# ErickRosete/tacorl

Measured on AMD Instinct MI355X. Metric: offline grad-steps/sec (batch=256, 84x84 RGB), higher is better.
Workload: dtype bf16; 1 GPU; tacorl actor-critic training_step, frozen LMP (BASELINE configs[1]); per_gpu_batch=256, global_batch=256, window=16, image=84x84x3, frames=fp32 CHW (reference batch schema), latent_plan=16, n_action_samples=4, phase=Q (epoch>=bc_epochs), action_decoder_loss=every step (reference behaviour), parallelism=dp1, hip_graph=True, losses_finite=True

## Files before the change

### include/tacorl_hip.h

```cpp
#ifndef TACORL_HIP_H
#define TACORL_HIP_H
#include <stddef.h>
#ifdef __cplusplus
extern "C" {
#endif

typedef void* tacorl_stream_t;

#define TACORL_MAXP 16
enum { TACORL_F32 = 0, TACORL_BF16 = 1 };
enum { TACORL_ACT_NONE = 0, TACORL_ACT_RELU = 1, TACORL_ACT_SILU = 2, TACORL_ACT_TANH = 3 };

int tacorl_hip_version(void);
int tacorl_hip_init(int device);
const char* tacorl_hip_last_error(void);
int tacorl_time_mark(unsigned long long* marks, int slot, tacorl_stream_t stream);
int tacorl_time_spin(unsigned long long* marks, int slot, long ticks, tacorl_stream_t stream);

int tacorl_linear_fwd(int nprob, const float* const* x, int ldx, const float* const* w,
                      const float* const* b, float* const* y, float* const* z, const int* M,
                      int K, int N, int act, int compute_dtype, tacorl_stream_t stream);
size_t tacorl_linear_add_fwd_ws_bytes(int nprob, const int* M, int K, int N);
int tacorl_linear_add_fwd(int nprob, const float* const* x, int ldx, const float* const* w,
                          const float* const* b, const float* const* addend, int ld_add, float* const* y,
                          int ldy, const int* M, int K, int N, int act, int compute_dtype, void* ws,
                          size_t ws_bytes, tacorl_stream_t stream);
int tacorl_rnn_linear_supported(int M, int K, int N);
int tacorl_rnn_linear_fwd(const void* x_bf16, const void* w_bf16, const float* bias, const float* addend,
                          int ld_add, float* y, void* y_bf16, int M, int K, int N, int act,
                          tacorl_stream_t stream);
int tacorl_rnn_linear_fwd_batch(int nprob, const void* const* x_bf16, const void* const* w_bf16,
                                const float* const* bias, const float* const* addend, int ld_add,
                                float* const* y, void* const* y_bf16, int M, int K, int N, const int* acts,
                                tacorl_stream_t stream);
int tacorl_rnn_linear_fwd_batch_twin(int nprob, const void* const* x_bf16, const void* const* x2_bf16,
                                     const void* const* w_bf16, const float* const* bias, const float* const* addend,
                                     const float* const* addend2, int ld_add, float* const* y, float* const* y2,
                                     void* const* y_bf16, void* const* y2_bf16, int M, int M2, int K, int N,
                                     const int* acts, tacorl_stream_t stream);
int tacorl_rnn_linear_fwd_batch_ext(int nprob, const void* const* x_bf16, const void* const* x2_bf16,
                                    const void* const* w_bf16, const float* const* bias, const float* const* addend,
                                    const float* const* addend2, int ld_add, float* const* y, float* const* y2,
                                    void* const* y_bf16, void* const* y2_bf16, int M, int M2, int K, int N,
                                    const int* acts, const void* const* x_ext, const void* const* x2_ext,
                                    const void* const* w_ext, const float* const* bias2, tacorl_stream_t stream);
int tacorl_rnn_linear_ld_supported(int M, int K, int N, int ldx, int ldy);
int tacorl_rnn_linear_ld(int nprob, const void* const* x_bf16, int ldx, const void* const* w_bf16, const float* const* bias,
                         const float* const* bias2, const float* const* addend, int ld_add, const void* const* x_ext,
                         const void* const* w_ext, const float* const* mask_src, float* const* y, void* const* y_bf16, int ldy,
                         int M, int K, int N, int act, tacorl_stream_t stream);
int tacorl_build_ad_input_bf16(const float* plan, const float* emb, int ld_emb, void* out_bf16, int B, int T, int Tm,
                               int P, int E, tacorl_stream_t stream);
int tacorl_rnn_linear_bwd_step(const void* x_bf16, const void* wt_bf16, const float* addend, int ld_add,
                               const float* mask_src, float* y, void* y_bf16, int M, int K, int N,
                               tacorl_stream_t stream);
int tacorl_rnn_wgrad_supported(int R, int M, int N);
int tacorl_rnn_wgrad(const void* dz_bf16, int ld_dz, const void* x_bf16, int ld_x, int R, int M, int N, float* dw,
                     float* db, int accumulate, tacorl_stream_t stream);
int tacorl_rnn_wgrad_batch(int n, const void* const* dz_bf16, int ld_dz, const void* const* x_bf16, int ld_x, const int* R,
                           int M, int N, float* const* dw, float* const* db, int accumulate, tacorl_stream_t stream);
size_t tacorl_rnn_wgrad_slabs_ws_bytes(int slabs, int Mp, int N);
int tacorl_rnn_wgrad_slabs(const void* dz_bf16, int ld_dz, const void* x_bf16, int ld_x, int R, int Mp, int N, int rows,
                           int slabs, float* dw, float* db, int accumulate, void* ws, size_t ws_bytes, tacorl_stream_t stream);
int tacorl_rnn_linear_bwd_batch(int nprob, const void* const* x_bf16, const void* const* wt_bf16,
                                const float* const* addend, int ld_add, const float* const* mask_src,
                                float* const* y, void* const* y_bf16, int M, int K, int N, tacorl_stream_t stream);
int tacorl_birnn_swap_rows(const float* src, int ld_src, float* dst, int ld_dst, int n_outer, int n_inner, int cols,
                           tacorl_stream_t stream);
int tacorl_transpose_to_bf16(const float* src, void* dst, int R, int C, tacorl_stream_t stream);
int tacorl_transpose_to_bf16_batch(int n, const float* const* src, void* const* dst, const int* R, const int* C,
                                   tacorl_stream_t stream);
int tacorl_transpose_pad_to_bf16(const float* src, void* dst, int R, int C, int ld_dst, tacorl_stream_t stream);
int tacorl_pad_to_bf16(const float* src, int ld_src, void* dst, int ld_dst, long rows, int cols, tacorl_stream_t stream);

int tacorl_linear_dgrad(int nprob, const float* const* dz, int ld_dz, const float* const* w,
                        float* const* out, int ld_out, const float* const* src, int ld_src, int act_src,
                        const float* const* addend, int ld_add, const int* M, int O, int I,
                        int compute_dtype, tacorl_stream_t stream);
size_t tacorl_linear_dgrad_ws_bytes(int nprob, const int* M, int O, int I);
int tacorl_linear_dgrad_splitk(int nprob, const float* const* dz, int ld_dz, const float* const* w,
                               float* const* out, int ld_out, const float* const* src, int ld_src, int act_src,
                               const float* const* addend, int ld_add, const int* M, int O, int I,
                               int compute_dtype, void* ws, size_t ws_bytes, tacorl_stream_t stream);
size_t tacorl_linear_wgrad_ws_bytes(int nprob, const int* M, int K, int O);
int tacorl_linear_wgrad(int nprob, const float* const* x, int ldx, const float* const* dz, int ld_dz,
                        const int* M, int K, int O, float* const* dw, float* const* db, int accumulate,
                        int compute_dtype, void* ws, size_t ws_bytes, tacorl_stream_t stream);
int tacorl_conv2d_relu_fwd(int nprob, const void* const* x, const float* const* w,
                           const float* const* b, float* const* y, const int* n_img, int H, int W,
                           int C, int KH, int KW, int S, int CO, int x_dtype, int compute_dtype,
                           tacorl_stream_t stream);

long tacorl_encoder_param_layout(long* offsets11);
long tacorl_encoder_act_layout(int n_img, int H, int W, long* offsets5);
int tacorl_encoder_fwd(int nprob, const void* const* img, const float* const* params,
                       float* const* out , float* const* act, const int* n_img, int H,
                       int W, int img_dtype, int compute_dtype, tacorl_stream_t stream);
size_t tacorl_encoder_bwd_ws_bytes(int nprob, const int* n_img, int H, int W);
int tacorl_encoder_bwd(int nprob, const void* const* img, const float* const* params,
                       const float* const* act, const float* const* d_out, float* const* grads,
                       const int* n_img, int H, int W, int img_dtype, int compute_dtype,
                       int accumulate, void* ws, size_t ws_bytes, tacorl_stream_t stream);

long tacorl_encoder_fused_wpk_bytes(void);
int tacorl_encoder_fused_supported(int H, int W);
int tacorl_encoder_fused_act_format(int H, int W);
int tacorl_encoder_pack_weights(int nprob, const float* const* params, void* const* packed,
                                tacorl_stream_t stream);
int tacorl_encoder_fwd_fused(int nprob, const void* const* img, const void* const* packed,
                             const float* const* params, float* const* out, float* const* act,
                             const int* n_img, int H, int W, tacorl_stream_t stream);
int tacorl_encoder_fwd_fused_wg(int nprob, const void* const* img, const void* const* packed,
                                const float* const* params, float* const* out, float* const* act,
                                const int* n_img, int H, int W, int max_workgroups, tacorl_stream_t stream);

size_t tacorl_encoder_bwd_fused_ws_bytes(int nprob, const int* n_img, int H, int W);
int tacorl_encoder_bwd_fused(int nprob, const void* const* img, const float* const* params,
                             const float* const* act, const float* const* d_out,
                             float* const* grads, const int* n_img, int H, int W, int accumulate,
                             void* ws, size_t ws_bytes, tacorl_stream_t stream);
int tacorl_encoder_bwd_fused_pack(int nprob, const float* const* params, const int* n_img, int H, int W,
                                  void* ws, size_t ws_bytes, tacorl_stream_t stream);
int tacorl_encoder_bwd_fused_head(int nprob, const float* const* params, const float* const* act,
                                  const float* const* d_out, const int* n_img, int H, int W,
                                  int prepacked, void* ws, size_t ws_bytes, tacorl_stream_t stream);
int tacorl_encoder_bwd_fused_fc_wgrad(int nprob, const float* const* act, const float* const* d_out,
                                      float* const* grads, const int* n_img, int H, int W,
                                      int accumulate, void* ws, size_t ws_bytes, tacorl_stream_t stream);
int tacorl_encoder_bwd_fused_conv(int nprob, const void* const* img, const float* const* params,
                                  const float* const* act, float* const* grads, const int* n_img, int H,
                                  int W, int accumulate, int prepacked, void* ws, size_t ws_bytes,
                                  tacorl_stream_t stream);
int tacorl_encoder_bwd_fused_conv_parts(int nprob, const void* const* img, const float* const* params,
                                        const float* const* act, float* const* grads, const int* n_img, int H,
                                        int W, int accumulate, int prepacked, int parts, void* ws,
                                        size_t ws_bytes, tacorl_stream_t stream);

long tacorl_mlp_param_layout(int n_layers, const int* dims, long* w_off, long* b_off);
long tacorl_mlp_act_layout(int M, int n_layers, const int* dims, const int* acts, long* z_off,
                           long* y_off);
int tacorl_mlp_fwd(int nprob, const float* const* x, int ldx, const float* const* params,
                   float* const* act, const int* M, int n_layers, const int* dims,
                   const int* acts, int compute_dtype, tacorl_stream_t stream);
int tacorl_mlp_fwd_fused_supported(int nprob, int n_layers, const int* dims, int ldx);
int tacorl_mlp_lean_supported(int nprob, int n_layers, const int* dims, int ldx, int ldo, int ldd);
int tacorl_mlp_fwd_fused(int nprob, const float* const* x, int ldx, const float* const* params,
                         const void* const* params_bf16, float* const* act, const int* M,
                         int n_layers, const int* dims, const int* acts, int lean, tacorl_stream_t stream);
int tacorl_mlp_fwd_fused_gather_supported(int nprob, const int* M, int n_layers, const int* dims, const int* acts,
                                          int ldx, int lean);
int tacorl_mlp_fwd_fused_gather(int nprob, const int* nseg, const float* const* seg_ptr, const int* seg_ld,
                                const int* seg_c0, const int* seg_mod, float* const* x_out, int ldx,
                                const float* const* params, const void* const* params_bf16, float* const* act,
                                const int* M, int n_layers, const int* dims, const int* acts, int lean,
                                tacorl_stream_t stream);
int tacorl_to_bf16_batch(int n, const float* const* src, void* const* dst, const long* count,
                         tacorl_stream_t stream);
size_t tacorl_mlp_bwd_ws_bytes(int nprob, const int* M, int n_layers, const int* dims);
int tacorl_mlp_bwd(int nprob, const float* const* x, int ldx, const float* const* params,
                   const float* const* act, const float* const* d_out, int ldo, float* const* grads,
                   float* const* d_x, int ldd, const int* M, int n_layers, const int* dims,
                   const int* acts, int compute_dtype, int accumulate, void* ws, size_t ws_bytes,
                   tacorl_stream_t stream);
int tacorl_mlp_bwd_fused_supported(int nprob, int n_layers, const int* dims, int ldo, int ldd);
size_t tacorl_mlp_bwd_fused_ws_bytes(int nprob, const int* M, int n_layers, const int* dims);
int tacorl_mlp_bwd_fused_dgrad(int nprob, const float* const* params, const float* const* act,
                               const float* const* d_out, int ldo, float* const* d_x, int ldd,
                               const int* M, int n_layers, const int* dims, const int* acts,
                               int prepacked, void* ws, size_t ws_bytes, tacorl_stream_t stream);
int tacorl_mlp_bwd_fused_pack(int nprob, const float* const* params, const int* M, int n_layers,
                              const int* dims, void* ws, size_t ws_bytes, tacorl_stream_t stream);
int tacorl_prep_batch_begin(void);
int tacorl_reduce_batch_begin(void);
int tacorl_reduce_batch_end(tacorl_stream_t stream);
int tacorl_prep_batch_end(tacorl_stream_t stream);
int tacorl_mlp_bwd_fused_wgrad(int nprob, const float* const* x, int ldx, const float* const* act,
                               const float* const* d_out, int ldo, float* const* grads, const int* M,
                               int n_layers, const int* dims, const int* acts, int accumulate, int lean,
                               void* ws, size_t ws_bytes, tacorl_stream_t stream);

int tacorl_pack_images(const float* src, long img_pitch, int src_nchw, void* dst, int dst_dtype,
                       int n, int C, int H, int W, tacorl_stream_t stream);
int tacorl_pack_images_batch(int njobs, const float* const* src, const long* img_pitch, void* const* dst,
                             const int* n_img, int dst_dtype, int H, int W, tacorl_stream_t stream);
int tacorl_pack_images_window_batch(int njobs, const float* const* src, const long* img_pitch, void* const* dst,
                                    const int* n_img, void* const* dst_first, void* const* dst_last,
                                    const int* window, int dst_dtype, int H, int W, tacorl_stream_t stream);
int tacorl_pack_images_u8_batch(int njobs, const void* const* src, const long* img_pitch_bytes, void* const* dst,
                                const int* n_img, int dst_dtype, int H, int W, tacorl_stream_t stream);
int tacorl_pack_images_u8_gather_batch(int njobs, const void* const* src, const long* img_pitch_bytes,
                                       const long* const* index, const int* index_stride, void* const* dst,
                                       const int* n_img, int dst_dtype, int H, int W, tacorl_stream_t stream);
int tacorl_gather_frames_u8(const void* frames, long frame_bytes, const long* index, void* dst, long n,
                            tacorl_stream_t stream);
int tacorl_pack_images_u8_aug_batch(int njobs, const void* const* src, const long* img_pitch_bytes,
                                    void* const* dst, const int* const* shift, const float* const* jitter,
                                    const int* n_img, int dst_dtype, int H, int W, int pad,
                                    tacorl_stream_t stream);
int tacorl_pack_images_u8_resize_aug_gather_batch(int njobs, const void* const* src, const long* img_pitch_bytes,
                                                  const long* const* index, const int* index_stride, void* const* dst,
                                                  const int* const* shift, const float* const* jitter, const int* n_img,
                                                  int dst_dtype, int src_H, int src_W, int H, int W, int pad,
                                                  tacorl_stream_t stream);
int tacorl_pack_images_u8_aug_gather_batch(int njobs, const void* const* src, const long* img_pitch_bytes,
                                           const long* const* index, const int* index_stride, void* const* dst,
                                           const int* const* shift, const float* const* jitter, const int* n_img,
                                           int dst_dtype, int H, int W, int pad, tacorl_stream_t stream);
int tacorl_stage_transition(const void* disp, int disp_dtype, float* reward, float* done, int B,
                            const float* acts_src, float* acts_dst, long n_acts, tacorl_stream_t stream);
int tacorl_sample_transitions(const long* possible_steps, long n_possible, const long* ep_start, const long* ep_end,
                              int n_episodes, const long* nn_ptr, long n_nn, const long* nn_val, const float* actions,
                              const long* idx, const long* strategy, const long* disp, const double* u_choice,
                              long current_horizon, long n_frames, int B, int A, long* ids, float* action,
                              float* reward, float* done, int* status, tacorl_stream_t stream);
int tacorl_copy_cols(const float* src, int ld_src, float* dst, int ld_dst, int rows, int cols,
                     int src_row_mod, int accumulate, tacorl_stream_t stream);
int tacorl_copy_cols_batch(int n, const float* const* src, const int* ld_src, float* const* dst,
                           const int* ld_dst, const int* rows, const int* cols,
                           const int* src_row_mod, const int* accumulate, tacorl_stream_t stream);
int tacorl_reduce_rows_mod(const float* in, int ld_in, float* out, int ld_out, int B, int cols,
                           int reps, tacorl_stream_t stream);
int tacorl_reduce_rows_mod_batch(int n, const float* const* in, int ld_in, float* const* out, int ld_out, int B,
                                 int cols, int reps, tacorl_stream_t stream);
int tacorl_uniform_actions(const float* u01, float* dst, int ld_dst, int rows, int A,
                           int discrete_gripper, tacorl_stream_t stream);

int tacorl_tanh_normal_sample(const float* head, int ld_head, const float* eps, const float* gumbel_u,
                              int hard_rsample, float* act_out, int ld_act, float* logp, int* grip_idx,
                              int n, int M, int Ac, tacorl_stream_t stream);
int tacorl_tanh_normal_sample_batch(int njobs, const float* const* head, int ld_head,
                                    const float* const* eps, const float* const* gumbel_u,
                                    const int* hard_rsample, float* const* act_out, int ld_act,
                                    float* const* logp, int* const* grip_idx, const int* n, int M, int Ac,
                                    const float* u01, float* u_dst, int u_rows, int A, int u_discrete,
                                    tacorl_stream_t stream);

int tacorl_add_rows_bcast(const float* x, int ldx, const float* add, float* out, int R, int T, int D,
                          int Dp, tacorl_stream_t stream);
int tacorl_attention_fwd(const float* qkv, float* out, int B, int T, int D, int H, tacorl_stream_t stream);
int tacorl_attention_dropout_fwd(const float* qkv, float* out, const unsigned char* keep, float keep_scale, int B,
                                 int T, int D, int H, tacorl_stream_t stream);
int tacorl_attention_dropout_bwd(const float* qkv, const float* d_out, float* d_qkv, const unsigned char* keep,
                                 float keep_scale, int B, int T, int D, int H, tacorl_stream_t stream);
int tacorl_dropout_mul(float* x, const unsigned char* keep, float keep_scale, long n, tacorl_stream_t stream);
int tacorl_add_layernorm_fwd(const float* x, const float* res, const float* w, const float* b, float* y,
                             float* stats, int R, int D, float eps, tacorl_stream_t stream);
int tacorl_pr_encoder_fused_supported(int D, int T, int H, int FF, int L);
int tacorl_pr_encoder_fused_train_supported(int D, int T, int H, int FF, int L);
int tacorl_pr_encoder_fused(const float* emb, int ld_emb, const float* params, const void* params_bf16,
                            const long* offsets, float* pooled, int B, int D, int T, int H, int FF, int L,
                            tacorl_stream_t stream);
int tacorl_pr_encoder_fused_sample(const float* emb, int ld_emb, const float* params, const void* params_bf16,
                                   const long* offsets, float* pooled, int B, int D, int T, int H, int FF, int L,
                                   const float* Wc, const float* bc, const float* eps, float* head, float* plan,
                                   int A, float min_std, tacorl_stream_t stream);
int tacorl_pr_encoder_fused_train(const float* emb, int ld_emb, const float* params, const void* params_bf16,
                                  const long* offsets, float* pooled, int B, int D, int T, int H, int FF, int L,
                                  float* const* save, tacorl_stream_t stream);
int tacorl_pr_encoder_bwd_fused(const float* params, const long* offsets, const float* d_pool, const float* d_head,
                                const float* Wc, int A2, float* dx, const float* const* saved, float* const* dz,
                                const void* const* wt, float* ln_part, float* const* ln_grads, int B, int D, int T, int H,
                                int FF, int L, tacorl_stream_t stream);
int tacorl_pr_encoder_fused_train_sample(const float* emb, int ld_emb, const float* params, const void* params_bf16,
                                         const long* offsets, float* pooled, int B, int D, int T, int H, int FF, int L,
                                         float* const* save, const float* Wc, const float* bc, const float* eps,
                                         float* head, float* plan, int A, float min_std, tacorl_stream_t stream);
int tacorl_pr_head_compose(const float* w_fc, const float* b_fc, const float* w_head, const float* b_head,
                           float* Wc, float* bc, int D, int FC, int A2, tacorl_stream_t stream);
int tacorl_mean_over_t(const float* x, float* out, int B, int T, int D, tacorl_stream_t stream);
int tacorl_pr_sample(const float* head, const float* eps, float* plan, float* mu_out, float* std_out,
                     int B, int A, float min_std, tacorl_stream_t stream);

int tacorl_build_ad_input(const float* plan, const float* emb, int ld_emb, float* out, int B, int T,
// ... 89 lines not shown
```

### tacorl_amd/_lib.py

```python
import ctypes as C
import os

HERE = os.path.dirname(os.path.abspath(__file__))
LIB_PATH = os.environ.get("TACORL_HIP_LIB") or os.path.join(HERE, "lib", "libtacorl_hip.so")

F32, BF16 = 0, 1
ACT_NONE, ACT_RELU, ACT_SILU, ACT_TANH = 0, 1, 2, 3
MAXP = 16

LOG_SLOTS = [
    "alpha_loss", "alpha", "actor_loss", "bellman_q1_loss", "bellman_q2_loss", "conservative_q1_loss",
    "conservative_q2_loss", "q1_loss", "q2_loss", "alpha_prime", "alpha_prime_loss", "q1_data", "q1_random",
    "q1_policy", "q2_data", "q2_random", "q2_policy", "action_loss",
]

_p, _i, _l, _f, _sz = C.c_void_p, C.c_int, C.c_long, C.c_float, C.c_size_t
_SIGS = {
    "tacorl_hip_version": (_i, []),
    "tacorl_hip_init": (_i, [_i]),
    "tacorl_hip_last_error": (C.c_char_p, []),
    "tacorl_time_mark": (_i, [_p, _i, _p]),
    "tacorl_time_spin": (_i, [_p, _i, _l, _p]),
    "tacorl_linear_fwd": (_i, [_i, _p, _i, _p, _p, _p, _p, _p, _i, _i, _i, _i, _p]),
    "tacorl_linear_add_fwd_ws_bytes": (_sz, [_i, _p, _i, _i]),
    "tacorl_linear_add_fwd": (_i, [_i, _p, _i, _p, _p, _p, _i, _p, _i, _p, _i, _i, _i, _i, _p, _sz, _p]),
    "tacorl_rnn_linear_supported": (_i, [_i, _i, _i]),
    "tacorl_rnn_linear_fwd": (_i, [_p, _p, _p, _p, _i, _p, _p, _i, _i, _i, _i, _p]),
    "tacorl_rnn_linear_fwd_batch": (_i, [_i, _p, _p, _p, _p, _i, _p, _p, _i, _i, _i, _p, _p]),
    "tacorl_rnn_linear_fwd_batch_twin": (_i, [_i, _p, _p, _p, _p, _p, _p, _i, _p, _p, _p, _p, _i, _i, _i, _i, _p, _p]),
    "tacorl_rnn_linear_fwd_batch_ext": (_i, [_i, _p, _p, _p, _p, _p, _p, _i, _p, _p, _p, _p, _i, _i, _i, _i, _p, _p, _p, _p, _p, _p]),
    "tacorl_rnn_linear_ld_supported": (_i, [_i, _i, _i, _i, _i]),
    "tacorl_rnn_linear_ld": (_i, [_i, _p, _i, _p, _p, _p, _p, _i, _p, _p, _p, _p, _p, _i, _i, _i, _i, _i, _p]),
    "tacorl_rnn_linear_bwd_step": (_i, [_p, _p, _p, _i, _p, _p, _p, _i, _i, _i, _p]),
    "tacorl_rnn_linear_bwd_batch": (_i, [_i, _p, _p, _p, _i, _p, _p, _p, _i, _i, _i, _p]),
    "tacorl_rnn_wgrad_supported": (_i, [_i, _i, _i]),
    "tacorl_rnn_wgrad": (_i, [_p, _i, _p, _i, _i, _i, _i, _p, _p, _i, _p]),
    "tacorl_rnn_wgrad_batch": (_i, [_i, _p, _i, _p, _i, _p, _i, _i, _p, _p, _i, _p]),
    "tacorl_rnn_wgrad_slabs_ws_bytes": (_sz, [_i, _i, _i]),
    "tacorl_rnn_wgrad_slabs": (_i, [_p, _i, _p, _i, _i, _i, _i, _i, _i, _p, _p, _i, _p, _sz, _p]),
    "tacorl_birnn_swap_rows": (_i, [_p, _i, _p, _i, _i, _i, _i, _p]),
    "tacorl_transpose_to_bf16": (_i, [_p, _p, _i, _i, _p]),
    "tacorl_transpose_to_bf16_batch": (_i, [_i, _p, _p, _p, _p, _p]),
    "tacorl_transpose_pad_to_bf16": (_i, [_p, _p, _i, _i, _i, _p]),
    "tacorl_pad_to_bf16": (_i, [_p, _i, _p, _i, _l, _i, _p]),
    "tacorl_pr_encoder_fused_supported": (_i, [_i, _i, _i, _i, _i]),
    "tacorl_pr_encoder_fused_train_supported": (_i, [_i, _i, _i, _i, _i]),
    "tacorl_pr_encoder_fused": (_i, [_p, _i, _p, _p, _p, _p, _i, _i, _i, _i, _i, _i, _p]),
    "tacorl_pr_encoder_fused_train": (_i, [_p, _i, _p, _p, _p, _p, _i, _i, _i, _i, _i, _i, _p, _p]),
    "tacorl_pr_encoder_bwd_fused": (_i, [_p, _p, _p, _p, _p, _i, _p, _p, _p, _p, _p, _p, _i, _i, _i, _i, _i, _i, _p]),
    "tacorl_pr_encoder_fused_train_sample": (_i, [_p, _i, _p, _p, _p, _p, _i, _i, _i, _i, _i, _i, _p, _p, _p, _p, _p, _p, _i, _f, _p]),
    "tacorl_pr_encoder_fused_sample": (_i, [_p, _i, _p, _p, _p, _p, _i, _i, _i, _i, _i, _i, _p, _p, _p, _p, _p, _i, _f, _p]),
    "tacorl_pr_head_compose": (_i, [_p, _p, _p, _p, _p, _p, _i, _i, _i, _p]),
    "tacorl_to_bf16_batch": (_i, [_i, _p, _p, _p, _p]),
    "tacorl_mlp_bwd_fused_supported": (_i, [_i, _i, _p, _i, _i]),
    "tacorl_mlp_bwd_fused_ws_bytes": (_sz, [_i, _p, _i, _p]),
    "tacorl_mlp_bwd_fused_dgrad": (_i, [_i, _p, _p, _p, _i, _p, _i, _p, _i, _p, _p, _i, _p, _sz, _p]),
    "tacorl_mlp_bwd_fused_pack": (_i, [_i, _p, _p, _i, _p, _p, _sz, _p]),
    "tacorl_prep_batch_begin": (_i, []),
    "tacorl_reduce_batch_begin": (_i, []),
    "tacorl_reduce_batch_end": (_i, [_p]),
    "tacorl_prep_batch_end": (_i, [_p]),
    "tacorl_mlp_bwd_fused_wgrad": (_i, [_i, _p, _i, _p, _p, _i, _p, _p, _i, _p, _p, _i, _i, _p, _sz, _p]),
    "tacorl_mlp_fwd_fused_supported": (_i, [_i, _i, _p, _i]),
    "tacorl_mlp_lean_supported": (_i, [_i, _i, _p, _i, _i, _i]),
    "tacorl_mlp_fwd_fused": (_i, [_i, _p, _i, _p, _p, _p, _p, _i, _p, _p, _i, _p]),
    "tacorl_mlp_fwd_fused_gather_supported": (_i, [_i, _p, _i, _p, _p, _i, _i]),
    "tacorl_mlp_fwd_fused_gather": (_i, [_i, _p, _p, _p, _p, _p, _p, _i, _p, _p, _p, _p, _i, _p, _p, _i, _p]),
    "tacorl_add_rows_bcast": (_i, [_p, _i, _p, _p, _i, _i, _i, _i, _p]),
    "tacorl_attention_fwd": (_i, [_p, _p, _i, _i, _i, _i, _p]),
    "tacorl_attention_dropout_fwd": (_i, [_p, _p, _p, _f, _i, _i, _i, _i, _p]),
    "tacorl_attention_dropout_bwd": (_i, [_p, _p, _p, _p, _f, _i, _i, _i, _i, _p]),
    "tacorl_dropout_mul": (_i, [_p, _p, _f, _l, _p]),
    "tacorl_add_layernorm_fwd": (_i, [_p, _p, _p, _p, _p, _p, _i, _i, _f, _p]),
    "tacorl_mean_over_t": (_i, [_p, _p, _i, _i, _i, _p]),
    "tacorl_pr_sample": (_i, [_p, _p, _p, _p, _p, _i, _i, _f, _p]),
    "tacorl_build_ad_input": (_i, [_p, _p, _i, _p, _i, _i, _i, _i, _i, _p]),
    "tacorl_build_ad_input_bf16": (_i, [_p, _p, _i, _p, _i, _i, _i, _i, _i, _p]),
    "tacorl_ad_input_proj": (_i, [_p, _p, _i, _p, _p, _p, _i, _i, _i, _i, _i, _i, _p]),
    "tacorl_logistic_mixture_ws_bytes": (_sz, [_i, _i, _i]),
    "tacorl_logistic_mixture_loss": (_i, [_p, _i, _p, _p, _p, _i, _i, _i, _i, _i, _i, _f, _f, _p, _sz, _p]),
    "tacorl_logistic_mixture_finish": (_i, [_p, _sz, _i, _i, _i, _p, _p]),
    "tacorl_logistic_mixture_sample": (_i, [_p, _i, _p, _p, _p, _i, _i, _i, _p]),
    "tacorl_linear_dgrad": (_i, [_i, _p, _i, _p, _p, _i, _p, _i, _i, _p, _i, _p, _i, _i, _i, _p]),
    "tacorl_linear_dgrad_ws_bytes": (_sz, [_i, _p, _i, _i]),
    "tacorl_linear_dgrad_splitk": (_i, [_i, _p, _i, _p, _p, _i, _p, _i, _i, _p, _i, _p, _i, _i, _i, _p, _sz, _p]),
    "tacorl_linear_wgrad_ws_bytes": (_sz, [_i, _p, _i, _i]),
    "tacorl_linear_wgrad": (_i, [_i, _p, _i, _p, _i, _p, _i, _i, _p, _p, _i, _i, _p, _sz, _p]),
    "tacorl_relu_mask_mul": (_i, [_p, _p, _p, _p, _l, _p]),
    "tacorl_ad_input_bwd": (_i, [_p, _p, _p, _i, _i, _i, _i, _i, _i, _i, _p]),
    "tacorl_plmp_demb_finish": (_i, [_p, _p, _i, _i, _p, _i, _p, _p, _i, _i, _i, _i, _p]),
    "tacorl_bcast_over_t": (_i, [_p, _p, _i, _i, _i, _f, _i, _p]),
    "tacorl_attention_bwd": (_i, [_p, _p, _p, _i, _i, _i, _i, _p]),
    "tacorl_add_layernorm_bwd_ws_bytes": (_sz, [_i, _i]),
    "tacorl_add_layernorm_bwd": (_i, [_p, _p, _p, _p, _p, _p, _p, _p, _i, _i, _i, _p, _sz, _p]),
    "tacorl_gauss_kl_balanced": (_i, [_p, _p, _p, _p, _i, _i, _f, _f, _f, _i, _f, _p, _p]),
    "tacorl_pr_sample_bwd": (_i, [_p, _p, _p, _p, _i, _i, _f, _p]),
    "tacorl_conv2d_relu_fwd": (_i, [_i, _p, _p, _p, _p, _p, _i, _i, _i, _i, _i, _i, _i, _i, _i, _p]),
    "tacorl_encoder_param_layout": (_l, [_p]),
    "tacorl_encoder_act_layout": (_l, [_i, _i, _i, _p]),
    "tacorl_encoder_fwd": (_i, [_i, _p, _p, _p, _p, _p, _i, _i, _i, _i, _p]),
    "tacorl_encoder_bwd_ws_bytes": (_sz, [_i, _p, _i, _i]),
    "tacorl_encoder_bwd": (_i, [_i, _p, _p, _p, _p, _p, _p, _i, _i, _i, _i, _i, _p, _sz, _p]),
    "tacorl_encoder_fused_wpk_bytes": (_l, []),
    "tacorl_encoder_fused_supported": (_i, [_i, _i]),
    "tacorl_encoder_fused_act_format": (_i, [_i, _i]),
    "tacorl_encoder_pack_weights": (_i, [_i, _p, _p, _p]),
    "tacorl_encoder_fwd_fused": (_i, [_i, _p, _p, _p, _p, _p, _p, _i, _i, _p]),
    "tacorl_encoder_fwd_fused_wg": (_i, [_i, _p, _p, _p, _p, _p, _p, _i, _i, _i, _p]),
    "tacorl_encoder_bwd_fused_ws_bytes": (_sz, [_i, _p, _i, _i]),
    "tacorl_encoder_bwd_fused": (_i, [_i, _p, _p, _p, _p, _p, _p, _i, _i, _i, _p, _sz, _p]),
    "tacorl_encoder_bwd_fused_pack": (_i, [_i, _p, _p, _i, _i, _p, _sz, _p]),
    "tacorl_encoder_bwd_fused_head": (_i, [_i, _p, _p, _p, _p, _i, _i, _i, _p, _sz, _p]),
    "tacorl_encoder_bwd_fused_fc_wgrad": (_i, [_i, _p, _p, _p, _p, _i, _i, _i, _p, _sz, _p]),
    "tacorl_encoder_bwd_fused_conv": (_i, [_i, _p, _p, _p, _p, _p, _i, _i, _i, _i, _p, _sz, _p]),
    "tacorl_encoder_bwd_fused_conv_parts": (_i, [_i, _p, _p, _p, _p, _p, _i, _i, _i, _i, _i, _p, _sz, _p]),
    "tacorl_mlp_param_layout": (_l, [_i, _p, _p, _p]),
    "tacorl_mlp_act_layout": (_l, [_i, _i, _p, _p, _p, _p]),
    "tacorl_mlp_fwd": (_i, [_i, _p, _i, _p, _p, _p, _i, _p, _p, _i, _p]),
    "tacorl_mlp_bwd_ws_bytes": (_sz, [_i, _p, _i, _p]),
    "tacorl_mlp_bwd": (_i, [_i, _p, _i, _p, _p, _p, _i, _p, _p, _i, _p, _i, _p, _p, _i, _i, _p, _sz, _p]),
    "tacorl_pack_images": (_i, [_p, _l, _i, _p, _i, _i, _i, _i, _i, _p]),
    "tacorl_pack_images_batch": (_i, [_i, _p, _p, _p, _p, _i, _i, _i, _p]),
    "tacorl_pack_images_window_batch": (_i, [_i, _p, _p, _p, _p, _p, _p, _p, _i, _i, _i, _p]),
    "tacorl_pack_images_u8_batch": (_i, [_i, _p, _p, _p, _p, _i, _i, _i, _p]),
    "tacorl_pack_images_u8_gather_batch": (_i, [_i, _p, _p, _p, _p, _p, _p, _i, _i, _i, _p]),
    "tacorl_pack_images_u8_aug_gather_batch": (_i, [_i, _p, _p, _p, _p, _p, _p, _p, _p, _i, _i, _i, _i, _p]),
    "tacorl_pack_images_u8_resize_aug_gather_batch": (_i, [_i, _p, _p, _p, _p, _p, _p, _p, _p, _i, _i, _i, _i, _i, _i, _p]),
    "tacorl_gather_frames_u8": (_i, [_p, _l, _p, _p, _l, _p]),
    "tacorl_pack_images_u8_aug_batch": (_i, [_i, _p, _p, _p, _p, _p, _p, _i, _i, _i, _i, _p]),
    "tacorl_stage_transition": (_i, [_p, _i, _p, _p, _i, _p, _p, _l, _p]),
    "tacorl_sample_transitions": (_i, [_p, _l, _p, _p, _i, _p, _l, _p, _p, _p, _p, _p, _p, _l, _l, _i, _i, _p, _p, _p, _p, _p, _p]),
    "tacorl_copy_cols": (_i, [_p, _i, _p, _i, _i, _i, _i, _i, _p]),
    "tacorl_copy_cols_batch": (_i, [_i, _p, _p, _p, _p, _p, _p, _p, _p, _p]),
    "tacorl_reduce_rows_mod": (_i, [_p, _i, _p, _i, _i, _i, _i, _p]),
    "tacorl_reduce_rows_mod_batch": (_i, [_i, _p, _i, _p, _i, _i, _i, _i, _p]),
    "tacorl_uniform_actions": (_i, [_p, _p, _i, _i, _i, _i, _p]),
    "tacorl_tanh_normal_sample": (_i, [_p, _i, _p, _p, _i, _p, _i, _p, _p, _i, _i, _i, _p]),
    "tacorl_tanh_normal_sample_batch": (_i, [_i, _p, _i, _p, _p, _p, _p, _i, _p, _p, _p, _i, _i, _p, _p, _i, _i, _i, _p]),
    "tacorl_alpha_loss": (_i, [_p, _i, _p, _f, _f, _p, _p, _p]),
    "tacorl_alpha_loss_step": (_i, [_p, _i, _p, _f, _p, _p, _p, _p, _f, _p, _p]),
    "tacorl_actor_qmin": (_i, [_p, _p, _p, _i, _p, _p, _p, _f, _p, _p]),
    "tacorl_actor_head_bwd": (_i, [_p, _i, _p, _p, _p, _p, _i, _p, _i, _p, _p, _f, _p, _i, _i, _i, _p, _p]),
    "tacorl_tanh_normal_nll": (_i, [_p, _i, _p, _i, _i, _i, _i, _f, _p, _p, _p]),
    "tacorl_cql_ws_bytes": (_sz, [_i]),
    "tacorl_cql_loss": (_i, [_p] * 13 + [_i, _i, _i, _f, _f, _f, _f, _f, _i, _f, _p, _p, _p, _sz, _p]),
    "tacorl_adam_ws_bytes": (_sz, [_l]),
    "tacorl_adam_step": (_i, [_p, _p, _p, _p, _l, _f, _f, _p, _p, _f, _p, _sz, _p]),
    "tacorl_adam_batch_ws_bytes": (_sz, [_i]),
    "tacorl_adam_step_batch": (_i, [_i, _p, _p, _p, _p, _p, _p, _p, _p, _p, _p, _p, _sz, _p]),
    "tacorl_adam_step_batch_mirror": (_i, [_i, _p, _p, _p, _p, _p, _p, _p, _p, _p, _p, _p, _p, _p, _sz, _p]),
    "tacorl_cem_supported": (_i, [_i, _i, _i, _i, _i, _i]),
    "tacorl_cem_ws_bytes": (_sz, [_i, _i, _i, _i, _i, _i, _i]),
    "tacorl_cem_refine": (_i, [_i, _i, _p, _p, _p, _p, _p, _p, _i, _i, _i, _i, _i, _i, _i, _f, _f, _f, _i, _i, _p, _p, _p, _p, _p,
                               _p, _sz, _p]),
}

_lib = None


class TacorlHipError(RuntimeError):
    pass


def lib():
    global _lib
    if _lib is None:
        import torch

        if not os.path.exists(LIB_PATH):
            raise TacorlHipError(
                f"{LIB_PATH} not found: the HIP extension is required (no CPU fallback). "
                "Build it with `python -m tacorl_amd.build`.")
        L = C.CDLL(LIB_PATH)
        override = bool(os.environ.get("TACORL_HIP_LIB"))
        missing = []
        for name, (res, args) in _SIGS.items():
            fn = getattr(L, name, None)
            if fn is None:
                missing.append(name)
                continue
            fn.restype, fn.argtypes = res, args
        if override:
            import sys

            if missing:
                raise TacorlHipError(f"TACORL_HIP_LIB={LIB_PATH} lacks {len(missing)} entry point(s) of this binding "
                                     f"({', '.join(missing[:5])}...): rebuild it from this tree")
            print(f"[tacorl_amd] TACORL_HIP_LIB override active: {LIB_PATH}", file=sys.stderr, flush=True)
        _lib = L
    return _lib


def declared_symbols():
    return list(_SIGS)


def call(name, *args):
    fn = getattr(lib(), name)
    rc = fn(*args)
    if fn.restype is _i and rc != 0:
        raise TacorlHipError(f"{name} failed ({rc}): {lib().tacorl_hip_last_error().decode()}")
    return rc


def ptr(t):
    return None if t is None else C.c_void_p(t.data_ptr())


def ptr_array(tensors):
    arr = (C.c_void_p * len(tensors))()
    for i, t in enumerate(tensors):
        if t is None:
            arr[i] = None
        elif isinstance(t, int):
            arr[i] = t
        elif isinstance(t, C.c_void_p):
            arr[i] = t.value
        else:
            arr[i] = t.data_ptr()
    return arr


def int_array(vals):
    return (C.c_int * len(vals))(*[int(v) for v in vals])


def stream():
    import torch

    return C.c_void_p(torch.cuda.current_stream().cuda_stream)
```

### tacorl_amd/csrc/dense_ops.hip

```cpp
#include <stdio.h>
#include <stdlib.h>
#include <string.h>

#include <type_traits>

#include "../../include/tacorl_hip.h"
#include "enc_bwd_fused.h"
#include "mlp_fused.h"
#include "functors.h"

static thread_local char g_err[256] = "";
#define FAIL(code, ...)                        \
  do {                                         \
    snprintf(g_err, sizeof(g_err), __VA_ARGS__); \
    return (code);                             \
  } while (0)
#define CHECK(x)            \
  do {                      \
    int _r = (x);           \
    if (_r != TACORL_OK) return _r; \
  } while (0)

extern "C" const char* tacorl_hip_last_error(void) { return g_err; }
extern "C" int tacorl_hip_version(void) { return 1; }
// ... 588 lines not shown
  hipStream_t st = (hipStream_t)stream;
  EncDims d;
  if (!enc_dims(H, W, d)) FAIL(TACORL_EINVAL, "encoder: image %dx%d too small", H, W);
  if (nprob < 1 || nprob > GEMM_MAXP) FAIL(TACORL_EINVAL, "encoder_fwd: nprob %d", nprob);
  long po[E_N];
  tacorl_encoder_param_layout(po);
  const float *w1[GEMM_MAXP], *b1[GEMM_MAXP], *w2[GEMM_MAXP], *b2[GEMM_MAXP], *w3[GEMM_MAXP], *b3[GEMM_MAXP],
      *fw1[GEMM_MAXP], *fb1[GEMM_MAXP], *fw2[GEMM_MAXP], *fb2[GEMM_MAXP];
  float *y1[GEMM_MAXP], *y2[GEMM_MAXP], *y3[GEMM_MAXP], *sa[GEMM_MAXP], *h1[GEMM_MAXP];
  for (int p = 0; p < nprob; p++) {
    long ao[5];
    tacorl_encoder_act_layout(n_img[p], H, W, ao);
    const float* P = params[p];
    w1[p] = P + po[E_W1]; b1[p] = P + po[E_B1]; w2[p] = P + po[E_W2]; b2[p] = P + po[E_B2];
    w3[p] = P + po[E_W3]; b3[p] = P + po[E_B3]; fw1[p] = P + po[E_FW1]; fb1[p] = P + po[E_FB1];
    fw2[p] = P + po[E_FW2]; fb2[p] = P + po[E_FB2];
    y1[p] = act[p] + ao[0]; y2[p] = act[p] + ao[1]; y3[p] = act[p] + ao[2]; sa[p] = act[p] + ao[3];
    h1[p] = act[p] + ao[4];
  }
  CHECK(conv_fwd_any(nprob, img, w1, b1, y1, n_img, d.c1, img_dtype, cd, st));
  CHECK(conv_fwd_any(nprob, (const void* const*)y1, w2, b2, y2, n_img, d.c2, TACORL_F32, cd, st));
  CHECK(conv_fwd_any(nprob, (const void* const*)y2, w3, b3, y3, n_img, d.c3, TACORL_F32, cd, st));
  {
    SaArgs sg{};
    int mxn = 0;
    for (int p = 0; p < nprob; p++) {
      sg.y3[p] = y3[p]; sg.temp[p] = params[p] + po[E_T]; sg.out[p] = sa[p]; sg.n[p] = n_img[p];
      mxn = n_img[p] > mxn ? n_img[p] : mxn;
    }
    if (mxn > 0) hipLaunchKernelGGL(softargmax_fwd_kernel, dim3(mxn, nprob), dim3(256), 0, st, sg, d.c3.OH, d.c3.OW);
  }
  CHECK(k_linear_fwd(nprob, sa, 128, fw1, fb1, h1, nullptr, n_img, 128, 256, 256, ACT_RELU, cd, st));
  CHECK(k_linear_fwd(nprob, h1, 256, fw2, fb2, out, nullptr, n_img, 256, 32, 32, ACT_NONE, cd, st));
  return hipGetLastError() == hipSuccess ? TACORL_OK : TACORL_ELAUNCH;
}

static size_t enc_slab_bytes(int nprob, long maxn, const EncDims& d) {
  size_t m = 0, s;
  s = wgrad_ws_bytes(nprob, 192, 32, maxn * d.c1.OH * d.c1.OW); m = s > m ? s : m;
  s = wgrad_ws_bytes(nprob, 512, 64, maxn * d.c2.OH * d.c2.OW); m = s > m ? s : m;
  s = wgrad_ws_bytes(nprob, 576, 64, maxn * d.c3.OH * d.c3.OW); m = s > m ? s : m;
  s = wgrad_ws_bytes(nprob, 128, 256, maxn); m = s > m ? s : m;
  s = wgrad_ws_bytes(nprob, 256, 32, maxn); m = s > m ? s : m;
  return m;
}
static long enc_bwd_scratch_layout(int n, const EncDims& d, long* o) {
  const long sz[6] = {(long)n * 256, (long)n * 128, (long)n * d.c3.OH * d.c3.OW * 64,
                      (long)n * d.c2.OH * d.c2.OW * 64, (long)n * d.c1.OH * d.c1.OW * 32, (long)n};
  long off = 0;
  for (int i = 0; i < 6; i++) { if (o) o[i] = off; off = al4(off + sz[i]); }
  return off;
}
extern "C" size_t tacorl_encoder_bwd_ws_bytes(int nprob, const int* n_img, int H, int W) {
  EncDims d;
  if (!enc_dims(H, W, d)) return 0;
  long tot = 0, maxn = 0;
  for (int p = 0; p < nprob; p++) { tot += enc_bwd_scratch_layout(n_img[p], d, nullptr); maxn = n_img[p] > maxn ? n_img[p] : maxn; }
  return (size_t)tot * sizeof(float) + enc_slab_bytes(nprob, maxn, d);
}

extern "C" int tacorl_encoder_bwd(int nprob, const void* const* img, const float* const* params,
                                  const float* const* act, const float* const* d_out, float* const* grads,
                                  const int* n_img, int H, int W, int img_dtype, int cd, int accumulate,
                                  void* ws, size_t ws_bytes, tacorl_stream_t stream) {
  hipStream_t st = (hipStream_t)stream;
  EncDims d;
  if (!enc_dims(H, W, d)) FAIL(TACORL_EINVAL, "encoder: image %dx%d too small", H, W);
  if (nprob < 1 || nprob * 4 > GEMM_MAXP) FAIL(TACORL_EINVAL, "encoder_bwd: nprob %d (max %d)", nprob, GEMM_MAXP / 4);
  if (ws_bytes < tacorl_encoder_bwd_ws_bytes(nprob, n_img, H, W)) FAIL(TACORL_ENOMEM, "encoder_bwd: workspace too small");
  long po[E_N];
  tacorl_encoder_param_layout(po);
  const float *w2[GEMM_MAXP], *w3[GEMM_MAXP], *fw1[GEMM_MAXP], *fw2[GEMM_MAXP];
  const float *y1[GEMM_MAXP], *y2[GEMM_MAXP], *y3[GEMM_MAXP], *sa[GEMM_MAXP], *h1[GEMM_MAXP];
  float *d_h1[GEMM_MAXP], *d_sa[GEMM_MAXP], *dz3[GEMM_MAXP], *dz2[GEMM_MAXP], *dz1[GEMM_MAXP], *dtp[GEMM_MAXP];
  float *g_w1[GEMM_MAXP], *g_b1[GEMM_MAXP], *g_w2[GEMM_MAXP], *g_b2[GEMM_MAXP], *g_w3[GEMM_MAXP], *g_b3[GEMM_MAXP],
      *g_fw1[GEMM_MAXP], *g_fb1[GEMM_MAXP], *g_fw2[GEMM_MAXP], *g_fb2[GEMM_MAXP];
  float* cur = (float*)ws;
  long maxn = 0;
  for (int p = 0; p < nprob; p++) {
    long ao[5], so[6];
    tacorl_encoder_act_layout(n_img[p], H, W, ao);
    const long tot = enc_bwd_scratch_layout(n_img[p], d, so);
    const float* P = params[p];
    w2[p] = P + po[E_W2]; w3[p] = P + po[E_W3]; fw1[p] = P + po[E_FW1]; fw2[p] = P + po[E_FW2];
    y1[p] = act[p] + ao[0]; y2[p] = act[p] + ao[1]; y3[p] = act[p] + ao[2]; sa[p] = act[p] + ao[3]; h1[p] = act[p] + ao[4];
    d_h1[p] = cur + so[0]; d_sa[p] = cur + so[1]; dz3[p] = cur + so[2]; dz2[p] = cur + so[3]; dz1[p] = cur + so[4]; dtp[p] = cur + so[5];
    cur += tot;
    float* G = grads[p];
    g_w1[p] = G + po[E_W1]; g_b1[p] = G + po[E_B1]; g_w2[p] = G + po[E_W2]; g_b2[p] = G + po[E_B2];
    g_w3[p] = G + po[E_W3]; g_b3[p] = G + po[E_B3]; g_fw1[p] = G + po[E_FW1]; g_fb1[p] = G + po[E_FB1];
    g_fw2[p] = G + po[E_FW2]; g_fb2[p] = G + po[E_FB2];
    maxn = n_img[p] > maxn ? n_img[p] : maxn;
  }
  void* slab = cur;
  const size_t slab_bytes = enc_slab_bytes(nprob, maxn, d);
  CHECK(k_linear_wgrad(nprob, h1, 256, d_out, 32, n_img, 256, 32, g_fw2, g_fb2, accumulate, slab, slab_bytes, cd, st));
  CHECK(k_linear_dgrad(nprob, d_out, 32, fw2, d_h1, 256, h1, ACT_RELU, n_img, 32, 256, cd, st));
  CHECK(k_linear_wgrad(nprob, sa, 128, (const float* const*)d_h1, 256, n_img, 128, 256, g_fw1, g_fb1, accumulate, slab, slab_bytes, cd, st));
  CHECK(k_linear_dgrad(nprob, (const float* const*)d_h1, 256, fw1, d_sa, 128, nullptr, ACT_NONE, n_img, 256, 128, cd, st));
  {
    SaArgs sg{};
    int mxn = 0;
    for (int p = 0; p < nprob; p++) {
      sg.y3[p] = y3[p]; sg.temp[p] = params[p] + po[E_T]; sg.sa[p] = sa[p]; sg.d_sa[p] = d_sa[p]; sg.out[p] = dz3[p];
      sg.dtp[p] = dtp[p]; sg.n[p] = n_img[p];
      mxn = n_img[p] > mxn ? n_img[p] : mxn;
    }
    const int P3 = d.c3.OH * d.c3.OW;
    if (cd == TACORL_BF16 && nprob <= EBW_MAXP && P3 > 4 * SAB_MAXI_BIG && P3 <= 4 * SAB_MAXI_HUGE) {
      SabArgs sb{};
      for (int p = 0; p < nprob; p++) {
        sb.y3[p] = y3[p]; sb.temp[p] = params[p] + po[E_T]; sb.sa[p] = sa[p]; sb.d_sa[p] = d_sa[p]; sb.dz3[p] = dz3[p];
        sb.dtp[p] = dtp[p]; sb.gtemp[p] = grads[p] + po[E_T]; sb.n[p] = n_img[p];
      }
      if (mxn > 0) {
        hipLaunchKernelGGL(softargmax_bwd_batch_kernel<SAB_MAXI_HUGE>, dim3(mxn, nprob), dim3(256), 0, st, sb, P3, d.c3.OW);
        hipLaunchKernelGGL(sum_to_scalar_batch_kernel, dim3(nprob), dim3(256), 0, st, sb, accumulate);
      }
    } else {
      if (mxn > 0) hipLaunchKernelGGL(softargmax_bwd_kernel, dim3(mxn, nprob), dim3(256), 0, st, sg, d.c3.OH, d.c3.OW);
      for (int p = 0; p < nprob; p++)
        if (n_img[p] > 0)
          hipLaunchKernelGGL(sum_to_scalar_kernel, dim3(1), dim3(256), 0, st, dtp[p], n_img[p], grads[p] + po[E_T], accumulate);
    }
  }
  CHECK(k_conv_wgrad<float>(nprob, (const void* const*)y2, (const float* const*)dz3, n_img, d.c3, g_w3, g_b3, accumulate, slab, slab_bytes, cd, st));
  CHECK(k_conv_dgrad(nprob, (const float* const*)dz3, w3, dz2, y2, n_img, d.c3, cd, st));
  CHECK(k_conv_wgrad<float>(nprob, (const void* const*)y1, (const float* const*)dz2, n_img, d.c2, g_w2, g_b2, accumulate, slab, slab_bytes, cd, st));
  CHECK(k_conv_dgrad(nprob, (const float* const*)dz2, w2, dz1, y1, n_img, d.c2, cd, st));
  if (img_dtype == TACORL_BF16)
    CHECK(k_conv_wgrad<__bf16>(nprob, img, (const float* const*)dz1, n_img, d.c1, g_w1, g_b1, accumulate, slab, slab_bytes, cd, st));
  else
    CHECK(k_conv_wgrad<float>(nprob, img, (const float* const*)dz1, n_img, d.c1, g_w1, g_b1, accumulate, slab, slab_bytes, cd, st));
  return hipGetLastError() == hipSuccess ? TACORL_OK : TACORL_ELAUNCH;
}

static const int kFcDims[3] = {128, 256, 32};
static size_t enc_fc_slab_bytes(int nprob, long maxn) {
  size_t a = wgrad_ws_bytes(nprob, 256, 32, maxn), b = wgrad_ws_bytes(nprob, 128, 256, maxn);
  int Mx[EBW_MAXP];
  for (int p = 0; p < nprob && p < EBW_MAXP; p++) Mx[p] = (int)maxn;
  const size_t c = mlp_fused_wgrad_slab_floats(nprob, Mx, 2, kFcDims) * sizeof(float);
  a = a > b ? a : b;
  return ((a > c ? a : c) + 255) & ~(size_t)255;
}
struct EncBwdPlan {
  EncDims d;
  long po[E_N];
  size_t scratch_bytes, fcwt_off[EBW_MAXP], fcwt_each, slab_off, slab_bytes, conv_off, total;
  long so[EBW_MAXP][6], ao[EBW_MAXP][5], sbase[EBW_MAXP];
  long maxn;
};
static const int kFcActs[2] = {ACT_RELU, ACT_NONE};
static bool enc_bwd_plan(int nprob, const int* n_img, int H, int W, EncBwdPlan& pl) {
  if (!enc_dims(H, W, pl.d) || !ebw_supported(H, W) || nprob < 1 || nprob > EBW_MAXP) return false;
  tacorl_encoder_param_layout(pl.po);
  long tot = 0;
  pl.maxn = 0;
  for (int p = 0; p < nprob; p++) {
    pl.sbase[p] = tot;
    tot += enc_bwd_scratch_layout(n_img[p], pl.d, pl.so[p]);
    tacorl_encoder_act_layout(n_img[p], H, W, pl.ao[p]);
    pl.maxn = n_img[p] > pl.maxn ? n_img[p] : pl.maxn;
  }
  size_t b = ((size_t)tot * sizeof(float) + 255) & ~(size_t)255;
  pl.scratch_bytes = b;
  pl.fcwt_each = (mlp_fused_wt_elems(2, kFcDims, nullptr) * 2 + 255) & ~(size_t)255;
  for (int p = 0; p < nprob; p++) { pl.fcwt_off[p] = b; b += pl.fcwt_each; }
  pl.slab_off = b;
  pl.slab_bytes = enc_fc_slab_bytes(nprob, pl.maxn);
  b += pl.slab_bytes;
  pl.conv_off = b;
  pl.total = b + ebw_ws_bytes(nprob, n_img, H, W);
  return true;
}
extern "C" size_t tacorl_encoder_bwd_fused_ws_bytes(int nprob, const int* n_img, int H, int W) {
  EncBwdPlan pl;
  return enc_bwd_plan(nprob, n_img, H, W, pl) ? pl.total : 0;
}
static void enc_bwd_conv_problems(int nprob, const void* const* img, const float* const* params, const float* const* act,
                                  float* const* grads, const int* n_img, const EncBwdPlan& pl, void* ws, EbwProblem* pr) {
  for (int p = 0; p < nprob; p++) {
    const float* P = params[p];
    float* G = grads ? grads[p] : nullptr;
    float* sc = (float*)ws + pl.sbase[p];
    pr[p].img = img ? img[p] : nullptr;
    pr[p].y1 = act ? act[p] + pl.ao[p][0] : nullptr; pr[p].y2 = act ? act[p] + pl.ao[p][1] : nullptr;
    pr[p].dz3 = sc + pl.so[p][2];
    pr[p].w2 = P + pl.po[E_W2]; pr[p].w3 = P + pl.po[E_W3];
    pr[p].g_w1 = G ? G + pl.po[E_W1] : nullptr; pr[p].g_b1 = G ? G + pl.po[E_B1] : nullptr;
    pr[p].g_w2 = G ? G + pl.po[E_W2] : nullptr; pr[p].g_b2 = G ? G + pl.po[E_B2] : nullptr;
    pr[p].g_w3 = G ? G + pl.po[E_W3] : nullptr; pr[p].g_b3 = G ? G + pl.po[E_B3] : nullptr;
    pr[p].n = n_img[p];
  }
}
static int enc_bwd_fc_chain(int nprob, const float* const* params, const float* const* act, const float* const* d_out,
                            const int* n_img, const EncBwdPlan& pl, void* ws, hipStream_t st, int mode) {
  long wo[2], bo[2], src[MF_MAXP * MF_MAXL], dzo[MF_MAXP * MF_MAXL];
  tacorl_mlp_param_layout(2, kFcDims, wo, bo);
  const float* fcp[EBW_MAXP];
  float *dz[EBW_MAXP], *dsa[EBW_MAXP];
  void* wt[EBW_MAXP];
  for (int p = 0; p < nprob; p++) {
    fcp[p] = params[p] + pl.po[E_FW1];
    src[p * MF_MAXL + 0] = pl.ao[p][4];
    src[p * MF_MAXL + 1] = -1;
    dzo[p * MF_MAXL + 0] = pl.sbase[p] + pl.so[p][0];
    dz[p] = (float*)ws;
    dsa[p] = (float*)ws + pl.sbase[p] + pl.so[p][1];
    wt[p] = (unsigned char*)ws + pl.fcwt_off[p];
  }
  return mlp_fused_bwd(nprob, fcp, act, d_out, 32, dz, dsa, 128, wt, n_img, 2, kFcDims, kFcActs, src, dzo, wo, st, mode);
}

extern "C" int tacorl_encoder_bwd_fused_pack(int nprob, const float* const* params, const int* n_img, int H, int W,
                                             void* ws, size_t ws_bytes, tacorl_stream_t stream) {
  EncBwdPlan pl;
  if (!enc_bwd_plan(nprob, n_img, H, W, pl)) FAIL(TACORL_EINVAL, "encoder_bwd_fused_pack: geometry %dx%d / nprob %d", H, W, nprob);
  if (ws_bytes < pl.total) FAIL(TACORL_ENOMEM, "encoder_bwd_fused_pack: workspace too small");
  EbwProblem pr[EBW_MAXP];
  enc_bwd_conv_problems(nprob, nullptr, params, nullptr, nullptr, n_img, pl, ws, pr);
  int rc = enc_bwd_fc_chain(nprob, params, nullptr, nullptr, n_img, pl, ws, (hipStream_t)stream, 1);
  if (rc == TACORL_OK) rc = ebw_conv_backward(nprob, pr, H, W, 0, (unsigned char*)ws + pl.conv_off, pl.total - pl.conv_off, (hipStream_t)stream, 1);
  if (rc != TACORL_OK) FAIL(rc, "encoder_bwd_fused_pack: launch failed (%d)", rc);
  return TACORL_OK;
}
extern "C" int tacorl_encoder_bwd_fused_head(int nprob, const float* const* params, const float* const* act,
                                             const float* const* d_out, const int* n_img, int H, int W, int prepacked,
                                             void* ws, size_t ws_bytes, tacorl_stream_t stream) {
  EncBwdPlan pl;
  if (!enc_bwd_plan(nprob, n_img, H, W, pl)) FAIL(TACORL_EINVAL, "encoder_bwd_fused_head: geometry %dx%d / nprob %d", H, W, nprob);
  if (ws_bytes < pl.total) FAIL(TACORL_ENOMEM, "encoder_bwd_fused_head: workspace too small");
  const int rc = enc_bwd_fc_chain(nprob, params, act, d_out, n_img, pl, ws, (hipStream_t)stream, prepacked ? 2 : 0);
  if (rc != TACORL_OK) FAIL(rc, "encoder_bwd_fused_head: launch failed (%d)", rc);
  return TACORL_OK;
}
extern "C" int tacorl_encoder_bwd_fused_fc_wgrad(int nprob, const float* const* act, const float* const* d_out,
                                                 float* const* grads, const int* n_img, int H, int W, int accumulate,
                                                 void* ws, size_t ws_bytes, tacorl_stream_t stream) {
  hipStream_t st = (hipStream_t)stream;
  EncBwdPlan pl;
  if (!enc_bwd_plan(nprob, n_img, H, W, pl)) FAIL(TACORL_EINVAL, "encoder_bwd_fused_fc_wgrad: geometry %dx%d / nprob %d", H, W, nprob);
  if (ws_bytes < pl.total) FAIL(TACORL_ENOMEM, "encoder_bwd_fused_fc_wgrad: workspace too small");
  const float *sa[EBW_MAXP], *h1[EBW_MAXP], *d_h1[EBW_MAXP];
  float *g_fw1[EBW_MAXP], *g_fb1[EBW_MAXP], *g_fw2[EBW_MAXP], *g_fb2[EBW_MAXP];
  for (int p = 0; p < nprob; p++) {
    sa[p] = act[p] + pl.ao[p][3]; h1[p] = act[p] + pl.ao[p][4];
    d_h1[p] = (const float*)ws + pl.sbase[p] + pl.so[p][0];
    float* G = grads[p];
    g_fw1[p] = G + pl.po[E_FW1]; g_fb1[p] = G + pl.po[E_FB1]; g_fw2[p] = G + pl.po[E_FW2]; g_fb2[p] = G + pl.po[E_FB2];
  }
  void* slab = (unsigned char*)ws + pl.slab_off;
  if (mlp_fused_wgrad_ok(nprob, 2, kFcDims) &&
      mlp_fused_wgrad_slab_floats(nprob, n_img, 2, kFcDims) * sizeof(float) <= pl.slab_bytes) {
    long yoffs[MF_MAXP * MF_MAXL] = {}, dzoffs[MF_MAXP * MF_MAXL] = {};
    const float* dzb[EBW_MAXP];
    for (int p = 0; p < nprob; p++) {
      yoffs[p * MF_MAXL] = pl.ao[p][4];
      dzoffs[p * MF_MAXL] = pl.sbase[p] + pl.so[p][0];
      dzb[p] = (const float*)ws;
    }
    const long wo[2] = {pl.po[E_FW1], pl.po[E_FW2]}, bo[2] = {pl.po[E_FB1], pl.po[E_FB2]};
    if (mlp_fused_wgrad(nprob, sa, 128, act, d_out, 32, dzb, grads, (float*)slab, n_img, 2, kFcDims, yoffs, dzoffs, wo, bo,
                        accumulate, st))
      FAIL(TACORL_ELAUNCH, "encoder_bwd_fused_fc_wgrad: launch failed");
    return TACORL_OK;
  }
  CHECK(k_linear_wgrad(nprob, h1, 256, d_out, 32, n_img, 256, 32, g_fw2, g_fb2, accumulate, slab, pl.slab_bytes, TACORL_BF16, st));
  CHECK(k_linear_wgrad(nprob, sa, 128, d_h1, 256, n_img, 128, 256, g_fw1, g_fb1, accumulate, slab, pl.slab_bytes, TACORL_BF16, st));
  return TACORL_OK;
}
extern "C" int tacorl_encoder_bwd_fused_conv(int nprob, const void* const* img, const float* const* params,
                                             const float* const* act, float* const* grads, const int* n_img, int H, int W,
                                             int accumulate, int prepacked, void* ws, size_t ws_bytes,
                                             tacorl_stream_t stream) {
  return tacorl_encoder_bwd_fused_conv_parts(nprob, img, params, act, grads, n_img, H, W, accumulate, prepacked, 127, ws,
                                             ws_bytes, stream);
}
extern "C" int tacorl_encoder_bwd_fused_conv_parts(int nprob, const void* const* img, const float* const* params,
                                                   const float* const* act, float* const* grads, const int* n_img, int H,
                                                   int W, int accumulate, int prepacked, int parts, void* ws,
                                                   size_t ws_bytes, tacorl_stream_t stream) {
  hipStream_t st = (hipStream_t)stream;
  EncBwdPlan pl;
  if (!enc_bwd_plan(nprob, n_img, H, W, pl)) FAIL(TACORL_EINVAL, "encoder_bwd_fused_conv: geometry %dx%d / nprob %d", H, W, nprob);
  if (ws_bytes < pl.total) FAIL(TACORL_ENOMEM, "encoder_bwd_fused_conv: workspace too small");
  if (pl.d.c3.OH * pl.d.c3.OW > 4 * SAB_MAXI_HUGE) FAIL(TACORL_EINVAL, "encoder_bwd_fused: conv3 output too large");
  EbwProblem pr[EBW_MAXP];
  enc_bwd_conv_problems(nprob, img, params, act, grads, n_img, pl, ws, pr);
  SabArgs sb{};
  for (int p = 0; p < nprob; p++) {
    float* sc = (float*)ws + pl.sbase[p];
    sb.y3[p] = act[p] + pl.ao[p][2]; sb.temp[p] = params[p] + pl.po[E_T]; sb.sa[p] = act[p] + pl.ao[p][3];
    sb.d_sa[p] = sc + pl.so[p][1]; sb.dz3[p] = sc + pl.so[p][2]; sb.dtp[p] = sc + pl.so[p][5];
    sb.gtemp[p] = grads[p] + pl.po[E_T]; sb.n[p] = n_img[p];
  }
  const char* fe = getenv("TACORL_EBW_FUSE3");
  const int fuse3 = fe ? atoi(fe) : 1;
  const bool fused3 = fuse3 && (parts & 127) == 127 && ebw_fused3_supported(H, W);
  if (fused3) {
    for (int p = 0; p < nprob; p++) {
      pr[p].y3 = sb.y3[p]; pr[p].temp = sb.temp[p]; pr[p].sa = sb.sa[p]; pr[p].d_sa = sb.d_sa[p];
      pr[p].dtp = sb.dtp[p]; pr[p].g_temp = sb.gtemp[p];
    }
  }
  if (pl.maxn > 0 && (parts & 1) && !fused3) {
    const int P3 = pl.d.c3.OH * pl.d.c3.OW;
    if (P3 <= 4 * 13) hipLaunchKernelGGL(softargmax_bwd_batch_kernel<13>, dim3((unsigned)pl.maxn, nprob), dim3(256), 0, st, sb, P3, pl.d.c3.OW);
    else if (P3 <= 4 * SAB_MAXI_BIG) hipLaunchKernelGGL(softargmax_bwd_batch_kernel<SAB_MAXI_BIG>, dim3((unsigned)pl.maxn, nprob), dim3(256), 0, st, sb, P3, pl.d.c3.OW);
    else hipLaunchKernelGGL(softargmax_bwd_batch_kernel<SAB_MAXI_HUGE>, dim3((unsigned)pl.maxn, nprob), dim3(256), 0, st, sb, P3, pl.d.c3.OW);
    hipLaunchKernelGGL(sum_to_scalar_batch_kernel, dim3(nprob), dim3(256), 0, st, sb, accumulate);
  }
  if (!(parts & EBW_ALL)) return hipGetLastError() == hipSuccess ? TACORL_OK : TACORL_ELAUNCH;
  if ((parts & EBW_ALL) != EBW_ALL && !prepacked) FAIL(TACORL_EINVAL, "encoder_bwd_fused_conv_parts: partial calls need prepacked fragments");
  const int rc = ebw_conv_backward(nprob, pr, H, W, accumulate, (unsigned char*)ws + pl.conv_off, pl.total - pl.conv_off, st, prepacked ? 2 : 0,
                                   (parts & EBW_ALL) | (fused3 ? EBW_FUSED3 : 0));
  if (rc != TACORL_OK) FAIL(rc, "encoder_bwd_fused_conv: conv backward launch failed (%d)", rc);
  return hipGetLastError() == hipSuccess ? TACORL_OK : TACORL_ELAUNCH;
}
extern "C" int tacorl_encoder_bwd_fused(int nprob, const void* const* img, const float* const* params,
                                        const float* const* act, const float* const* d_out, float* const* grads,
                                        const int* n_img, int H, int W, int accumulate, void* ws, size_t ws_bytes,
                                        tacorl_stream_t stream) {
  int rc = tacorl_encoder_bwd_fused_head(nprob, params, act, d_out, n_img, H, W, 0, ws, ws_bytes, stream);
  if (rc == TACORL_OK) rc = tacorl_encoder_bwd_fused_fc_wgrad(nprob, act, d_out, grads, n_img, H, W, accumulate, ws, ws_bytes, stream);
  if (rc == TACORL_OK) rc = tacorl_encoder_bwd_fused_conv(nprob, img, params, act, grads, n_img, H, W, accumulate, 0, ws, ws_bytes, stream);
  return rc;
}

extern "C" long tacorl_mlp_param_layout(int L, const int* dims, long* w_off, long* b_off) {
  long off = 0;
  for (int l = 0; l < L; l++) {
    if (w_off) w_off[l] = off;
    off = al4(off + (long)dims[l + 1] * dims[l]);
    if (b_off) b_off[l] = off;
    off = al4(off + dims[l + 1]);
  }
  return off;
}
extern "C" long tacorl_mlp_act_layout(int M, int L, const int* dims, const int* acts, long* z_off, long* y_off) {
  long off = 0;
  for (int l = 0; l < L; l++) {
    if (z_off) z_off[l] = -1;
    if (acts[l] == ACT_SILU) { if (z_off) z_off[l] = off; off = al4(off + (long)M * dims[l + 1]); }
    if (y_off) y_off[l] = off;
    off = al4(off + (long)M * dims[l + 1]);
  }
  return off;
}
#define MLP_MAXL 8

struct OutActTbl { const float* d[GEMM_MAXP]; const float* y[GEMM_MAXP]; float* dz[GEMM_MAXP]; int M[GEMM_MAXP]; };
__global__ __launch_bounds__(256) void out_act_grad_kernel(OutActTbl t, int ldo, int N, int act) {
  const int p = blockIdx.y;
  const long total = (long)t.M[p] * N;
  for (long e = (long)blockIdx.x * 256 + threadIdx.x; e < total; e += (long)gridDim.x * 256) {
    const long m = e / N;
    t.dz[p][e] = t.d[p][m * ldo + (e - m * N)] * act_grad(act, t.y[p][e]);
  }
}
static int out_act_grad(int nprob, const OutActTbl& t, int ldo, int N, int act, hipStream_t st) {
  long mx = 0;
  for (int p = 0; p < nprob; p++) mx = (long)t.M[p] * N > mx ? (long)t.M[p] * N : mx;
  if (mx == 0) return TACORL_OK;
  const int gx = cdiv(mx, 256) > 1024 ? 1024 : cdiv(mx, 256);
  hipLaunchKernelGGL(out_act_grad_kernel, dim3(gx, nprob), dim3(256), 0, st, t, ldo, N, act);
  return hipGetLastError() == hipSuccess ? TACORL_OK : TACORL_ELAUNCH;
}

extern "C" int tacorl_mlp_fwd(int nprob, const float* const* x, int ldx, const float* const* params,
                              float* const* act, const int* M, int L, const int* dims, const int* acts, int cd,
                              tacorl_stream_t stream) {
  hipStream_t st = (hipStream_t)stream;
  if (L < 1 || L > MLP_MAXL || nprob < 1 || nprob > GEMM_MAXP) FAIL(TACORL_EINVAL, "mlp_fwd: bad L/nprob");
  long wo[MLP_MAXL], bo[MLP_MAXL];
  tacorl_mlp_param_layout(L, dims, wo, bo);
  for (int l = 0; l < L; l++) {
    const float *xin[GEMM_MAXP], *w[GEMM_MAXP], *b[GEMM_MAXP];
    float *y[GEMM_MAXP], *z[GEMM_MAXP];
    for (int p = 0; p < nprob; p++) {
      long zo[MLP_MAXL], yo[MLP_MAXL];
      tacorl_mlp_act_layout(M[p], L, dims, acts, zo, yo);
      xin[p] = l == 0 ? x[p] : act[p] + yo[l - 1];
      w[p] = params[p] + wo[l]; b[p] = params[p] + bo[l];
      y[p] = act[p] + yo[l]; z[p] = zo[l] >= 0 ? act[p] + zo[l] : nullptr;
    }
    CHECK(k_linear_fwd(nprob, xin, l == 0 ? ldx : dims[l], w, b, y, z, M, dims[l], dims[l + 1], dims[l + 1], acts[l], cd, st));
  }
  return TACORL_OK;
}

extern "C" int tacorl_mlp_fwd_fused_supported(int nprob, int L, const int* dims, int ldx) {
  return mlp_fused_fwd_ok(nprob, L, dims, ldx) ? 1 : 0;
}
extern "C" int tacorl_mlp_lean_supported(int nprob, int L, const int* dims, int ldx, int ldo, int ldd) {
  return mlp_fused_fwd_ok(nprob, L, dims, ldx) && mlp_fused_bwd_ok(nprob, L, dims, ldo, ldd) && mlp_fused_wgrad_ok(nprob, L, dims) ? 1 : 0;
}
static int mlp_fwd_fused_impl(int nprob, const float* const* x, int ldx, const float* const* params,
                              const void* const* params_bf16, float* const* act, const int* M, int L,
                              const int* dims, const int* acts, int lean, tacorl_stream_t stream, const MlpXGather* gather) {
  if (!mlp_fused_fwd_ok(nprob, L, dims, ldx)) FAIL(TACORL_EINVAL, "mlp_fwd_fused: shapes not supported");
  long wo[MLP_MAXL], bo[MLP_MAXL];
  tacorl_mlp_param_layout(L, dims, wo, bo);
  const float *xs[2][MF_MAXP], *ps[2][MF_MAXP];
  const void* pb[2][MF_MAXP];
  float* as[2][MF_MAXP];
  int Ms[2][MF_MAXP], gm[2][MF_MAXP], n[2] = {0, 0};
  long zo[MF_MAXP * MF_MAXL], yo[MF_MAXP * MF_MAXL], ybf[MF_MAXP * MF_MAXL], sbf[MF_MAXP * MF_MAXL], yout[MF_MAXP];
  for (int p = 0; p < nprob; p++) {
    long z1[MLP_MAXL], y1[MLP_MAXL];
    tacorl_mlp_act_layout(M[p], L, dims, acts, z1, y1);
    const int b = (lean && mlp_big_prob_ok(M[p], L, dims, acts)) ? 1 : 0, q = n[b]++;
    gm[b][q] = p;
    xs[b][q] = x ? x[p] : nullptr; ps[b][q] = params[p]; pb[b][q] = params_bf16[p]; as[b][q] = act[p]; Ms[b][q] = M[p];
    for (int l = 0; l < L; l++) {
      if (b) { ybf[q * MF_MAXL + l] = y1[l]; sbf[q * MF_MAXL + l] = z1[l]; }
      else {
        zo[q * MF_MAXL + l] = z1[l];
        yo[q * MF_MAXL + l] = (lean && l + 1 < L && z1[l] >= 0) ? -1 : y1[l];
      }
    }
    if (b) yout[q] = y1[L - 1];
  }
  if (n[1]) {
    const int rc = mlp_big_fwd(n[1], xs[1], ldx, ps[1], pb[1], as[1], Ms[1], L, dims, acts, ybf, sbf, yout, wo, bo, (hipStream_t)stream, gather, gm[1]);
    if (rc != TACORL_OK) FAIL(rc, "mlp_fwd_fused: many-row launch failed (%d)", rc);
  }
  if (n[0]) {
    const int rc = mlp_fused_fwd(n[0], xs[0], ldx, ps[0], pb[0], as[0], Ms[0], L, dims, acts, zo, yo, wo, bo, (hipStream_t)stream, gather, gm[0]);
    if (rc != TACORL_OK) FAIL(rc, "mlp_fwd_fused: launch failed (%d)", rc);
  }
  return TACORL_OK;
}
extern "C" int tacorl_mlp_fwd_fused(int nprob, const float* const* x, int ldx, const float* const* params,
                                    const void* const* params_bf16, float* const* act, const int* M, int L,
                                    const int* dims, const int* acts, int lean, tacorl_stream_t stream) {
  return mlp_fwd_fused_impl(nprob, x, ldx, params, params_bf16, act, M, L, dims, acts, lean, stream, nullptr);
}
extern "C" int tacorl_mlp_fwd_fused_gather_supported(int nprob, const int* M, int L, const int* dims, const int* acts, int ldx,
                                                     int lean) {
  (void)M; (void)acts; (void)lean;
  return mlp_fused_fwd_ok(nprob, L, dims, ldx) ? 1 : 0;
}
extern "C" int tacorl_mlp_fwd_fused_gather(int nprob, const int* nseg, const float* const* seg_ptr, const int* seg_ld,
                                           const int* seg_c0, const int* seg_mod, float* const* x_out, int ldx,
                                           const float* const* params, const void* const* params_bf16, float* const* act,
                                           const int* M, int L, const int* dims, const int* acts, int lean,
                                           tacorl_stream_t stream) {
  if (nprob < 1 || nprob > MF_MAXP || !nseg || !seg_ptr || !seg_ld || !seg_c0 || !seg_mod) FAIL(TACORL_EINVAL, "mlp_fwd_fused_gather: arguments");
  MlpXGather g{};
  for (int p = 0; p < nprob; p++) {
    if (nseg[p] < 1 || nseg[p] > MF_MAXSEG) FAIL(TACORL_EINVAL, "mlp_fwd_fused_gather: nseg[%d] = %d", p, nseg[p]);
    g.nseg[p] = nseg[p];
    g.xw[p] = x_out ? x_out[p] : nullptr;
    for (int t = 0; t < nseg[p]; t++) {
      g.ptr[p][t] = seg_ptr[MF_MAXSEG * p + t]; g.ld[p][t] = seg_ld[MF_MAXSEG * p + t];
      g.c0[p][t] = seg_c0[MF_MAXSEG * p + t]; g.mod[p][t] = seg_mod[MF_MAXSEG * p + t];
    }
  }
  return mlp_fwd_fused_impl(nprob, nullptr, ldx, params, params_bf16, act, M, L, dims, acts, lean, stream, &g);
}
struct ToBf16Tbl { const float* src[16]; __bf16* dst[16]; long n4[16]; };
__global__ void to_bf16_batch_kernel(ToBf16Tbl t) {
  const int b = blockIdx.y;
  for (long q = (long)blockIdx.x * blockDim.x + threadIdx.x; q < t.n4[b]; q += (long)gridDim.x * blockDim.x) {
    const f32x4 v = reinterpret_cast<const f32x4*>(t.src[b])[q];
    reinterpret_cast<bf16x4*>(t.dst[b])[q] = bf16x4{(__bf16)v[0], (__bf16)v[1], (__bf16)v[2], (__bf16)v[3]};
  }
}
extern "C" int tacorl_to_bf16_batch(int n, const float* const* src, void* const* dst, const long* count,
                                    tacorl_stream_t stream) {
  if (n < 1 || n > 16) FAIL(TACORL_EINVAL, "to_bf16_batch: n %d", n);
  ToBf16Tbl t{};
  long mx = 0;
  for (int i = 0; i < n; i++) {
    if (count[i] % 4 || !aligned16(src[i]) || ((uintptr_t)dst[i] & 7)) FAIL(TACORL_EINVAL, "to_bf16_batch: count %% 4 and alignment");
    t.src[i] = src[i]; t.dst[i] = (__bf16*)dst[i]; t.n4[i] = count[i] / 4;
    mx = t.n4[i] > mx ? t.n4[i] : mx;
  }
  if (mx == 0) return TACORL_OK;
// ... 268 lines not shown
```

### tacorl_amd/csrc/enc_bwd_fused.h

```cpp
#pragma once
#include <hip/hip_runtime.h>
#include <stddef.h>

#define EBW_MAXP 8

struct EbwProblem {
  const void* img;
  const void* y1;
  const void* y2;
  const float* dz3;
  const float* w2;
  const float* w3;
  float *g_w1, *g_b1, *g_w2, *g_b2, *g_w3, *g_b3;
  int n;
  const float *y3, *temp, *sa, *d_sa;
  float *dtp, *g_temp;
};

bool ebw_supported(int H, int W);
size_t ebw_ws_bytes(int nprob, const int* n_img, int H, int W);
enum { EBW_DGRAD3 = 2, EBW_WGRAD3 = 4, EBW_DGRAD2 = 8, EBW_WGRAD2 = 16, EBW_WGRAD1 = 32, EBW_REDUCE = 64, EBW_ALL = 126,
       EBW_FUSED3 = 128 };
bool ebw_fused3_supported(int H, int W);
int ebw_conv_backward(int nprob, const EbwProblem* pr, int H, int W, int accumulate, void* ws, size_t ws_bytes,
                      hipStream_t st, int mode, int parts = EBW_ALL);
```

### tacorl_amd/csrc/encoder_bwd_fused.hip

```cpp
#include "enc_bwd_fused.h"

#include <stdlib.h>

#include <type_traits>

#include "common.h"

namespace {

#ifndef EBW_ROLL_IMG
#define EBW_ROLL_IMG 0
#endif
constexpr int NT = 512;
constexpr int NW = NT / 64;

constexpr int cmax(int a, int b) { return a > b ? a : b; }
constexpr int pitch8(int need) { return (need % 16 <= 8) ? need - need % 16 + 8 : need - need % 16 + 24; }

template <int KH_, int S_, int CI_, int CO_, int IH_, int IW_>
struct ConvL {
  static constexpr int KH = KH_, KW = KH_, S = S_, CI = CI_, CO = CO_, IH = IH_, IW = IW_;
  static constexpr int OH = (IH - KH) / S + 1, OW = (IW - KW) / S + 1;
  static constexpr int PH = (IH + S - 1) / S, PW = (IW + S - 1) / S;
  static constexpr int KA = KH / S, KB = KW / S;
  static constexpr int TAPS = KH * KW * CI;
  static constexpr int NPL = CI * S * S;
  static constexpr int PWP = (PW + 7) / 8 * 8;
  static constexpr int KQ = (OH * PWP + 31) / 32 * 32;
  static constexpr int PLP = pitch8(cmax(PH * PWP, (KA - 1) * PWP + KQ));
  static constexpr int NCOPY = KB;
  static constexpr int DZP = KQ + 8;
  static constexpr int MT = CO / 16, NTL = TAPS / 16;
  static constexpr int SLABF = CO * TAPS + CO;
  static constexpr int HA = KA - 1, HB = KB - 1, R = PH + HA, C = PW + 8, PP = CO + 16;
  static_assert(HB <= 8, "halo columns");
  static constexpr int KS = KA * KB * CO / 32;
  static constexpr int NCLS = S * S, NTI = CI / 16;
  static constexpr int MTC = (PH * PW + 15) / 16;
  static constexpr int NCOMBO = NCLS * NTI;
  static_assert(TAPS % 16 == 0 && CO % 32 == 0 && KH % S == 0, "tile shapes");
};

template <int H, int W>
struct Geo {
  using L1 = ConvL<8, 4, 3, 32, H, W>;
  using L2 = ConvL<4, 2, 32, 64, L1::OH, L1::OW>;
  using L3 = ConvL<3, 1, 64, 64, L2::OH, L2::OW>;
};

__device__ __forceinline__ uint32_t pack2(float a, float b) {
  const __bf16 x = (__bf16)a, y = (__bf16)b;
  return (uint32_t)__builtin_bit_cast(unsigned short, x) | ((uint32_t)__builtin_bit_cast(unsigned short, y) << 16);
}
__device__ __forceinline__ void load8(const float* p, float (&v)[8]) {
  const f32x4 a = *reinterpret_cast<const f32x4*>(p), b = *reinterpret_cast<const f32x4*>(p + 4);
  v[0] = a[0]; v[1] = a[1]; v[2] = a[2]; v[3] = a[3]; v[4] = b[0]; v[5] = b[1]; v[6] = b[2]; v[7] = b[3];
}
__device__ __forceinline__ void load8(const __bf16* p, float (&v)[8]) {
  const bf16x8 a = *reinterpret_cast<const bf16x8*>(p);
#pragma unroll
  for (int j = 0; j < 8; j++) v[j] = (float)a[j];
}
__device__ __forceinline__ bf16x8 load8v(const float* p) {
  float v[8];
  load8(p, v);
  bf16x8 r;
#pragma unroll
  for (int j = 0; j < 8; j++) r[j] = (__bf16)v[j];
  return r;
}
__device__ __forceinline__ bf16x8 load8v(const __bf16* p) { return *reinterpret_cast<const bf16x8*>(p); }

struct WgArgs {
  const void* in[EBW_MAXP];
  const void* dz[EBW_MAXP];
  int n[EBW_MAXP];
  float* slab;
  int wpp;
};

typedef __bf16 bf16x4v __attribute__((ext_vector_type(4)));
#define LDS_BF4(p) ((__attribute__((address_space(3))) bf16x4v*)(p))
__device__ __forceinline__ bf16x8 tr_frag(const __bf16* lo, const __bf16* hi) {
  const bf16x4v a = __builtin_amdgcn_ds_read_tr16_b64_v4bf16(LDS_BF4(lo));
  const bf16x4v b = __builtin_amdgcn_ds_read_tr16_b64_v4bf16(LDS_BF4(hi));
  return __builtin_shufflevector(a, b, 0, 1, 2, 3, 4, 5, 6, 7);
}

template <class L> struct TrTile;
template <int H, int W> struct TrTile<ConvL<3, 1, 64, 64, H, W>> { static constexpr int MGRP = 2, NGRP = 4, KGRP = 1, NBUF = 2, CIP = 80; };
template <int H, int W> struct TrTile<ConvL<4, 2, 32, 64, H, W>> { static constexpr int MGRP = 2, NGRP = 4, KGRP = 1, NBUF = 2, CIP = 40; };
template <int H, int W> struct TrTile<ConvL<8, 4, 3, 32, H, W>> { static constexpr int MGRP = 1, NGRP = 4, KGRP = 2, NBUF = 1, CIP = 3; };

template <class L>
struct TrGeo {
  using T = TrTile<L>;
  static constexpr bool IMG = L::CI < 8;
  static constexpr int DZR = L::CO + 16;
  static constexpr int CIP = T::CIP;
  static constexpr int NPIX_ALL = L::OH * L::OW;
  static constexpr size_t bytes_for(int nband) {
    const int br = (L::OH + nband - 1) / nband, rows = nband == 1 ? L::IH : (br - 1) * L::S + L::KH;
    return ((size_t)((br * L::OW + 31) / 32 * 32) * DZR + (size_t)(rows * L::IW * CIP + 7) / 8 * 8) * 2;
  }
  static constexpr size_t WHOLE_BYTES = bytes_for(1);
  static constexpr int NBAND = bytes_for(1) <= 160 * 1024 ? 1 : bytes_for(2) <= 160 * 1024 ? 2 : bytes_for(3) <= 160 * 1024 ? 3 : 4;
  static constexpr int BR = (L::OH + NBAND - 1) / NBAND;
  static constexpr int BROWS = NBAND == 1 ? L::IH : (BR - 1) * L::S + L::KH;
  static constexpr int NPIX = BR * L::OW, KS = (NPIX + 31) / 32, KQ = KS * 32;
  static constexpr int DZ_EL = KQ * DZR;
  static constexpr int IN_EL = (BROWS * L::IW * CIP + 7) / 8 * 8;
  static constexpr int BUF_EL = DZ_EL + IN_EL;
  static constexpr int NBUF = (T::NBUF == 2 && (size_t)2 * BUF_EL * 2 <= 160 * 1024 && NBAND == 1) ? 2 : 1;
  static constexpr int MPW = L::MT / T::MGRP, NPW = L::NTL / T::NGRP, TPW = MPW * NPW;
  static constexpr size_t lds_bytes = (size_t)NBUF * BUF_EL * 2;
  static constexpr int SLABF = T::KGRP * (L::CO * L::TAPS + L::CO);
  static_assert(L::MT % T::MGRP == 0 && L::NTL % T::NGRP == 0 && T::MGRP * T::NGRP * T::KGRP == NW, "wave tiling");
  static_assert(lds_bytes <= 160 * 1024, "wgrad tile does not fit LDS");
};

template <class L, class InT, class DzT>
__global__ __launch_bounds__(NT) void ebw_wgrad_tr_kernel(WgArgs a) {
  using G = TrGeo<L>;
  using T = TrTile<L>;
  constexpr bool IMG = L::CI < 8;
  extern __shared__ __attribute__((aligned(16))) unsigned char smem[];
  __bf16* lds = reinterpret_cast<__bf16*>(smem);
  const int tid = threadIdx.x, lane = tid & 63, w = tid >> 6, g = lane >> 4, l16 = lane & 15, q = l16 >> 2, pc = l16 & 3;
  const int p = blockIdx.x / a.wpp, j0 = blockIdx.x - p * a.wpp;
  const int n_img = a.n[p];
  const int ng = w % T::NGRP, mg = (w / T::NGRP) % T::MGRP, kg = w / (T::NGRP * T::MGRP);
  for (int e = tid; e < (int)(G::lds_bytes / 4); e += NT) reinterpret_cast<uint32_t*>(lds)[e] = 0u;
  int toff[G::NPW];
#pragma unroll
  for (int j = 0; j < G::NPW; j++) {
    const int nt = ng * G::NPW + j;
    if constexpr (IMG) {
      const int tap = 16 * nt + 4 * pc, ky = tap / (L::KW * L::CI), rem = tap - ky * (L::KW * L::CI);
      toff[j] = ky * L::IW * L::CI + rem;
    } else {
      constexpr int CPT16 = L::CI / 16;
      const int kk = nt / CPT16, c0 = 16 * (nt - kk * CPT16), ky = kk / L::KW, kx = kk - ky * L::KW;
      toff[j] = (ky * L::IW + kx) * G::CIP + c0 + 4 * pc;
    }
  }
  f32x4 acc[G::MPW][G::NPW], bacc[G::MPW];
#pragma unroll
  for (int i = 0; i < G::MPW; i++) {
    bacc[i] = f32x4{0.f, 0.f, 0.f, 0.f};
#pragma unroll
    for (int j = 0; j < G::NPW; j++) acc[i][j] = f32x4{0.f, 0.f, 0.f, 0.f};
  }
  bf16x8 ones;
#pragma unroll
  for (int j = 0; j < 8; j++) ones[j] = (__bf16)1.0f;
  const InT* in = reinterpret_cast<const InT*>(a.in[p]);
  const DzT* dz = reinterpret_cast<const DzT*>(a.dz[p]);
  constexpr int DCG = L::CO / 8, DCH = G::NPIX * DCG, DCPT = (DCH + NT - 1) / NT;
  constexpr int ICH = G::BROWS * L::IW * L::CI / 8, ICPT = (ICH + NT - 1) / NT;
  static_assert((G::BROWS * L::IW * L::CI) % 8 == 0 && (G::NBAND == 1 || (G::BR * L::S * L::IW * L::CI) % 8 == 0), "image / band bytes");
  bf16x8 dpre[DCPT], ipre[ICPT];
  auto band_rows = [&](int b) { return G::NBAND == 1 ? L::OH : (L::OH - b * G::BR < G::BR ? L::OH - b * G::BR : G::BR); };
  auto fetch = [&](int img, int b) {
    const int dch = G::NBAND == 1 ? DCH : band_rows(b) * L::OW * DCG;
    const DzT* d = dz + ((long)img * G::NPIX_ALL + (long)b * G::BR * L::OW) * L::CO;
#pragma unroll
    for (int r = 0; r < DCPT; r++) {
      const int c = tid + r * NT;
      dpre[r] = load8v(d + 8 * (c < dch ? c : dch - 1));
    }
    const int ich = G::NBAND == 1 ? ICH : ((band_rows(b) - 1) * L::S + L::KH) * L::IW * L::CI / 8;
    const InT* s = in + (long)img * L::IH * L::IW * L::CI + (long)b * G::BR * L::S * L::IW * L::CI;
#pragma unroll
    for (int r = 0; r < ICPT; r++) {
      const int c = tid + r * NT;
      ipre[r] = load8v(s + 8 * (c < ich ? c : ich - 1));
    }
  };
  auto put = [&](__bf16* buf, int b) {
    const int dch = G::NBAND == 1 ? DCH : band_rows(b) * L::OW * DCG;
#pragma unroll
    for (int r = 0; r < DCPT; r++) {
      const int c = tid + r * NT;
      if (c < dch) *reinterpret_cast<bf16x8*>(buf + (c / DCG) * G::DZR + 8 * (c % DCG)) = dpre[r];
      else if (G::NBAND > 1 && c < DCH) *reinterpret_cast<bf16x8*>(buf + (c / DCG) * G::DZR + 8 * (c % DCG)) = bf16x8{};
    }
    __bf16* ib = buf + G::DZ_EL;
    const int ich = G::NBAND == 1 ? ICH : ((band_rows(b) - 1) * L::S + L::KH) * L::IW * L::CI / 8;
#pragma unroll
    for (int r = 0; r < ICPT; r++) {
      const int c = tid + r * NT;
      if (c < ich) {
        if constexpr (IMG) *reinterpret_cast<bf16x8*>(ib + 8 * c) = ipre[r];
        else *reinterpret_cast<bf16x8*>(ib + (c / (L::CI / 8)) * G::CIP + 8 * (c % (L::CI / 8))) = ipre[r];
      }
    }
  };
  auto compute = [&](const __bf16* buf, int b) {
    const __bf16* dzs = buf;
    const __bf16* ins = buf + G::DZ_EL;
    const int npix = G::NBAND == 1 ? G::NPIX : band_rows(b) * L::OW;
    auto kstep = [&](int s) {
      if (T::KGRP > 1 && (s % T::KGRP) != kg) return;
      const int P0 = 32 * s + 4 * g + q, P1 = P0 + 16;
      const int Q0 = P0 < npix ? P0 : npix - 1, Q1 = P1 < npix ? P1 : npix - 1;
      const int b0 = ((Q0 / L::OW) * L::S * L::IW + (Q0 % L::OW) * L::S) * G::CIP;
      const int b1 = ((Q1 / L::OW) * L::S * L::IW + (Q1 % L::OW) * L::S) * G::CIP;
      bf16x8 A[G::MPW];
#pragma unroll
      for (int i = 0; i < G::MPW; i++) {
        const int col = 16 * (mg * G::MPW + i) + 4 * pc;
        A[i] = tr_frag(dzs + P0 * G::DZR + col, dzs + P1 * G::DZR + col);
      }
#pragma unroll
      for (int j = 0; j < G::NPW; j++) {
        const bf16x8 B = tr_frag(ins + b0 + toff[j], ins + b1 + toff[j]);
#pragma unroll
        for (int i = 0; i < G::MPW; i++) acc[i][j] = __builtin_amdgcn_mfma_f32_16x16x32_bf16(A[i], B, acc[i][j], 0, 0, 0);
      }
      if (ng == 0) {
#pragma unroll
        for (int i = 0; i < G::MPW; i++) bacc[i] = __builtin_amdgcn_mfma_f32_16x16x32_bf16(A[i], ones, bacc[i], 0, 0, 0);
      }
    };
    if constexpr (G::KS > 4 && (!IMG || EBW_ROLL_IMG || G::KS > 16)) {
#pragma unroll 1
      for (int s = 0; s < G::KS; s++) kstep(s);
    } else {
#pragma unroll
      for (int s = 0; s < G::KS; s++) kstep(s);
    }
  };
  __syncthreads();
  if constexpr (G::NBUF == 2) {
    if (j0 < n_img) { fetch(j0, 0); put(lds, 0); }
    __syncthreads();
    int k = 0;
    for (int img = j0; img < n_img; img += a.wpp, k ^= 1) {
      const int nxt = img + a.wpp;
      if (nxt < n_img) fetch(nxt, 0);
      compute(lds + k * G::BUF_EL, 0);
      if (nxt < n_img) put(lds + (k ^ 1) * G::BUF_EL, 0);
      __syncthreads();
    }
  } else {
    if (j0 < n_img) fetch(j0, 0);
    for (int img = j0; img < n_img; img += a.wpp) {
#pragma unroll 1
      for (int b = 0; b < G::NBAND; b++) {
        __syncthreads();
        put(lds, b);
        __syncthreads();
        if (b + 1 < G::NBAND) fetch(img, b + 1);
        else if (img + a.wpp < n_img) fetch(img + a.wpp, 0);
        compute(lds, b);
      }
    }
  }
  float* sl = a.slab + (long)blockIdx.x * G::SLABF;
#pragma unroll
  for (int i = 0; i < G::MPW; i++)
#pragma unroll
    for (int j = 0; j < G::NPW; j++)
      *reinterpret_cast<f32x4*>(sl + (((w * G::MPW + i) * G::NPW + j) * 64 + lane) * 4) = acc[i][j];
  if (ng == 0 && l16 == 0) {
#pragma unroll
    for (int i = 0; i < G::MPW; i++)
#pragma unroll
      for (int r = 0; r < 4; r++)
        sl[T::KGRP * L::CO * L::TAPS + kg * L::CO + 16 * (mg * G::MPW + i) + 4 * g + r] = bacc[i][r];
  }
}

struct RdTrArgs {
  const float* slab[3];
  float* gw[3][EBW_MAXP];
  float* gb[3][EBW_MAXP];
  int co[3], taps[3], mpw[3], npw[3], mgrp[3], ngrp[3], kgrp[3], slabf[3];
  int ileave[3];
  int wpp, accumulate;
  const float* dtp[EBW_MAXP];
  float* g_temp[EBW_MAXP];
  int ndt[EBW_MAXP];
};
__global__ __launch_bounds__(256) void ebw_reduce_tr_kernel(RdTrArgs a) {
  __shared__ float sh[4][64];
  const int l = blockIdx.y % 3, p = blockIdx.y / 3;
  const int nW = a.co[l] * a.taps[l], per = nW + a.co[l], KG = a.kgrp[l];
  const int e = blockIdx.x * 64 + (threadIdx.x & 63), kq = threadIdx.x >> 6;
  if (a.ndt[p] > 0 && l == 0 && blockIdx.x == gridDim.x - 1) {
    float s = 0.f;
    for (int i = threadIdx.x; i < a.ndt[p]; i += 256) s += a.dtp[p][i];
    s = wave_sum(s);
    if ((threadIdx.x & 63) == 0) sh[0][kq] = s;
    __syncthreads();
    if (threadIdx.x == 0) {
      const float v = ((sh[0][0] + sh[0][1]) + sh[0][2]) + sh[0][3];
      *a.g_temp[p] = a.accumulate ? *a.g_temp[p] + v : v;
    }
    return;
  }
  if (blockIdx.x * 64 >= per) return;
  float sum = 0.f;
  if (e < per) {
    const float* s0 = a.slab[l] + (long)p * a.wpp * a.slabf[l];
    for (int kg = 0; kg < KG; kg++) {
      const float* s = s0 + (e < nW ? (long)kg * nW + e : (long)KG * nW + kg * a.co[l] + (e - nW));
#pragma unroll 8
      for (int k = kq; k < a.wpp; k += 4) sum += s[(long)k * a.slabf[l]];
    }
  }
  sh[kq][threadIdx.x & 63] = sum;
  __syncthreads();
  if (kq == 0 && e < per) {
    const int t = threadIdx.x;
    const float v = ((sh[0][t] + sh[1][t]) + sh[2][t]) + sh[3][t];
    float* o;
    if (e < nW) {
      const int r = e & 3, lane = (e >> 2) & 63, tt = e >> 8;
      const int nj = tt % a.npw[l], mi = (tt / a.npw[l]) % a.mpw[l], wg = tt / (a.npw[l] * a.mpw[l]);
      const int ng = wg % a.ngrp[l], mg = wg / a.ngrp[l];
      const int co = 16 * (mg * a.mpw[l] + mi) + 4 * (lane >> 4) + r;
      const int tap = 16 * (a.ileave[l] ? nj * a.ngrp[l] + ng : ng * a.npw[l] + nj) + (lane & 15);
      o = a.gw[l][p] + (long)co * a.taps[l] + tap;
    } else {
      o = a.gb[l][p] + (e - nW);
    }
    *o = a.accumulate ? *o + v : v;
  }
}

struct DgArgs {
  const void* dz[EBW_MAXP];
  const __bf16* yin[EBW_MAXP];
  const uint4* wpk[EBW_MAXP];
  __bf16* dx[EBW_MAXP];
  int n[EBW_MAXP];
  int wpp;
};
struct PkArgs {
  const float* w[EBW_MAXP];
  uint4* out[EBW_MAXP];
};

template <class L>
__global__ __launch_bounds__(256) void ebw_pack_kernel(PkArgs a) {
  const int idx = blockIdx.x * 256 + threadIdx.x;
  if (idx >= L::NCOMBO * L::KS * 64) return;
  const int lane = idx & 63, ks = (idx >> 6) % L::KS, combo = (idx >> 6) / L::KS;
  const int cls = combo / L::NTI, nt = combo % L::NTI, py = cls / L::S, px = cls % L::S;
  const int tp = ks / (L::CO / 32), hf = ks % (L::CO / 32), ta = tp / L::KB, tb = tp % L::KB;
  const int ky = py + L::S * ta, kx = px + L::S * tb, ci = 16 * nt + (lane & 15), co0 = 32 * hf + 8 * (lane >> 4);
  const float* w = a.w[blockIdx.y];
  uint32_t v[4];
#pragma unroll
  for (int e = 0; e < 4; e++)
    v[e] = pack2(w[(((co0 + 2 * e) * L::KH + ky) * L::KW + kx) * L::CI + ci],
                 w[(((co0 + 2 * e + 1) * L::KH + ky) * L::KW + kx) * L::CI + ci]);
  a.out[blockIdx.y][idx] = make_uint4(v[0], v[1], v[2], v[3]);
}

template <class LA, class LB>
__global__ __launch_bounds__(256) void ebw_pack2_kernel(PkArgs a, PkArgs b) {
  constexpr int BA = (LA::NCOMBO * LA::KS * 64 + 255) / 256;
  const bool first = (int)blockIdx.x < BA;
  const int idx = (first ? blockIdx.x : blockIdx.x - BA) * 256 + threadIdx.x;
  auto body = [&](auto tag, const PkArgs& k) {
    using L = decltype(tag);
    if (idx >= L::NCOMBO * L::KS * 64) return;
    const int lane = idx & 63, ks = (idx >> 6) % L::KS, combo = (idx >> 6) / L::KS;
    const int cls = combo / L::NTI, nt = combo % L::NTI, py = cls / L::S, px = cls % L::S;
    const int tp = ks / (L::CO / 32), hf = ks % (L::CO / 32), ta = tp / L::KB, tb = tp % L::KB;
    const int ky = py + L::S * ta, kx = px + L::S * tb, ci = 16 * nt + (lane & 15), co0 = 32 * hf + 8 * (lane >> 4);
    const float* w = k.w[blockIdx.y];
    uint32_t v[4];
#pragma unroll
    for (int e = 0; e < 4; e++)
      v[e] = pack2(w[(((co0 + 2 * e) * L::KH + ky) * L::KW + kx) * L::CI + ci],
                   w[(((co0 + 2 * e + 1) * L::KH + ky) * L::KW + kx) * L::CI + ci]);
    k.out[blockIdx.y][idx] = make_uint4(v[0], v[1], v[2], v[3]);
  };
  if (first) body(LA{}, a); else body(LB{}, b);
}

template <class L>
constexpr int dgrad_mask_bytes() { return (L::IH * L::IW * L::CI / 8 + 15) / 16 * 16; }
template <class L>
constexpr int dgrad_nbuf() { return (size_t)2 * L::R * L::C * L::PP * 2 + 2 * dgrad_mask_bytes<L>() <= 160 * 1024 ? 2 : 1; }
template <class L>
constexpr size_t dgrad_lds_bytes() { return (size_t)dgrad_nbuf<L>() * (L::R * L::C * L::PP * 2 + dgrad_mask_bytes<L>()); }

template <class L, class DzT>
__global__ __launch_bounds__(NT) void ebw_dgrad_kernel(DgArgs a) {
  constexpr int MPARTS = NW / L::NCOMBO, MTW = (L::MTC + MPARTS - 1) / MPARTS;
  static_assert(NW % L::NCOMBO == 0, "wave tiling");
  constexpr int BUF = L::R * L::C * L::PP, NB = dgrad_nbuf<L>();
  constexpr int NCG = L::CO / 8, NCH = L::OH * L::OW * NCG, CPT = (NCH + NT - 1) / NT;
  extern __shared__ __attribute__((aligned(16))) unsigned char smem[];
  __bf16* dzh = reinterpret_cast<__bf16*>(smem);
  constexpr int MKB = dgrad_mask_bytes<L>(), NYC = L::IH * L::IW * L::CI / 8, CPY = (NYC + NT - 1) / NT;
  static_assert(L::CI % 8 == 0, "mask bytes hold 8 channels of one pixel");
  unsigned char* mkb = smem + (size_t)NB * BUF * 2;
  const int tid = threadIdx.x, lane = tid & 63, w = tid >> 6, i = lane & 15, g = lane >> 4;
  const int p = blockIdx.x / a.wpp, j0 = blockIdx.x - p * a.wpp;
  const int n_img = a.n[p];
  for (int e = tid; e < NB * BUF / 2; e += NT) reinterpret_cast<uint32_t*>(dzh)[e] = 0u;
  const int combo = w % L::NCOMBO, mpart = w / L::NCOMBO, cls = combo / L::NTI, nt = combo % L::NTI;
  const int py = cls / L::S, px = cls % L::S;
  bf16x8 Bf[L::KS];
#pragma unroll
  for (int ks = 0; ks < L::KS; ks++) {
    const uint4 t = a.wpk[p][(combo * L::KS + ks) * 64 + lane];
    Bf[ks] = __builtin_bit_cast(bf16x8, t);
  }
  int abase[MTW];
#pragma unroll
  for (int t = 0; t < MTW; t++) {
    int m = 16 * (mpart + t * MPARTS) + i;
    m = m < L::PH * L::PW ? m : L::PH * L::PW - 1;
    const int Y = m / L::PW, X = m - Y * L::PW;
    abase[t] = (Y * L::C + X) * L::PP + 8 * g;
  }
  int oidx[MTW];
#pragma unroll
  for (int t = 0; t < MTW; t++) {
    const int m = 16 * (mpart + t * MPARTS) + i, Y = m / L::PW, X = m - Y * L::PW;
    const int y = L::S * Y + py, x = L::S * X + px;
    oidx[t] = (m < L::PH * L::PW && y < L::IH && x < L::IW) ? (y * L::IW + x) * L::CI + 16 * nt + 4 * g : -1;
  }
  const DzT* dz = reinterpret_cast<const DzT*>(a.dz[p]);
  const __bf16* yin = a.yin[p];
  __bf16* dx = a.dx[p];
  bf16x8 pre[CPT];
  uint4 ypre[CPY];
  auto fetch = [&](int img) {
#pragma unroll
    for (int r = 0; r < CPT; r++) {
      const int c = tid + r * NT;
      if (c < NCH) pre[r] = load8v(dz + ((long)img * L::OH * L::OW + c / NCG) * L::CO + 8 * (c % NCG));
    }
#pragma unroll
    for (int r = 0; r < CPY; r++) {
      const int c = tid + r * NT;
      ypre[r] = *reinterpret_cast<const uint4*>(yin + (long)img * L::IH * L::IW * L::CI + 8 * (c < NYC ? c : NYC - 1));
    }
  };
  auto put = [&](__bf16* buf, unsigned char* mb) {
#pragma unroll
    for (int r = 0; r < CPY; r++) {
      const int c = tid + r * NT;
      if (c < NYC) {
        const uint32_t d[4] = {ypre[r].x, ypre[r].y, ypre[r].z, ypre[r].w};
        unsigned b = 0;
#pragma unroll
        for (int j = 0; j < 4; j++) {
          b |= ((((d[j] & 0xffffu) - 1u) & 0xffffu) < 0x7fffu ? 1u : 0u) << (2 * j);
          b |= ((((d[j] >> 16) - 1u) & 0xffffu) < 0x7fffu ? 1u : 0u) << (2 * j + 1);
        }
        mb[c] = (unsigned char)b;
      }
    }
#pragma unroll
    for (int r = 0; r < CPT; r++) {
      const int c = tid + r * NT;
      if (c < NCH) {
        const int pix = c / NCG, cg = c - pix * NCG, oy = pix / L::OW, ox = pix - oy * L::OW;
        *reinterpret_cast<bf16x8*>(buf + ((oy + L::HA) * L::C + ox + L::HB) * L::PP + 8 * cg) = pre[r];
      }
    }
  };
  __syncthreads();
  if (j0 < n_img) { fetch(j0); put(dzh, mkb); }
  __syncthreads();
  int k = 0;
  for (int img = j0; img < n_img; img += a.wpp, k ^= (NB - 1)) {
    const int nxt = img + a.wpp;
    if (nxt < n_img) fetch(nxt);
    const __bf16* buf = dzh + k * BUF;
    const unsigned char* mb = mkb + k * MKB;
    const long ibase = (long)img * L::IH * L::IW * L::CI;
#pragma unroll
    for (int t = 0; t < MTW; t++) {
      const int mt = mpart + t * MPARTS;
      if (mt >= L::MTC) break;
      f32x4 acc = {0.f, 0.f, 0.f, 0.f};
#pragma unroll
      for (int ks = 0; ks < L::KS; ks++) {
        const int tp = ks / (L::CO / 32), hf = ks % (L::CO / 32), ta = tp / L::KB, tb = tp % L::KB;
        const bf16x8 A = *reinterpret_cast<const bf16x8*>(buf + abase[t] + ((L::HA - ta) * L::C + L::HB - tb) * L::PP + 32 * hf);
        acc = __builtin_amdgcn_mfma_f32_16x16x32_bf16(Bf[ks], A, acc, 0, 0, 0);
      }
      if (oidx[t] >= 0) {
        const unsigned bits = (unsigned)mb[oidx[t] >> 3] >> (oidx[t] & 7);
        *reinterpret_cast<bf16x4*>(dx + ibase + oidx[t]) =
            bf16x4{(__bf16)((bits & 1) ? acc[0] : 0.f), (__bf16)((bits & 2) ? acc[1] : 0.f),
                   (__bf16)((bits & 4) ? acc[2] : 0.f), (__bf16)((bits & 8) ? acc[3] : 0.f)};
      }
    }
    if constexpr (NB == 2) {
      if (nxt < n_img) put(dzh + (k ^ 1) * BUF, mkb + (k ^ 1) * MKB);
      __syncthreads();
    } else {
      __syncthreads();
      if (nxt < n_img) put(dzh, mkb);
      __syncthreads();
    }
  }
}


struct L3Args {
  const float* y3[EBW_MAXP];
  const float* temp[EBW_MAXP];
  const float* sa[EBW_MAXP];
  const float* d_sa[EBW_MAXP];
  const __bf16* y2[EBW_MAXP];
  const uint4* wpk[EBW_MAXP];
  __bf16* dz2[EBW_MAXP];
  float* dtp[EBW_MAXP];
  float* slab;
  int n[EBW_MAXP];
  int wpp;
};
#ifdef L3_STAMPS
__device__ unsigned long long l3_st[16];
extern "C" int tacorl_l3_stamps_read(unsigned long long* out) {
  return hipMemcpyFromSymbol(out, HIP_SYMBOL(l3_st), sizeof(l3_st)) == hipSuccess ? 0 : -1;
}
#define L3_ST(i) do { if (tid == 64 * w && blockIdx.x == 0 && (w == 0 || w == ND3)) { const unsigned long long t_ = clock64(); st[i] += t_ - tl; tl = t_; } } while (0)
#else
#define L3_ST(i) do { } while (0)
#endif
constexpr int NT3 = 512, NW3 = NT3 / 64, ND3 = 4;
struct L3Tile { static constexpr int MGRP = 1, NGRP = 4, KGRP = 1; };
template <class L>
struct L3Geo {
  using TG = TrGeo<L>;
  static constexpr int P3 = L::OH * L::OW, K3 = (P3 + NW3 - 1) / NW3;
  static constexpr int HALO = L::R * L::C * L::PP;
  static constexpr int CIP = TG::CIP, Y2E = (L::IH * L::IW * CIP + 7) / 8 * 8;
  static constexpr int KS = (P3 + 31) / 32;
  static constexpr int Z2E = L::IH * L::IW * L::CI;
  static constexpr int MPW = L::MT / L3Tile::MGRP, NPW = L::NTL / L3Tile::NGRP;
  static constexpr size_t lds_bytes = ((size_t)HALO + 2 * Y2E + 2 * Z2E) * 2 + 2 * NW3 * 64 * 4 + 64;
  static_assert(L::S == 1 && L::CI == 64 && L::CO == 64 && L::NCOMBO == ND3, "conv3 of the LMPVisionEncoder");
  static constexpr bool ok = K3 <= 8 && lds_bytes <= 160 * 1024;
};

template <class L>
__global__ __launch_bounds__(NT3) void ebw_l3_kernel(L3Args a) {
  using G = L3Geo<L>;
  using TG = TrGeo<L>;
  using T = L3Tile;
  static_assert(T::MGRP * T::NGRP * T::KGRP == NW3 - ND3, "wgrad waves");
  static_assert(G::ok, "geometry not supported by the fused conv3 backward");
  extern __shared__ __attribute__((aligned(16))) unsigned char smem[];
  __bf16* dzh = reinterpret_cast<__bf16*>(smem);
  __bf16* y2s = dzh + G::HALO;
  __bf16* z2s = y2s + 2 * G::Y2E;
  float* shm = reinterpret_cast<float*>(z2s + 2 * G::Z2E);
  float* shs = shm + NW3 * 64;
  float* shd = shs + NW3 * 64;
  const int tid = threadIdx.x, lane = tid & 63, g = lane >> 4, l16 = lane & 15, q = l16 >> 2, pc = l16 & 3;
  const int w = __builtin_amdgcn_readfirstlane(tid >> 6);
  const int p = blockIdx.x / a.wpp, j0 = blockIdx.x - p * a.wpp;
  const int n_img = a.n[p];
  for (int e = tid; e < G::HALO / 8; e += NT3) reinterpret_cast<uint4*>(dzh)[e] = make_uint4(0u, 0u, 0u, 0u);
  const float it = 1.0f / a.temp[p][0];
  const float* y3 = a.y3[p];
  const __bf16* y2 = a.y2[p];
  constexpr int ICH = L::IH * L::IW * (L::CI / 8), ICPT = (ICH + NT3 - 1) / NT3;
  auto run = [&](auto role_tag) {
    constexpr int ROLE = decltype(role_tag)::value;
    float vn[G::K3];
    f32x2 gn, fn;
    bf16x8 ipre[ICPT];
    auto fetch3 = [&](int img) {
#pragma unroll
      for (int k = 0; k < G::K3; k++) {
        const int i = w + NW3 * k;
        vn[k] = y3[((long)img * G::P3 + (i < G::P3 ? i : G::P3 - 1)) * 64 + lane];
      }
      gn = *reinterpret_cast<const f32x2*>(a.d_sa[p] + (long)img * 128 + 2 * lane);
      fn = *reinterpret_cast<const f32x2*>(a.sa[p] + (long)img * 128 + 2 * lane);
    };
    auto fetch = [&](int img) {
#pragma unroll
      for (int r = 0; r < ICPT; r++) {
        const int c = tid + r * NT3;
        ipre[r] = *reinterpret_cast<const bf16x8*>(y2 + (long)img * L::IH * L::IW * L::CI + 8 * (c < ICH ? c : ICH - 1));
      }
    };
    auto put = [&](__bf16* buf) {
#pragma unroll
      for (int r = 0; r < ICPT; r++) {
        const int c = tid + r * NT3;
        if (c < ICH) *reinterpret_cast<bf16x8*>(buf + (c / (L::CI / 8)) * G::CIP + 8 * (c % (L::CI / 8))) = ipre[r];
      }
    };
    constexpr int ZCH = G::Z2E / 8, ZCPT = (ZCH + NT3 - 1) / NT3;
    auto flush = [&](int img, const __bf16* zb) {
#pragma unroll
      for (int r = 0; r < ZCPT; r++) {
        const int c = tid + r * NT3;
        if (c < ZCH) *reinterpret_cast<bf16x8*>(a.dz2[p] + (long)img * G::Z2E + 8 * c) = *reinterpret_cast<const bf16x8*>(zb + 8 * c);
      }
    };
    constexpr int MT = L::MTC, TG3 = 2, NGRP3 = (MT + TG3 - 1) / TG3;
    bf16x8 Bf[ROLE == 0 ? L::KS : 1];
    int abase[ROLE == 0 ? MT : 1];
    int obase = 0;
    if constexpr (ROLE == 0) {
      const int nt = w;
#pragma unroll
      for (int ks = 0; ks < L::KS; ks++) Bf[ks] = __builtin_bit_cast(bf16x8, a.wpk[p][(nt * L::KS + ks) * 64 + lane]);
#pragma unroll
      for (int t = 0; t < MT; t++) {
        const int m0 = 16 * t + l16;
        const int m = m0 < L::PH * L::PW ? m0 : L::PH * L::PW - 1;
        const int Y = m / L::PW, X = m - Y * L::PW;
        abase[t] = (Y * L::C + X) * L::PP + 8 * g;
      }
      obase = l16 * L::CI + 16 * nt + 4 * g;
    }
    static_assert(L::CI / 16 == T::NGRP, "one tap per n-tile round");
    const int wv = w - ND3, ng = wv % T::NGRP, mg = (wv / T::NGRP) % T::MGRP;
    const int coff = 16 * ng + 4 * pc;
    int zr0[ROLE == 1 ? G::KS : 1], zr1[ROLE == 1 ? G::KS : 1], ir0[ROLE == 1 ? G::KS : 1], ir1[ROLE == 1 ? G::KS : 1];
    f32x4 acc[ROLE == 1 ? G::MPW : 1][ROLE == 1 ? G::NPW : 1], bacc[ROLE == 1 ? G::MPW : 1];
    bf16x8 ones;
    if constexpr (ROLE == 1) {
#pragma unroll
      for (int s = 0; s < G::KS; s++) {
        const int P0 = 32 * s + 4 * g + q, P1 = P0 + 16;
        const int Q0 = P0 < G::P3 ? P0 : G::P3 - 1, Q1 = P1 < G::P3 ? P1 : G::P3 - 1;
        zr0[s] = P0 < G::P3 ? ((P0 / L::OW + L::HA) * L::C + P0 % L::OW + L::HB) * L::PP : 0;
        zr1[s] = P1 < G::P3 ? ((P1 / L::OW + L::HA) * L::C + P1 % L::OW + L::HB) * L::PP : 0;
        ir0[s] = ((Q0 / L::OW) * L::IW + Q0 % L::OW) * G::CIP;
        ir1[s] = ((Q1 / L::OW) * L::IW + Q1 % L::OW) * G::CIP;
      }
#pragma unroll
      for (int i = 0; i < G::MPW; i++) {
        bacc[i] = f32x4{0.f, 0.f, 0.f, 0.f};
#pragma unroll
        for (int j = 0; j < G::NPW; j++) acc[i][j] = f32x4{0.f, 0.f, 0.f, 0.f};
      }
#pragma unroll
      for (int j = 0; j < 8; j++) ones[j] = (__bf16)1.0f;
    }
    float dt = 0.f;
#ifdef L3_STAMPS
    unsigned long long st[6] = {0, 0, 0, 0, 0, 0}, tl = clock64();
    const unsigned long long w0 = wall_clock64(), c0 = tl;
#endif
    __syncthreads();
    if (j0 < n_img) { fetch(j0); fetch3(j0); put(y2s); }
    __syncthreads();
    int kb = 0;
    L3_ST(0);
    for (int img = j0; img < n_img; img += a.wpp, kb ^= 1) {
      const int nxt = img + a.wpp;
      int wl = w;
      asm volatile("" : "+s"(wl));
      float v[G::K3];
#pragma unroll
      for (int k = 0; k < G::K3; k++) v[k] = vn[k];
      const float gx = gn[0], gy = gn[1], dot = gn[0] * fn[0] + gn[1] * fn[1];
      asm volatile("" : : "v"(gx), "v"(gy), "v"(dot) : "memory");
#pragma unroll
      for (int k = 0; k < G::K3; k++) asm volatile("" : : "v"(v[k]) : "memory");
      if (nxt < n_img) { fetch(nxt); fetch3(nxt); }
      const __bf16* yb = y2s + kb * G::Y2E;
      float mx = -INFINITY;
#pragma unroll
      for (int k = 0; k < G::K3; k++) {
        v[k] *= it;
        if (wl + NW3 * k < G::P3) mx = fmaxf(mx, v[k]);
      }
      float se = 0.f;
#pragma unroll
      for (int k = 0; k < G::K3; k++) se += (wl + NW3 * k < G::P3) ? __expf(v[k] - mx) : 0.f;
      shm[wl * 64 + lane] = mx;
      shs[wl * 64 + lane] = se;
      __syncthreads();
      {
        float mw[NW3], sw[NW3];
#pragma unroll
        for (int ww = 0; ww < NW3; ww++) { mw[ww] = shm[ww * 64 + lane]; sw[ww] = shs[ww * 64 + lane]; }
        __builtin_amdgcn_sched_barrier(0);
#pragma unroll
        for (int ww = 0; ww < NW3; ww++) mx = fmaxf(mx, mw[ww]);
        se = 0.f;
#pragma unroll
        for (int ww = 0; ww < NW3; ww++) se += sw[ww] * __expf(mw[ww] - mx);
      }
      const float rse = 1.0f / se;
#pragma unroll
      for (int k = 0; k < G::K3; k++) {
        const int i = wl + NW3 * k;
        if (i < G::P3) {
          const int iy = i / L::OW;
          const float pr = __expf(v[k] - mx) * rse;
          const float ds = pr * (gx * (float)(i - iy * L::OW) + gy * (float)iy - dot);
          dt -= ds * v[k] * it;
          dzh[((iy + L::HA) * L::C + (i - iy * L::OW) + L::HB) * L::PP + lane] = (__bf16)(v[k] != 0.f ? ds * it : 0.f);
        }
      }
      L3_ST(1);
      if (img != j0) flush(img - a.wpp, z2s + (kb ^ 1) * G::Z2E);
      __syncthreads();
      L3_ST(2);
      if constexpr (ROLE == 0) {
        __bf16* zw = z2s + kb * G::Z2E;
#pragma unroll
        for (int tg = 0; tg < NGRP3; tg++) {
          f32x4 o[TG3];
#pragma unroll
          for (int u = 0; u < TG3; u++) o[u] = f32x4{0.f, 0.f, 0.f, 0.f};
          constexpr int HK = L::KS / 2;
          static_assert(L::KS % 2 == 0, "fragment steps in two halves");
          auto aoff = [&](int ks) {
            const int tp = ks / (L::CO / 32), hf = ks % (L::CO / 32), ta = tp / L::KB, tb = tp % L::KB;
            return ((L::HA - ta) * L::C + L::HB - tb) * L::PP + 32 * hf;
          };
          bf16x8 A[TG3][HK];
#pragma unroll
          for (int ks = 0; ks < HK; ks++)
#pragma unroll
            for (int u = 0; u < TG3; u++)
              A[u][ks] = *reinterpret_cast<const bf16x8*>(dzh + abase[tg * TG3 + u < MT ? tg * TG3 + u : MT - 1] + aoff(ks));
          __builtin_amdgcn_sched_barrier(0);
#pragma unroll
          for (int ks = 0; ks < L::KS; ks++) {
#pragma unroll
            for (int u = 0; u < TG3; u++) {
              o[u] = __builtin_amdgcn_mfma_f32_16x16x32_bf16(Bf[ks], A[u][ks % HK], o[u], 0, 0, 0);
              if (ks + HK < L::KS)
                A[u][ks % HK] = *reinterpret_cast<const bf16x8*>(dzh + abase[tg * TG3 + u < MT ? tg * TG3 + u : MT - 1] + aoff(ks + HK));
            }
            __builtin_amdgcn_sched_barrier(0);
          }
#pragma unroll
          for (int u = 0; u < TG3; u++) {
            const int t = tg * TG3 + u;
            if (t >= MT) continue;
            const int oi = obase + t * 16 * L::CI;
            if (oi < L::PH * L::PW * L::CI) {
              const uint2 yv = *reinterpret_cast<const uint2*>(yb + (oi >> 6) * G::CIP + (oi & 63));
              const bool m0 = (((yv.x & 0xffffu) - 1u) & 0xffffu) < 0x7fffu, m1 = (((yv.x >> 16) - 1u) & 0xffffu) < 0x7fffu;
              const bool m2 = (((yv.y & 0xffffu) - 1u) & 0xffffu) < 0x7fffu, m3 = (((yv.y >> 16) - 1u) & 0xffffu) < 0x7fffu;
              *reinterpret_cast<bf16x4*>(zw + oi) =
                  bf16x4{(__bf16)(m0 ? o[u][0] : 0.f), (__bf16)(m1 ? o[u][1] : 0.f), (__bf16)(m2 ? o[u][2] : 0.f),
                         (__bf16)(m3 ? o[u][3] : 0.f)};
            }
          }
        }
      } else {
#pragma unroll
        for (int s = 0; s < G::KS; s++) {
          constexpr int JB = (G::NPW + 2) / 3;
          bf16x8 A[G::MPW], B[JB];
#pragma unroll
          for (int i = 0; i < G::MPW; i++) {
            const int col = 16 * (mg * G::MPW + i) + 4 * pc;
            A[i] = tr_frag(dzh + zr0[s] + col, dzh + zr1[s] + col);
          }
#pragma unroll
          for (int jb = 0; jb < G::NPW; jb += JB) {
#pragma unroll
            for (int j = jb; j < jb + JB && j < G::NPW; j++) {
              const int tofs = ((j / L::KW) * L::IW + j % L::KW) * G::CIP;
              B[j - jb] = tr_frag(yb + ir0[s] + coff + tofs, yb + ir1[s] + coff + tofs);
            }
            __builtin_amdgcn_sched_barrier(0);
#pragma unroll
            for (int j = jb; j < jb + JB && j < G::NPW; j++)
#pragma unroll
              for (int i = 0; i < G::MPW; i++) acc[i][j] = __builtin_amdgcn_mfma_f32_16x16x32_bf16(A[i], B[j - jb], acc[i][j], 0, 0, 0);
            __builtin_amdgcn_sched_barrier(0);
          }
          if (ng == 0) {
#pragma unroll
            for (int i = 0; i < G::MPW; i++) bacc[i] = __builtin_amdgcn_mfma_f32_16x16x32_bf16(A[i], ones, bacc[i], 0, 0, 0);
          }
        }
      }
      L3_ST(3);
      if (nxt < n_img) put(y2s + (kb ^ 1) * G::Y2E);
      __syncthreads();
      L3_ST(4);
    }
    if (j0 < n_img) flush(j0 + ((n_img - 1 - j0) / a.wpp) * a.wpp, z2s + (kb ^ 1) * G::Z2E);
    if constexpr (ROLE == 1) {
      float* sl = a.slab + (long)blockIdx.x * TG::SLABF;
#pragma unroll
      for (int i = 0; i < G::MPW; i++)
#pragma unroll
        for (int j = 0; j < G::NPW; j++)
          *reinterpret_cast<f32x4*>(sl + (((wv * G::MPW + i) * G::NPW + j) * 64 + lane) * 4) = acc[i][j];
      if (ng == 0 && l16 == 0) {
#pragma unroll
        for (int i = 0; i < G::MPW; i++)
#pragma unroll
          for (int r = 0; r < 4; r++) sl[L::CO * L::TAPS + 16 * (mg * G::MPW + i) + 4 * g + r] = bacc[i][r];
      }
    }
    dt = wave_sum(dt);
    if (lane == 0) shd[w] = dt;
    __syncthreads();
    if (tid == 0 && j0 < n_img) {
      float sum = 0.f;
#pragma unroll
      for (int ww = 0; ww < NW3; ww++) sum += shd[ww];
      a.dtp[p][j0] = sum;
    }
#ifdef L3_STAMPS
    L3_ST(5);
    if (tid == 64 * w && blockIdx.x == 0 && (w == 0 || w == ND3)) {
      const int o = w == 0 ? 0 : 8;
      for (int i = 0; i < 6; i++) l3_st[o + i] = st[i];
      l3_st[o + 6] = clock64() - c0; l3_st[o + 7] = wall_clock64() - w0;
    }
#endif
  };
  if (w < ND3) run(std::integral_constant<int, 0>{});
  else run(std::integral_constant<int, 1>{});
}

inline size_t al256(size_t x) { return (x + 255) & ~(size_t)255; }
inline int cdivi(long a, long b) { return (int)((a + b - 1) / b); }
constexpr int cdivi_c(int a, int b) { return (a + b - 1) / b; }

struct WsPlan {
  size_t wpk2[EBW_MAXP], wpk3[EBW_MAXP], dz2[EBW_MAXP], dz1[EBW_MAXP], slab1, slab2, slab3, total;
  int wpp;
};
template <class G>
WsPlan plan(int nprob, const int* n) {
  WsPlan w{};
  long maxn = 1;
  for (int p = 0; p < nprob; p++) maxn = n[p] > maxn ? n[p] : maxn;
  const int per = 256 / nprob > 1 ? 256 / nprob : 1;
  w.wpp = (int)(per < maxn ? per : maxn);
  size_t off = 0;
  for (int p = 0; p < nprob; p++) {
    w.wpk2[p] = off; off += al256((size_t)G::L2::NCOMBO * G::L2::KS * 64 * 16);
    w.wpk3[p] = off; off += al256((size_t)G::L3::NCOMBO * G::L3::KS * 64 * 16);
    w.dz2[p] = off; off += al256((size_t)n[p] * G::L3::IH * G::L3::IW * 64 * 2);
    w.dz1[p] = off; off += al256((size_t)n[p] * G::L2::IH * G::L2::IW * 32 * 2);
  }
  const size_t nwg = (size_t)nprob * w.wpp;
  w.slab1 = off; off += al256(nwg * TrGeo<typename G::L1>::SLABF * 4);
  w.slab2 = off; off += al256(nwg * TrGeo<typename G::L2>::SLABF * 4);
  w.slab3 = off; off += al256(nwg * TrGeo<typename G::L3>::SLABF * 4);
  w.total = off;
  return w;
}

template <class K>
int set_lds(K kern, size_t bytes) {
  return hipFuncSetAttribute(reinterpret_cast<const void*>(kern), hipFuncAttributeMaxDynamicSharedMemorySize, (int)bytes) ==
                 hipSuccess ? 0 : -1;
}

template <class L, class InT, class DzT>
int launch_wgrad_tr(const WgArgs& a, int nwg, hipStream_t st) {
  auto kern = ebw_wgrad_tr_kernel<L, InT, DzT>;
  constexpr size_t lds = TrGeo<L>::lds_bytes;
  static int once = set_lds(kern, lds);
  if (once) return TACORL_ELAUNCH;
  hipLaunchKernelGGL(kern, dim3(nwg), dim3(NT), lds, st, a);
  return TACORL_OK;
}
template <class L, class DzT>
int launch_dgrad(const DgArgs& a, int nwg, hipStream_t st) {
  auto kern = ebw_dgrad_kernel<L, DzT>;
  constexpr size_t lds = dgrad_lds_bytes<L>();
  static int once = set_lds(kern, lds);
  if (once) return TACORL_ELAUNCH;
  hipLaunchKernelGGL(kern, dim3(nwg), dim3(NT), lds, st, a);
  return TACORL_OK;
}
template <class L>
int launch_l3(const L3Args& a, int nwg, hipStream_t st) {
  auto kern = ebw_l3_kernel<L>;
  constexpr size_t lds = L3Geo<L>::lds_bytes;
  static int once = set_lds(kern, lds);
  if (once) return TACORL_ELAUNCH;
  hipLaunchKernelGGL(kern, dim3(nwg), dim3(NT3), lds, st, a);
  return TACORL_OK;
}
template <class G>
int run(int nprob, const EbwProblem* pr, int accumulate, void* ws, size_t ws_bytes, hipStream_t st, int mode, int parts) {
  using L1 = typename G::L1; using L2 = typename G::L2; using L3 = typename G::L3;
  int n[EBW_MAXP];
  for (int p = 0; p < nprob; p++) n[p] = pr[p].n;
  const WsPlan w = plan<G>(nprob, n);
  if (ws_bytes < w.total) return TACORL_ENOMEM;
  unsigned char* base = (unsigned char*)ws;
  const int nwg = nprob * w.wpp;
  PkArgs k2{}, k3{};
  for (int p = 0; p < nprob; p++) {
    k2.w[p] = pr[p].w2; k2.out[p] = (uint4*)(base + w.wpk2[p]);
    k3.w[p] = pr[p].w3; k3.out[p] = (uint4*)(base + w.wpk3[p]);
  }
  if (mode != 2) {
    hipLaunchKernelGGL((ebw_pack2_kernel<L2, L3>), dim3(cdivi(L2::NCOMBO * L2::KS * 64, 256) + cdivi(L3::NCOMBO * L3::KS * 64, 256), nprob),
                       dim3(256), 0, st, k2, k3);
  }
  if (mode == 1) return hipGetLastError() == hipSuccess ? TACORL_OK : TACORL_ELAUNCH;
  DgArgs d3{}, d2{};
  WgArgs g3{}, g2{}, g1{};
  float *gw1[EBW_MAXP], *gb1[EBW_MAXP], *gw2[EBW_MAXP], *gb2[EBW_MAXP], *gw3[EBW_MAXP], *gb3[EBW_MAXP];
  for (int p = 0; p < nprob; p++) {
    __bf16* dz2 = (__bf16*)(base + w.dz2[p]);
    __bf16* dz1 = (__bf16*)(base + w.dz1[p]);
    d3.dz[p] = pr[p].dz3; d3.yin[p] = (const __bf16*)pr[p].y2; d3.wpk[p] = k3.out[p]; d3.dx[p] = dz2; d3.n[p] = n[p];
    d2.dz[p] = dz2; d2.yin[p] = (const __bf16*)pr[p].y1; d2.wpk[p] = k2.out[p]; d2.dx[p] = dz1; d2.n[p] = n[p];
    g3.in[p] = pr[p].y2; g3.dz[p] = pr[p].dz3; g3.n[p] = n[p];
    g2.in[p] = pr[p].y1; g2.dz[p] = dz2; g2.n[p] = n[p];
    g1.in[p] = pr[p].img; g1.dz[p] = dz1; g1.n[p] = n[p];
    gw1[p] = pr[p].g_w1; gb1[p] = pr[p].g_b1; gw2[p] = pr[p].g_w2; gb2[p] = pr[p].g_b2;
    gw3[p] = pr[p].g_w3; gb3[p] = pr[p].g_b3;
  }
  d3.wpp = d2.wpp = g3.wpp = g2.wpp = g1.wpp = w.wpp;
  constexpr int dg2 = 2;
  long maxn = 1;
  for (int p = 0; p < nprob; p++) maxn = n[p] > maxn ? n[p] : maxn;
  auto per_cu = [](size_t lds) { return (size_t)dg2 * lds <= 160 * 1024 ? dg2 : 1; };
  const int k3w = per_cu(dgrad_lds_bytes<L3>()), k2w = per_cu(dgrad_lds_bytes<L2>());
  d3.wpp = (int)((long)k3w * w.wpp < maxn ? (long)k3w * w.wpp : maxn);
  d2.wpp = (int)((long)k2w * w.wpp < maxn ? (long)k2w * w.wpp : maxn);
  g1.slab = (float*)(base + w.slab1); g2.slab = (float*)(base + w.slab2); g3.slab = (float*)(base + w.slab3);
  int rc;
  const bool fused3 = (parts & EBW_FUSED3) != 0;
  if (fused3 && (parts & EBW_ALL) != EBW_ALL) return TACORL_EINVAL;
  {
    if (fused3) {
      L3Args f{};
      for (int p = 0; p < nprob; p++) {
        f.y3[p] = pr[p].y3; f.temp[p] = pr[p].temp; f.sa[p] = pr[p].sa; f.d_sa[p] = pr[p].d_sa;
        f.y2[p] = (const __bf16*)pr[p].y2; f.wpk[p] = k3.out[p]; f.dz2[p] = (__bf16*)(base + w.dz2[p]);
        f.dtp[p] = pr[p].dtp; f.n[p] = n[p];
      }
      f.slab = g3.slab; f.wpp = w.wpp;
      if constexpr (L3Geo<L3>::ok) {
        if ((rc = launch_l3<L3>(f, nwg, st))) return rc;
      } else {
        return TACORL_EINVAL;
      }
    } else {
      if ((parts & EBW_DGRAD3) && (rc = launch_dgrad<L3, float>(d3, nprob * d3.wpp, st))) return rc;
      if ((parts & EBW_WGRAD3) && (rc = launch_wgrad_tr<L3, __bf16, float>(g3, nwg, st))) return rc;
    }
    if ((parts & EBW_DGRAD2) && (rc = launch_dgrad<L2, __bf16>(d2, nprob * d2.wpp, st))) return rc;
    if ((parts & EBW_WGRAD2) && (rc = launch_wgrad_tr<L2, __bf16, __bf16>(g2, nwg, st))) return rc;
    if ((parts & EBW_WGRAD1) && (rc = launch_wgrad_tr<L1, __bf16, __bf16>(g1, nwg, st))) return rc;
    if (!(parts & EBW_REDUCE)) return hipGetLastError() == hipSuccess ? TACORL_OK : TACORL_ELAUNCH;
    RdTrArgs t{};
    t.slab[0] = g1.slab; t.slab[1] = g2.slab; t.slab[2] = g3.slab;
    auto fill = [&](int l, auto geo, int co, int taps) {
      using TG = decltype(geo);
      t.co[l] = co; t.taps[l] = taps; t.mpw[l] = TG::MPW; t.npw[l] = TG::NPW; t.mgrp[l] = TG::T::MGRP;
      t.ngrp[l] = TG::T::NGRP; t.kgrp[l] = TG::T::KGRP; t.slabf[l] = TG::SLABF;
    };
    fill(0, TrGeo<L1>{}, L1::CO, L1::TAPS); fill(1, TrGeo<L2>{}, L2::CO, L2::TAPS); fill(2, TrGeo<L3>{}, L3::CO, L3::TAPS);
    t.wpp = w.wpp; t.accumulate = accumulate;
    for (int p = 0; p < nprob; p++) {
      t.gw[0][p] = gw1[p]; t.gb[0][p] = gb1[p]; t.gw[1][p] = gw2[p]; t.gb[1][p] = gb2[p];
      t.gw[2][p] = gw3[p]; t.gb[2][p] = gb3[p];
    }
    constexpr int maxper_t = cmax(L1::SLABF, cmax(L2::SLABF, L3::SLABF));
    static_assert(cdivi_c(maxper_t, 64) - 1 > cdivi_c(L1::SLABF, 64), "the temperature block must lie beyond conv1's elements");
    if (fused3) {
      for (int p = 0; p < nprob; p++) { t.dtp[p] = pr[p].dtp; t.g_temp[p] = pr[p].g_temp; t.ndt[p] = n[p] < w.wpp ? n[p] : w.wpp; }
      t.ileave[2] = 1; t.mpw[2] = L3Geo<L3>::MPW; t.npw[2] = L3Geo<L3>::NPW; t.mgrp[2] = L3Tile::MGRP; t.ngrp[2] = L3Tile::NGRP;
    }
    hipLaunchKernelGGL(ebw_reduce_tr_kernel, dim3(cdivi(maxper_t, 64), 3 * nprob), dim3(256), 0, st, t);
    return hipGetLastError() == hipSuccess ? TACORL_OK : TACORL_ELAUNCH;
  }
}

}

#define EBW_GEOMS(X) X(84, 84) X(64, 64) X(44, 60) X(128, 128) X(150, 200)

bool ebw_fused3_supported(int H, int W) {
#define X(h, w) if (H == h && W == w) return L3Geo<Geo<h, w>::L3>::ok;
  EBW_GEOMS(X)
#undef X
  return false;
}
bool ebw_supported(int H, int W) {
#define X(h, w) if (H == h && W == w) return true;
  EBW_GEOMS(X)
#undef X
  return false;
}
size_t ebw_ws_bytes(int nprob, const int* n_img, int H, int W) {
  if (nprob < 1 || nprob > EBW_MAXP) return 0;
#define X(h, w) if (H == h && W == w) return plan<Geo<h, w>>(nprob, n_img).total;
  EBW_GEOMS(X)
#undef X
  return 0;
}
int ebw_conv_backward(int nprob, const EbwProblem* pr, int H, int W, int accumulate, void* ws, size_t ws_bytes,
                      hipStream_t st, int mode, int parts) {
  if (nprob < 1 || nprob > EBW_MAXP) return TACORL_EINVAL;
#define X(h, w) if (H == h && W == w) return run<Geo<h, w>>(nprob, pr, accumulate, ws, ws_bytes, st, mode, parts);
  EBW_GEOMS(X)
#undef X
  return TACORL_EINVAL;
}
```

Measured before the change: 1232 grad-steps/s.

## Balance encoder backward work across workgroups with a contiguous image line split

The encoder conv backward kernels used to assign a fixed number of workgroups per problem, each striding over that problem's images. Now all images of all problems form one global line that is cut into contiguous, near-equal ranges per workgroup. A workgroup may cross a problem boundary, in which case it flushes its partial slab and switches pointers. The reduce kernel now sums variable per-problem slab counts. The aim is to remove load imbalance and idle workgroups when problems differ in image count. The cost is extra slab partials, boundary-handling logic, and an optional max_workgroups knob that defaults to 0 on existing paths.

```diff
diff --git a/include/tacorl_hip.h b/include/tacorl_hip.h
--- a/include/tacorl_hip.h
+++ b/include/tacorl_hip.h
@@ -119,6 +119,12 @@
                              const float* const* act, const float* const* d_out,
                              float* const* grads, const int* n_img, int H, int W, int accumulate,
                              void* ws, size_t ws_bytes, tacorl_stream_t stream);
+int tacorl_encoder_bwd_fused_wg(int nprob, const void* const* img, const float* const* params,
+                                const float* const* act, const float* const* d_out,
+                                float* const* grads, const int* n_img, int H, int W, int accumulate,
+                                int max_workgroups, void* ws, size_t ws_bytes, tacorl_stream_t stream);
+int tacorl_encoder_bwd_fused_plan(int nprob, const int* n_img, int H, int W, int max_workgroups, int* out,
+                                  int* ranges, size_t* ws_bytes);
 int tacorl_encoder_bwd_fused_pack(int nprob, const float* const* params, const int* n_img, int H, int W,
                                   void* ws, size_t ws_bytes, tacorl_stream_t stream);
 int tacorl_encoder_bwd_fused_head(int nprob, const float* const* params, const float* const* act,
diff --git a/tacorl_amd/_lib.py b/tacorl_amd/_lib.py
--- a/tacorl_amd/_lib.py
+++ b/tacorl_amd/_lib.py
@@ -109,6 +109,8 @@
     "tacorl_encoder_fwd_fused_wg": (_i, [_i, _p, _p, _p, _p, _p, _p, _i, _i, _i, _p]),
     "tacorl_encoder_bwd_fused_ws_bytes": (_sz, [_i, _p, _i, _i]),
     "tacorl_encoder_bwd_fused": (_i, [_i, _p, _p, _p, _p, _p, _p, _i, _i, _i, _p, _sz, _p]),
+    "tacorl_encoder_bwd_fused_wg": (_i, [_i, _p, _p, _p, _p, _p, _p, _i, _i, _i, _i, _p, _sz, _p]),
+    "tacorl_encoder_bwd_fused_plan": (_i, [_i, _p, _i, _i, _i, _p, _p, _p]),
     "tacorl_encoder_bwd_fused_pack": (_i, [_i, _p, _p, _i, _i, _p, _sz, _p]),
     "tacorl_encoder_bwd_fused_head": (_i, [_i, _p, _p, _p, _p, _i, _i, _i, _p, _sz, _p]),
     "tacorl_encoder_bwd_fused_fc_wgrad": (_i, [_i, _p, _p, _p, _p, _i, _i, _i, _p, _sz, _p]),
diff --git a/tacorl_amd/csrc/dense_ops.hip b/tacorl_amd/csrc/dense_ops.hip
--- a/tacorl_amd/csrc/dense_ops.hip
+++ b/tacorl_amd/csrc/dense_ops.hip
@@ -764,7 +764,7 @@
   long maxn;
 };
 static const int kFcActs[2] = {ACT_RELU, ACT_NONE};
-static bool enc_bwd_plan(int nprob, const int* n_img, int H, int W, EncBwdPlan& pl) {
+static bool enc_bwd_plan(int nprob, const int* n_img, int H, int W, EncBwdPlan& pl, int max_wg = 0) {
   if (!enc_dims(H, W, pl.d) || !ebw_supported(H, W) || nprob < 1 || nprob > EBW_MAXP) return false;
   tacorl_encoder_param_layout(pl.po);
   long tot = 0;
@@ -783,7 +783,7 @@
   pl.slab_bytes = enc_fc_slab_bytes(nprob, pl.maxn);
   b += pl.slab_bytes;
   pl.conv_off = b;
-  pl.total = b + ebw_ws_bytes(nprob, n_img, H, W);
+  pl.total = b + ebw_ws_bytes(nprob, n_img, H, W, max_wg);
   return true;
 }
 extern "C" size_t tacorl_encoder_bwd_fused_ws_bytes(int nprob, const int* n_img, int H, int W) {
@@ -889,12 +889,21 @@
   return tacorl_encoder_bwd_fused_conv_parts(nprob, img, params, act, grads, n_img, H, W, accumulate, prepacked, 127, ws,
                                              ws_bytes, stream);
 }
+static int enc_bwd_conv_parts(int nprob, const void* const* img, const float* const* params, const float* const* act,
+                              float* const* grads, const int* n_img, int H, int W, int accumulate, int prepacked,
+                              int parts, int max_wg, void* ws, size_t ws_bytes, tacorl_stream_t stream);
 extern "C" int tacorl_encoder_bwd_fused_conv_parts(int nprob, const void* const* img, const float* const* params,
                                                    const float* const* act, float* const* grads, const int* n_img, int H,
                                                    int W, int accumulate, int prepacked, int parts, void* ws,
                                                    size_t ws_bytes, tacorl_stream_t stream) {
+  return enc_bwd_conv_parts(nprob, img, params, act, grads, n_img, H, W, accumulate, prepacked, parts, 0, ws, ws_bytes, stream);
+}
+static int enc_bwd_conv_parts(int nprob, const void* const* img, const float* const* params, const float* const* act,
+                              float* const* grads, const int* n_img, int H, int W, int accumulate, int prepacked,
+                              int parts, int max_wg, void* ws, size_t ws_bytes, tacorl_stream_t stream) {
   hipStream_t st = (hipStream_t)stream;
   EncBwdPlan pl;
+  if (max_wg < 0) FAIL(TACORL_EINVAL, "encoder_bwd_fused_conv: max_workgroups %d", max_wg);
   if (!enc_bwd_plan(nprob, n_img, H, W, pl)) FAIL(TACORL_EINVAL, "encoder_bwd_fused_conv: geometry %dx%d / nprob %d", H, W, nprob);
   if (ws_bytes < pl.total) FAIL(TACORL_ENOMEM, "encoder_bwd_fused_conv: workspace too small");
   if (pl.d.c3.OH * pl.d.c3.OW > 4 * SAB_MAXI_HUGE) FAIL(TACORL_EINVAL, "encoder_bwd_fused: conv3 output too large");
@@ -926,7 +935,7 @@
   if (!(parts & EBW_ALL)) return hipGetLastError() == hipSuccess ? TACORL_OK : TACORL_ELAUNCH;
   if ((parts & EBW_ALL) != EBW_ALL && !prepacked) FAIL(TACORL_EINVAL, "encoder_bwd_fused_conv_parts: partial calls need prepacked fragments");
   const int rc = ebw_conv_backward(nprob, pr, H, W, accumulate, (unsigned char*)ws + pl.conv_off, pl.total - pl.conv_off, st, prepacked ? 2 : 0,
-                                   (parts & EBW_ALL) | (fused3 ? EBW_FUSED3 : 0));
+                                   (parts & EBW_ALL) | (fused3 ? EBW_FUSED3 : 0), max_wg);
   if (rc != TACORL_OK) FAIL(rc, "encoder_bwd_fused_conv: conv backward launch failed (%d)", rc);
   return hipGetLastError() == hipSuccess ? TACORL_OK : TACORL_ELAUNCH;
 }
@@ -938,6 +947,23 @@
   if (rc == TACORL_OK) rc = tacorl_encoder_bwd_fused_fc_wgrad(nprob, act, d_out, grads, n_img, H, W, accumulate, ws, ws_bytes, stream);
   if (rc == TACORL_OK) rc = tacorl_encoder_bwd_fused_conv(nprob, img, params, act, grads, n_img, H, W, accumulate, 0, ws, ws_bytes, stream);
   return rc;
+}
+extern "C" int tacorl_encoder_bwd_fused_wg(int nprob, const void* const* img, const float* const* params,
+                                           const float* const* act, const float* const* d_out, float* const* grads,
+                                           const int* n_img, int H, int W, int accumulate, int max_workgroups, void* ws,
+                                           size_t ws_bytes, tacorl_stream_t stream) {
+  int rc = tacorl_encoder_bwd_fused_head(nprob, params, act, d_out, n_img, H, W, 0, ws, ws_bytes, stream);
+  if (rc == TACORL_OK) rc = tacorl_encoder_bwd_fused_fc_wgrad(nprob, act, d_out, grads, n_img, H, W, accumulate, ws, ws_bytes, stream);
+  if (rc == TACORL_OK) rc = enc_bwd_conv_parts(nprob, img, params, act, grads, n_img, H, W, accumulate, 0, 127, max_workgroups, ws, ws_bytes, stream);
+  return rc;
+}
+extern "C" int tacorl_encoder_bwd_fused_plan(int nprob, const int* n_img, int H, int W, int max_workgroups, int* out,
+                                             int* ranges, size_t* ws_bytes) {
+  EncBwdPlan pl;
+  if (max_workgroups < 0 || !out || !enc_bwd_plan(nprob, n_img, H, W, pl, max_workgroups))
+    FAIL(TACORL_EINVAL, "encoder_bwd_fused_plan: geometry %dx%d / nprob %d / max_workgroups %d", H, W, nprob, max_workgroups);
+  if (ws_bytes) *ws_bytes = pl.total;
+  return ebw_plan_query(nprob, n_img, H, W, max_workgroups, out, ranges);
 }
 
 extern "C" long tacorl_mlp_param_layout(int L, const int* dims, long* w_off, long* b_off) {
diff --git a/tacorl_amd/csrc/enc_bwd_fused.h b/tacorl_amd/csrc/enc_bwd_fused.h
--- a/tacorl_amd/csrc/enc_bwd_fused.h
+++ b/tacorl_amd/csrc/enc_bwd_fused.h
@@ -18,9 +18,12 @@
 };
 
 bool ebw_supported(int H, int W);
-size_t ebw_ws_bytes(int nprob, const int* n_img, int H, int W);
+size_t ebw_ws_bytes(int nprob, const int* n_img, int H, int W, int max_wg = 0);
+#define EBW_PLAN_STRIDE (2 + EBW_MAXP)
+#define EBW_PLAN_RANGES 513
+int ebw_plan_query(int nprob, const int* n_img, int H, int W, int max_wg, int* out, int* ranges);
 enum { EBW_DGRAD3 = 2, EBW_WGRAD3 = 4, EBW_DGRAD2 = 8, EBW_WGRAD2 = 16, EBW_WGRAD1 = 32, EBW_REDUCE = 64, EBW_ALL = 126,
        EBW_FUSED3 = 128 };
 bool ebw_fused3_supported(int H, int W);
 int ebw_conv_backward(int nprob, const EbwProblem* pr, int H, int W, int accumulate, void* ws, size_t ws_bytes,
-                      hipStream_t st, int mode, int parts = EBW_ALL);
+                      hipStream_t st, int mode, int parts = EBW_ALL, int max_wg = 0);
diff --git a/tacorl_amd/csrc/encoder_bwd_fused.hip b/tacorl_amd/csrc/encoder_bwd_fused.hip
--- a/tacorl_amd/csrc/encoder_bwd_fused.hip
+++ b/tacorl_amd/csrc/encoder_bwd_fused.hip
@@ -71,12 +71,35 @@
 }
 __device__ __forceinline__ bf16x8 load8v(const __bf16* p) { return *reinterpret_cast<const bf16x8*>(p); }
 
+struct ImgLine {
+  int start[EBW_MAXP + 1];
+  int fwg[EBW_MAXP];
+  int sbase[EBW_MAXP];
+  int q, r, nwg;
+};
+__host__ __device__ __forceinline__ int line_lo(const ImgLine& ln, int b) {
+  const int lo = b * ln.q + (int)((unsigned)(b * ln.r) / (unsigned)ln.nwg);
+#ifdef __HIP_DEVICE_COMPILE__
+  return __builtin_amdgcn_readfirstlane(lo);
+#else
+  return lo;
+#endif
+}
+__device__ __forceinline__ int at_use(int v) {
+  asm volatile("" : "+v"(v));
+  return v;
+}
+__device__ __forceinline__ int line_find(const ImgLine& ln, int gi) {
+  int p = 0;
+  while (ln.start[p + 1] <= gi) p++;
+  return p;
+}
+
 struct WgArgs {
   const void* in[EBW_MAXP];
   const void* dz[EBW_MAXP];
-  int n[EBW_MAXP];
+  ImgLine ln;
   float* slab;
-  int wpp;
 };
 
 typedef __bf16 bf16x4v __attribute__((ext_vector_type(4)));
@@ -127,8 +150,7 @@
   extern __shared__ __attribute__((aligned(16))) unsigned char smem[];
   __bf16* lds = reinterpret_cast<__bf16*>(smem);
   const int tid = threadIdx.x, lane = tid & 63, w = tid >> 6, g = lane >> 4, l16 = lane & 15, q = l16 >> 2, pc = l16 & 3;
-  const int p = blockIdx.x / a.wpp, j0 = blockIdx.x - p * a.wpp;
-  const int n_img = a.n[p];
+  const int lo = line_lo(a.ln, blockIdx.x), hi = line_lo(a.ln, blockIdx.x + 1);
   const int ng = w % T::NGRP, mg = (w / T::NGRP) % T::MGRP, kg = w / (T::NGRP * T::MGRP);
   for (int e = tid; e < (int)(G::lds_bytes / 4); e += NT) reinterpret_cast<uint32_t*>(lds)[e] = 0u;
   int toff[G::NPW];
@@ -145,17 +167,20 @@
     }
   }
   f32x4 acc[G::MPW][G::NPW], bacc[G::MPW];
-#pragma unroll
-  for (int i = 0; i < G::MPW; i++) {
-    bacc[i] = f32x4{0.f, 0.f, 0.f, 0.f};
-#pragma unroll
-    for (int j = 0; j < G::NPW; j++) acc[i][j] = f32x4{0.f, 0.f, 0.f, 0.f};
-  }
+  auto clear_acc = [&]() {
+#pragma unroll
+    for (int i = 0; i < G::MPW; i++) {
+      bacc[i] = f32x4{0.f, 0.f, 0.f, 0.f};
+#pragma unroll
+      for (int j = 0; j < G::NPW; j++) acc[i][j] = f32x4{0.f, 0.f, 0.f, 0.f};
+    }
+  };
   bf16x8 ones;
 #pragma unroll
   for (int j = 0; j < 8; j++) ones[j] = (__bf16)1.0f;
-  const InT* in = reinterpret_cast<const InT*>(a.in[p]);
-  const DzT* dz = reinterpret_cast<const DzT*>(a.dz[p]);
+  const InT* in = nullptr;
+  const DzT* dz = nullptr;
+  auto fetch_from = [&](int pp) { in = reinterpret_cast<const InT*>(a.in[pp]); dz = reinterpret_cast<const DzT*>(a.dz[pp]); };
   constexpr int DCG = L::CO / 8, DCH = G::NPIX * DCG, DCPT = (DCH + NT - 1) / NT;
   constexpr int ICH = G::BROWS * L::IW * L::CI / 8, ICPT = (ICH + NT - 1) / NT;
   static_assert((G::BROWS * L::IW * L::CI) % 8 == 0 && (G::NBAND == 1 || (G::BR * L::S * L::IW * L::CI) % 8 == 0), "image / band bytes");
@@ -231,44 +256,73 @@
       for (int s = 0; s < G::KS; s++) kstep(s);
     }
   };
+  auto store_slab = [&](int pp) {
+    float* sl = a.slab + (long)(a.ln.sbase[pp] + (int)blockIdx.x - a.ln.fwg[pp]) * G::SLABF;
+    float* sw = sl + at_use((w * G::TPW * 64 + lane) * 4);
+#pragma unroll
+    for (int i = 0; i < G::MPW; i++)
+#pragma unroll
+      for (int j = 0; j < G::NPW; j++)
+        *reinterpret_cast<f32x4*>(sw + (i * G::NPW + j) * 64 * 4) = acc[i][j];
+    if (ng == 0 && l16 == 0) {
+#pragma unroll
+      for (int i = 0; i < G::MPW; i++)
+#pragma unroll
+        for (int r = 0; r < 4; r++)
+          sl[T::KGRP * L::CO * L::TAPS + kg * L::CO + 16 * (mg * G::MPW + i) + 4 * g + r] = bacc[i][r];
+    }
+  };
+  int p = line_find(a.ln, lo), gi = lo;
+  fetch_from(p);
   __syncthreads();
   if constexpr (G::NBUF == 2) {
-    if (j0 < n_img) { fetch(j0, 0); put(lds, 0); }
+    fetch(lo - a.ln.start[p], 0);
+    put(lds, 0);
     __syncthreads();
     int k = 0;
-    for (int img = j0; img < n_img; img += a.wpp, k ^= 1) {
-      const int nxt = img + a.wpp;
-      if (nxt < n_img) fetch(nxt, 0);
-      compute(lds + k * G::BUF_EL, 0);
-      if (nxt < n_img) put(lds + (k ^ 1) * G::BUF_EL, 0);
-      __syncthreads();
+    while (true) {
+      const int pend = a.ln.start[p + 1] < hi ? a.ln.start[p + 1] : hi;
+      int np = p;
+      clear_acc();
+      for (; gi < pend; gi++, k ^= 1) {
+        const int nxt = gi + 1;
+        if (nxt < hi) {
+          if (nxt == pend) { np = line_find(a.ln, nxt); fetch_from(np); }
+          fetch(nxt - a.ln.start[np], 0);
+        }
+        compute(lds + k * G::BUF_EL, 0);
+        if (nxt < hi) put(lds + (k ^ 1) * G::BUF_EL, 0);
+        __syncthreads();
+      }
+      store_slab(p);
+      if (pend == hi) break;
+      p = np;
     }
   } else {
-    if (j0 < n_img) fetch(j0, 0);
-    for (int img = j0; img < n_img; img += a.wpp) {
+    fetch(lo - a.ln.start[p], 0);
+    while (true) {
+      const int pend = a.ln.start[p + 1] < hi ? a.ln.start[p + 1] : hi;
+      int np = p;
+      clear_acc();
+      for (; gi < pend; gi++) {
+        const int nxt = gi + 1, img = gi - a.ln.start[p];
 #pragma unroll 1
-      for (int b = 0; b < G::NBAND; b++) {
-        __syncthreads();
-        put(lds, b);
-        __syncthreads();
-        if (b + 1 < G::NBAND) fetch(img, b + 1);
-        else if (img + a.wpp < n_img) fetch(img + a.wpp, 0);
-        compute(lds, b);
-      }
-    }
-  }
-  float* sl = a.slab + (long)blockIdx.x * G::SLABF;
-#pragma unroll
-  for (int i = 0; i < G::MPW; i++)
-#pragma unroll
-    for (int j = 0; j < G::NPW; j++)
-      *reinterpret_cast<f32x4*>(sl + (((w * G::MPW + i) * G::NPW + j) * 64 + lane) * 4) = acc[i][j];
-  if (ng == 0 && l16 == 0) {
-#pragma unroll
-    for (int i = 0; i < G::MPW; i++)
-#pragma unroll
-      for (int r = 0; r < 4; r++)
-        sl[T::KGRP * L::CO * L::TAPS + kg * L::CO + 16 * (mg * G::MPW + i) + 4 * g + r] = bacc[i][r];
+        for (int b = 0; b < G::NBAND; b++) {
+          __syncthreads();
+          put(lds, b);
+          __syncthreads();
+          if (b + 1 < G::NBAND) fetch(img, b + 1);
+          else if (nxt < hi) {
+            if (nxt == pend) { np = line_find(a.ln, nxt); fetch_from(np); }
+            fetch(nxt - a.ln.start[np], 0);
+          }
+          compute(lds, b);
+        }
+      }
+      store_slab(p);
+      if (pend == hi) break;
+      p = np;
+    }
   }
 }
 
@@ -278,7 +332,7 @@
   float* gb[3][EBW_MAXP];
   int co[3], taps[3], mpw[3], npw[3], mgrp[3], ngrp[3], kgrp[3], slabf[3];
   int ileave[3];
-  int wpp, accumulate;
+  int sbase[EBW_MAXP], cnt[EBW_MAXP], accumulate;
   const float* dtp[EBW_MAXP];
   float* g_temp[EBW_MAXP];
   int ndt[EBW_MAXP];
@@ -303,11 +357,12 @@
   if (blockIdx.x * 64 >= per) return;
   float sum = 0.f;
   if (e < per) {
-    const float* s0 = a.slab[l] + (long)p * a.wpp * a.slabf[l];
+    const float* s0 = a.slab[l] + (long)a.sbase[p] * a.slabf[l];
+    const int cnt = a.cnt[p];
     for (int kg = 0; kg < KG; kg++) {
       const float* s = s0 + (e < nW ? (long)kg * nW + e : (long)KG * nW + kg * a.co[l] + (e - nW));
 #pragma unroll 8
-      for (int k = kq; k < a.wpp; k += 4) sum += s[(long)k * a.slabf[l]];
+      for (int k = kq; k < cnt; k += 4) sum += s[(long)k * a.slabf[l]];
     }
   }
   sh[kq][threadIdx.x & 63] = sum;
@@ -335,8 +390,7 @@
   const __bf16* yin[EBW_MAXP];
   const uint4* wpk[EBW_MAXP];
   __bf16* dx[EBW_MAXP];
-  int n[EBW_MAXP];
-  int wpp;
+  ImgLine ln;
 };
 struct PkArgs {
   const float* w[EBW_MAXP];
@@ -402,17 +456,21 @@
   static_assert(L::CI % 8 == 0, "mask bytes hold 8 channels of one pixel");
   unsigned char* mkb = smem + (size_t)NB * BUF * 2;
   const int tid = threadIdx.x, lane = tid & 63, w = tid >> 6, i = lane & 15, g = lane >> 4;
-  const int p = blockIdx.x / a.wpp, j0 = blockIdx.x - p * a.wpp;
-  const int n_img = a.n[p];
+  const int lo = line_lo(a.ln, blockIdx.x), hi = line_lo(a.ln, blockIdx.x + 1);
+  int p = line_find(a.ln, lo), gi = lo;
   for (int e = tid; e < NB * BUF / 2; e += NT) reinterpret_cast<uint32_t*>(dzh)[e] = 0u;
   const int combo = w % L::NCOMBO, mpart = w / L::NCOMBO, cls = combo / L::NTI, nt = combo % L::NTI;
   const int py = cls / L::S, px = cls % L::S;
   bf16x8 Bf[L::KS];
-#pragma unroll
-  for (int ks = 0; ks < L::KS; ks++) {
-    const uint4 t = a.wpk[p][(combo * L::KS + ks) * 64 + lane];
-    Bf[ks] = __builtin_bit_cast(bf16x8, t);
-  }
+  auto load_frags = [&](int pp) {
+    const uint4* src = a.wpk[pp] + at_use(combo * L::KS * 64 + lane);
+#pragma unroll
+    for (int ks = 0; ks < L::KS; ks++) {
+      const uint4 t = src[ks * 64];
+      Bf[ks] = __builtin_bit_cast(bf16x8, t);
+    }
+  };
+  load_frags(p);
   int abase[MTW];
 #pragma unroll
   for (int t = 0; t < MTW; t++) {
@@ -470,41 +528,57 @@
     }
   };
   __syncthreads();
-  if (j0 < n_img) { fetch(j0); put(dzh, mkb); }
+  fetch(lo - a.ln.start[p]);
+  put(dzh, mkb);
   __syncthreads();
   int k = 0;
-  for (int img = j0; img < n_img; img += a.wpp, k ^= (NB - 1)) {
-    const int nxt = img + a.wpp;
-    if (nxt < n_img) fetch(nxt);
-    const __bf16* buf = dzh + k * BUF;
-    const unsigned char* mb = mkb + k * MKB;
-    const long ibase = (long)img * L::IH * L::IW * L::CI;
-#pragma unroll
-    for (int t = 0; t < MTW; t++) {
-      const int mt = mpart + t * MPARTS;
-      if (mt >= L::MTC) break;
-      f32x4 acc = {0.f, 0.f, 0.f, 0.f};
-#pragma unroll
-      for (int ks = 0; ks < L::KS; ks++) {
-        const int tp = ks / (L::CO / 32), hf = ks % (L::CO / 32), ta = tp / L::KB, tb = tp % L::KB;
-        const bf16x8 A = *reinterpret_cast<const bf16x8*>(buf + abase[t] + ((L::HA - ta) * L::C + L::HB - tb) * L::PP + 32 * hf);
-        acc = __builtin_amdgcn_mfma_f32_16x16x32_bf16(Bf[ks], A, acc, 0, 0, 0);
-      }
-      if (oidx[t] >= 0) {
-        const unsigned bits = (unsigned)mb[oidx[t] >> 3] >> (oidx[t] & 7);
-        *reinterpret_cast<bf16x4*>(dx + ibase + oidx[t]) =
-            bf16x4{(__bf16)((bits & 1) ? acc[0] : 0.f), (__bf16)((bits & 2) ? acc[1] : 0.f),
-                   (__bf16)((bits & 4) ? acc[2] : 0.f), (__bf16)((bits & 8) ? acc[3] : 0.f)};
-      }
-    }
-    if constexpr (NB == 2) {
-      if (nxt < n_img) put(dzh + (k ^ 1) * BUF, mkb + (k ^ 1) * MKB);
-      __syncthreads();
-    } else {
-      __syncthreads();
-      if (nxt < n_img) put(dzh, mkb);
-      __syncthreads();
-    }
+  while (true) {
+    const int pend = a.ln.start[p + 1] < hi ? a.ln.start[p + 1] : hi;
+    int np = p;
+    for (; gi < pend; gi++, k ^= (NB - 1)) {
+      const int nxt = gi + 1;
+      if (nxt < hi) {
+        if (nxt == pend) {
+          np = line_find(a.ln, nxt);
+          dz = reinterpret_cast<const DzT*>(a.dz[np]);
+          yin = a.yin[np];
+        }
+        fetch(nxt - a.ln.start[np]);
+      }
+      const __bf16* buf = dzh + k * BUF;
+      const unsigned char* mb = mkb + k * MKB;
+      const long ibase = (long)(gi - a.ln.start[p]) * L::IH * L::IW * L::CI;
+#pragma unroll
+      for (int t = 0; t < MTW; t++) {
+        const int mt = mpart + t * MPARTS;
+        if (mt >= L::MTC) break;
+        f32x4 acc = {0.f, 0.f, 0.f, 0.f};
+#pragma unroll
+        for (int ks = 0; ks < L::KS; ks++) {
+          const int tp = ks / (L::CO / 32), hf = ks % (L::CO / 32), ta = tp / L::KB, tb = tp % L::KB;
+          const bf16x8 A = *reinterpret_cast<const bf16x8*>(buf + abase[t] + ((L::HA - ta) * L::C + L::HB - tb) * L::PP + 32 * hf);
+          acc = __builtin_amdgcn_mfma_f32_16x16x32_bf16(Bf[ks], A, acc, 0, 0, 0);
+        }
+        if (oidx[t] >= 0) {
+          const unsigned bits = (unsigned)mb[oidx[t] >> 3] >> (oidx[t] & 7);
+          *reinterpret_cast<bf16x4*>(dx + ibase + oidx[t]) =
+              bf16x4{(__bf16)((bits & 1) ? acc[0] : 0.f), (__bf16)((bits & 2) ? acc[1] : 0.f),
+                     (__bf16)((bits & 4) ? acc[2] : 0.f), (__bf16)((bits & 8) ? acc[3] : 0.f)};
+        }
+      }
+      if constexpr (NB == 2) {
+        if (nxt < hi) put(dzh + (k ^ 1) * BUF, mkb + (k ^ 1) * MKB);
+        __syncthreads();
+      } else {
+        __syncthreads();
+        if (nxt < hi) put(dzh, mkb);
+        __syncthreads();
+      }
+    }
+    if (pend == hi) break;
+    p = np;
+    dx = a.dx[p];
+    load_frags(p);
   }
 }
 
@@ -519,8 +593,7 @@
   __bf16* dz2[EBW_MAXP];
   float* dtp[EBW_MAXP];
   float* slab;
-  int n[EBW_MAXP];
-  int wpp;
+  ImgLine ln;
 };
 #ifdef L3_STAMPS
 __device__ unsigned long long l3_st[16];
@@ -563,26 +636,27 @@
   float* shd = shs + NW3 * 64;
   const int tid = threadIdx.x, lane = tid & 63, g = lane >> 4, l16 = lane & 15, q = l16 >> 2, pc = l16 & 3;
   const int w = __builtin_amdgcn_readfirstlane(tid >> 6);
-  const int p = blockIdx.x / a.wpp, j0 = blockIdx.x - p * a.wpp;
-  const int n_img = a.n[p];
+  const int lo = line_lo(a.ln, blockIdx.x), hi = line_lo(a.ln, blockIdx.x + 1);
   for (int e = tid; e < G::HALO / 8; e += NT3) reinterpret_cast<uint4*>(dzh)[e] = make_uint4(0u, 0u, 0u, 0u);
-  const float it = 1.0f / a.temp[p][0];
-  const float* y3 = a.y3[p];
-  const __bf16* y2 = a.y2[p];
   constexpr int ICH = L::IH * L::IW * (L::CI / 8), ICPT = (ICH + NT3 - 1) / NT3;
   auto run = [&](auto role_tag) {
     constexpr int ROLE = decltype(role_tag)::value;
     float vn[G::K3];
     f32x2 gn, fn;
     bf16x8 ipre[ICPT];
+    int p = line_find(a.ln, lo), gi = lo;
+    const float *y3, *sa, *d_sa;
+    const __bf16* y2;
+    auto fetch_from = [&](int pp) { y3 = a.y3[pp]; y2 = a.y2[pp]; sa = a.sa[pp]; d_sa = a.d_sa[pp]; };
+    fetch_from(p);
     auto fetch3 = [&](int img) {
 #pragma unroll
       for (int k = 0; k < G::K3; k++) {
         const int i = w + NW3 * k;
         vn[k] = y3[((long)img * G::P3 + (i < G::P3 ? i : G::P3 - 1)) * 64 + lane];
       }
-      gn = *reinterpret_cast<const f32x2*>(a.d_sa[p] + (long)img * 128 + 2 * lane);
-      fn = *reinterpret_cast<const f32x2*>(a.sa[p] + (long)img * 128 + 2 * lane);
+      gn = *reinterpret_cast<const f32x2*>(d_sa + (long)img * 128 + 2 * lane);
+      fn = *reinterpret_cast<const f32x2*>(sa + (long)img * 128 + 2 * lane);
     };
     auto fetch = [&](int img) {
 #pragma unroll
@@ -599,21 +673,26 @@
       }
     };
     constexpr int ZCH = G::Z2E / 8, ZCPT = (ZCH + NT3 - 1) / NT3;
-    auto flush = [&](int img, const __bf16* zb) {
+    auto flush = [&](__bf16* dst, const __bf16* zb) {
 #pragma unroll
       for (int r = 0; r < ZCPT; r++) {
         const int c = tid + r * NT3;
-        if (c < ZCH) *reinterpret_cast<bf16x8*>(a.dz2[p] + (long)img * G::Z2E + 8 * c) = *reinterpret_cast<const bf16x8*>(zb + 8 * c);
+        if (c < ZCH) *reinterpret_cast<bf16x8*>(dst + 8 * c) = *reinterpret_cast<const bf16x8*>(zb + 8 * c);
       }
     };
     constexpr int MT = L::MTC, TG3 = 2, NGRP3 = (MT + TG3 - 1) / TG3;
     bf16x8 Bf[ROLE == 0 ? L::KS : 1];
     int abase[ROLE == 0 ? MT : 1];
     int obase = 0;
+    auto load_frags = [&](int pp) {
+      if constexpr (ROLE == 0) {
+        const uint4* src = a.wpk[pp] + w * L::KS * 64 + at_use(lane);
+#pragma unroll
+        for (int ks = 0; ks < L::KS; ks++) Bf[ks] = __builtin_bit_cast(bf16x8, src[ks * 64]);
+      }
+    };
     if constexpr (ROLE == 0) {
       const int nt = w;
-#pragma unroll
-      for (int ks = 0; ks < L::KS; ks++) Bf[ks] = __builtin_bit_cast(bf16x8, a.wpk[p][(nt * L::KS + ks) * 64 + lane]);
 #pragma unroll
       for (int t = 0; t < MT; t++) {
         const int m0 = 16 * t + l16;
@@ -624,8 +703,7 @@
       obase = l16 * L::CI + 16 * nt + 4 * g;
     }
     static_assert(L::CI / 16 == T::NGRP, "one tap per n-tile round");
-    const int wv = w - ND3, ng = wv % T::NGRP, mg = (wv / T::NGRP) % T::MGRP;
-    const int coff = 16 * ng + 4 * pc;
+    const int coff = 16 * ((w - ND3) % T::NGRP) + 4 * pc;
     int zr0[ROLE == 1 ? G::KS : 1], zr1[ROLE == 1 ? G::KS : 1], ir0[ROLE == 1 ? G::KS : 1], ir1[ROLE == 1 ? G::KS : 1];
     f32x4 acc[ROLE == 1 ? G::MPW : 1][ROLE == 1 ? G::NPW : 1], bacc[ROLE == 1 ? G::MPW : 1];
     bf16x8 ones;
@@ -640,180 +718,205 @@
         ir1[s] = ((Q1 / L::OW) * L::IW + Q1 % L::OW) * G::CIP;
       }
 #pragma unroll
-      for (int i = 0; i < G::MPW; i++) {
-        bacc[i] = f32x4{0.f, 0.f, 0.f, 0.f};
-#pragma unroll
-        for (int j = 0; j < G::NPW; j++) acc[i][j] = f32x4{0.f, 0.f, 0.f, 0.f};
-      }
-#pragma unroll
       for (int j = 0; j < 8; j++) ones[j] = (__bf16)1.0f;
     }
-    float dt = 0.f;
+    float dt;
 #ifdef L3_STAMPS
     unsigned long long st[6] = {0, 0, 0, 0, 0, 0}, tl = clock64();
     const unsigned long long w0 = wall_clock64(), c0 = tl;
 #endif
+    const int wv = w - ND3, ng = wv % T::NGRP, mg = (wv / T::NGRP) % T::MGRP;
+    auto segment_end = [&](int pp) {
+      const int slot = (int)blockIdx.x - a.ln.fwg[pp];
+      if constexpr (ROLE == 1) {
+        float* sl = a.slab + (long)(a.ln.sbase[pp] + slot) * TG::SLABF;
+        float* sw = sl + wv * G::MPW * G::NPW * 64 * 4 + at_use(lane * 4);
+#pragma unroll
+        for (int i = 0; i < G::MPW; i++)
+#pragma unroll
+          for (int j = 0; j < G::NPW; j++)
+            *reinterpret_cast<f32x4*>(sw + (i * G::NPW + j) * 64 * 4) = acc[i][j];
+        if (ng == 0 && l16 == 0) {
+#pragma unroll
+          for (int i = 0; i < G::MPW; i++)
+#pragma unroll
+            for (int r = 0; r < 4; r++) sl[L::CO * L::TAPS + 16 * (mg * G::MPW + i) + 4 * g + r] = bacc[i][r];
+        }
+      }
+      dt = wave_sum(dt);
+      if (lane == 0) shd[w] = dt;
+      __syncthreads();
+      if (tid == 0) {
+        float sum = 0.f;
+#pragma unroll
+        for (int ww = 0; ww < NW3; ww++) sum += shd[ww];
+        a.dtp[pp][slot] = sum;
+      }
+    };
     __syncthreads();
-    if (j0 < n_img) { fetch(j0); fetch3(j0); put(y2s); }
+    fetch(lo - a.ln.start[p]);
+    fetch3(lo - a.ln.start[p]);
+    put(y2s);
     __syncthreads();
     int kb = 0;
+    __bf16* zprev = nullptr;
     L3_ST(0);
-    for (int img = j0; img < n_img; img += a.wpp, kb ^= 1) {
-      const int nxt = img + a.wpp;
-      int wl = w;
-      asm volatile("" : "+s"(wl));
-      float v[G::K3];
-#pragma unroll
-      for (int k = 0; k < G::K3; k++) v[k] = vn[k];
-      const float gx = gn[0], gy = gn[1], dot = gn[0] * fn[0] + gn[1] * fn[1];
-      asm volatile("" : : "v"(gx), "v"(gy), "v"(dot) : "memory");
-#pragma unroll
-      for (int k = 0; k < G::K3; k++) asm volatile("" : : "v"(v[k]) : "memory");
-      if (nxt < n_img) { fetch(nxt); fetch3(nxt); }
-      const __bf16* yb = y2s + kb * G::Y2E;
-      float mx = -INFINITY;
-#pragma unroll
-      for (int k = 0; k < G::K3; k++) {
-        v[k] *= it;
-        if (wl + NW3 * k < G::P3) mx = fmaxf(mx, v[k]);
-      }
-      float se = 0.f;
-#pragma unroll
-      for (int k = 0; k < G::K3; k++) se += (wl + NW3 * k < G::P3) ? __expf(v[k] - mx) : 0.f;
-      shm[wl * 64 + lane] = mx;
-      shs[wl * 64 + lane] = se;
-      __syncthreads();
-      {
-        float mw[NW3], sw[NW3];
-#pragma unroll
-        for (int ww = 0; ww < NW3; ww++) { mw[ww] = shm[ww * 64 + lane]; sw[ww] = shs[ww * 64 + lane]; }
-        __builtin_amdgcn_sched_barrier(0);
-#pragma unroll
-        for (int ww = 0; ww < NW3; ww++) mx = fmaxf(mx, mw[ww]);
-        se = 0.f;
-#pragma unroll
-        for (int ww = 0; ww < NW3; ww++) se += sw[ww] * __expf(mw[ww] - mx);
-      }
-      const float rse = 1.0f / se;
-#pragma unroll
-      for (int k = 0; k < G::K3; k++) {
-        const int i = wl + NW3 * k;
-        if (i < G::P3) {
-          const int iy = i / L::OW;
-          const float pr = __expf(v[k] - mx) * rse;
-          const float ds = pr * (gx * (float)(i - iy * L::OW) + gy * (float)iy - dot);
-          dt -= ds * v[k] * it;
-          dzh[((iy + L::HA) * L::C + (i - iy * L::OW) + L::HB) * L::PP + lane] = (__bf16)(v[k] != 0.f ? ds * it : 0.f);
-        }
-      }
-      L3_ST(1);
-      if (img != j0) flush(img - a.wpp, z2s + (kb ^ 1) * G::Z2E);
-      __syncthreads();
-      L3_ST(2);
-      if constexpr (ROLE == 0) {
-        __bf16* zw = z2s + kb * G::Z2E;
-#pragma unroll
-        for (int tg = 0; tg < NGRP3; tg++) {
-          f32x4 o[TG3];
-#pragma unroll
-          for (int u = 0; u < TG3; u++) o[u] = f32x4{0.f, 0.f, 0.f, 0.f};
-          constexpr int HK = L::KS / 2;
-          static_assert(L::KS % 2 == 0, "fragment steps in two halves");
-          auto aoff = [&](int ks) {
-            const int tp = ks / (L::CO / 32), hf = ks % (L::CO / 32), ta = tp / L::KB, tb = tp % L::KB;
-            return ((L::HA - ta) * L::C + L::HB - tb) * L::PP + 32 * hf;
-          };
-          bf16x8 A[TG3][HK];
-#pragma unroll
-          for (int ks = 0; ks < HK; ks++)
-#pragma unroll
-            for (int u = 0; u < TG3; u++)
-              A[u][ks] = *reinterpret_cast<const bf16x8*>(dzh + abase[tg * TG3 + u < MT ? tg * TG3 + u : MT - 1] + aoff(ks));
+    while (true) {
+      const int pend = a.ln.start[p + 1] < hi ? a.ln.start[p + 1] : hi;
+      const float it = 1.0f / a.temp[p][0];
+      int np = p;
+      load_frags(p);
+      if constexpr (ROLE == 1) {
+#pragma unroll
+        for (int i = 0; i < G::MPW; i++) {
+          bacc[i] = f32x4{0.f, 0.f, 0.f, 0.f};
+#pragma unroll
+          for (int j = 0; j < G::NPW; j++) acc[i][j] = f32x4{0.f, 0.f, 0.f, 0.f};
+        }
+      }
+      dt = 0.f;
+      for (; gi < pend; gi++, kb ^= 1) {
+        const int nxt = gi + 1;
+        int wl = w;
+        asm volatile("" : "+s"(wl));
+        float v[G::K3];
+#pragma unroll
+        for (int k = 0; k < G::K3; k++) v[k] = vn[k];
+        const float gx = gn[0], gy = gn[1], dot = gn[0] * fn[0] + gn[1] * fn[1];
+        asm volatile("" : : "v"(gx), "v"(gy), "v"(dot) : "memory");
+#pragma unroll
+        for (int k = 0; k < G::K3; k++) asm volatile("" : : "v"(v[k]) : "memory");
+        if (nxt < hi) {
+          if (nxt == pend) { np = line_find(a.ln, nxt); fetch_from(np); }
+          fetch(nxt - a.ln.start[np]);
+          fetch3(nxt - a.ln.start[np]);
+        }
+        const __bf16* yb = y2s + kb * G::Y2E;
+        float mx = -INFINITY;
+#pragma unroll
+        for (int k = 0; k < G::K3; k++) {
+          v[k] *= it;
+          if (wl + NW3 * k < G::P3) mx = fmaxf(mx, v[k]);
+        }
+        float se = 0.f;
+#pragma unroll
+        for (int k = 0; k < G::K3; k++) se += (wl + NW3 * k < G::P3) ? __expf(v[k] - mx) : 0.f;
+        shm[wl * 64 + lane] = mx;
+        shs[wl * 64 + lane] = se;
+        __syncthreads();
+        {
+          float mw[NW3], sw[NW3];
+#pragma unroll
+          for (int ww = 0; ww < NW3; ww++) { mw[ww] = shm[ww * 64 + lane]; sw[ww] = shs[ww * 64 + lane]; }
           __builtin_amdgcn_sched_barrier(0);
 #pragma unroll
-          for (int ks = 0; ks < L::KS; ks++) {
+          for (int ww = 0; ww < NW3; ww++) mx = fmaxf(mx, mw[ww]);
+          se = 0.f;
+#pragma unroll
+          for (int ww = 0; ww < NW3; ww++) se += sw[ww] * __expf(mw[ww] - mx);
+        }
+        const float rse = 1.0f / se;
+#pragma unroll
+        for (int k = 0; k < G::K3; k++) {
+          const int i = wl + NW3 * k;
+          if (i < G::P3) {
+            const int iy = i / L::OW;
+            const float pr = __expf(v[k] - mx) * rse;
+            const float ds = pr * (gx * (float)(i - iy * L::OW) + gy * (float)iy - dot);
+            dt -= ds * v[k] * it;
+            dzh[((iy + L::HA) * L::C + (i - iy * L::OW) + L::HB) * L::PP + lane] = (__bf16)(v[k] != 0.f ? ds * it : 0.f);
+          }
+        }
+        L3_ST(1);
+        if (gi != lo) flush(zprev, z2s + (kb ^ 1) * G::Z2E);
+        __syncthreads();
+        L3_ST(2);
+        if constexpr (ROLE == 0) {
+          __bf16* zw = z2s + kb * G::Z2E;
+#pragma unroll
+          for (int tg = 0; tg < NGRP3; tg++) {
+            f32x4 o[TG3];
+#pragma unroll
+            for (int u = 0; u < TG3; u++) o[u] = f32x4{0.f, 0.f, 0.f, 0.f};
+            constexpr int HK = L::KS / 2;
+            static_assert(L::KS % 2 == 0, "fragment steps in two halves");
+            auto aoff = [&](int ks) {
+              const int tp = ks / (L::CO / 32), hf = ks % (L::CO / 32), ta = tp / L::KB, tb = tp % L::KB;
+              return ((L::HA - ta) * L::C + L::HB - tb) * L::PP + 32 * hf;
+            };
+            bf16x8 A[TG3][HK];
+#pragma unroll
+            for (int ks = 0; ks < HK; ks++)
+#pragma unroll
+              for (int u = 0; u < TG3; u++)
+                A[u][ks] = *reinterpret_cast<const bf16x8*>(dzh + abase[tg * TG3 + u < MT ? tg * TG3 + u : MT - 1] + aoff(ks));
+            __builtin_amdgcn_sched_barrier(0);
+#pragma unroll
+            for (int ks = 0; ks < L::KS; ks++) {
+#pragma unroll
+              for (int u = 0; u < TG3; u++) {
+                o[u] = __builtin_amdgcn_mfma_f32_16x16x32_bf16(Bf[ks], A[u][ks % HK], o[u], 0, 0, 0);
+                if (ks + HK < L::KS)
+                  A[u][ks % HK] = *reinterpret_cast<const bf16x8*>(dzh + abase[tg * TG3 + u < MT ? tg * TG3 + u : MT - 1] + aoff(ks + HK));
+              }
+              __builtin_amdgcn_sched_barrier(0);
+            }
 #pragma unroll
             for (int u = 0; u < TG3; u++) {
-              o[u] = __builtin_amdgcn_mfma_f32_16x16x32_bf16(Bf[ks], A[u][ks % HK], o[u], 0, 0, 0);
-              if (ks + HK < L::KS)
-                A[u][ks % HK] = *reinterpret_cast<const bf16x8*>(dzh + abase[tg * TG3 + u < MT ? tg * TG3 + u : MT - 1] + aoff(ks + HK));
-            }
-            __builtin_amdgcn_sched_barrier(0);
-          }
-#pragma unroll
-          for (int u = 0; u < TG3; u++) {
-            const int t = tg * TG3 + u;
-            if (t >= MT) continue;
-            const int oi = obase + t * 16 * L::CI;
-            if (oi < L::PH * L::PW * L::CI) {
-              const uint2 yv = *reinterpret_cast<const uint2*>(yb + (oi >> 6) * G::CIP + (oi & 63));
-              const bool m0 = (((yv.x & 0xffffu) - 1u) & 0xffffu) < 0x7fffu, m1 = (((yv.x >> 16) - 1u) & 0xffffu) < 0x7fffu;
-              const bool m2 = (((yv.y & 0xffffu) - 1u) & 0xffffu) < 0x7fffu, m3 = (((yv.y >> 16) - 1u) & 0xffffu) < 0x7fffu;
-              *reinterpret_cast<bf16x4*>(zw + oi) =
-                  bf16x4{(__bf16)(m0 ? o[u][0] : 0.f), (__bf16)(m1 ? o[u][1] : 0.f), (__bf16)(m2 ? o[u][2] : 0.f),
-                         (__bf16)(m3 ? o[u][3] : 0.f)};
+              const int t = tg * TG3 + u;
+              if (t >= MT) continue;
+              const int oi = obase + t * 16 * L::CI;
+              if (oi < L::PH * L::PW * L::CI) {
+                const uint2 yv = *reinterpret_cast<const uint2*>(yb + (oi >> 6) * G::CIP + (oi & 63));
+                const bool m0 = (((yv.x & 0xffffu) - 1u) & 0xffffu) < 0x7fffu, m1 = (((yv.x >> 16) - 1u) & 0xffffu) < 0x7fffu;
+                const bool m2 = (((yv.y & 0xffffu) - 1u) & 0xffffu) < 0x7fffu, m3 = (((yv.y >> 16) - 1u) & 0xffffu) < 0x7fffu;
+                *reinterpret_cast<bf16x4*>(zw + oi) =
+                    bf16x4{(__bf16)(m0 ? o[u][0] : 0.f), (__bf16)(m1 ? o[u][1] : 0.f), (__bf16)(m2 ? o[u][2] : 0.f),
+                           (__bf16)(m3 ? o[u][3] : 0.f)};
+              }
             }
           }
-        }
-      } else {
-#pragma unroll
-        for (int s = 0; s < G::KS; s++) {
-          constexpr int JB = (G::NPW + 2) / 3;
-          bf16x8 A[G::MPW], B[JB];
-#pragma unroll
-          for (int i = 0; i < G::MPW; i++) {
-            const int col = 16 * (mg * G::MPW + i) + 4 * pc;
-            A[i] = tr_frag(dzh + zr0[s] + col, dzh + zr1[s] + col);
+        } else {
+#pragma unroll
+          for (int s = 0; s < G::KS; s++) {
+            constexpr int JB = (G::NPW + 2) / 3;
+            bf16x8 A[G::MPW], B[JB];
+#pragma unroll
+            for (int i = 0; i < G::MPW; i++) {
+              const int col = 16 * (mg * G::MPW + i) + 4 * pc;
+              A[i] = tr_frag(dzh + zr0[s] + col, dzh + zr1[s] + col);
+            }
+#pragma unroll
+            for (int jb = 0; jb < G::NPW; jb += JB) {
+#pragma unroll
+              for (int j = jb; j < jb + JB && j < G::NPW; j++) {
+                const int tofs = ((j / L::KW) * L::IW + j % L::KW) * G::CIP;
+                B[j - jb] = tr_frag(yb + ir0[s] + coff + tofs, yb + ir1[s] + coff + tofs);
+              }
+              __builtin_amdgcn_sched_barrier(0);
+#pragma unroll
+              for (int j = jb; j < jb + JB && j < G::NPW; j++)
+#pragma unroll
+                for (int i = 0; i < G::MPW; i++) acc[i][j] = __builtin_amdgcn_mfma_f32_16x16x32_bf16(A[i], B[j - jb], acc[i][j], 0, 0, 0);
+              __builtin_amdgcn_sched_barrier(0);
+            }
+            if (ng == 0) {
+#pragma unroll
+              for (int i = 0; i < G::MPW; i++) bacc[i] = __builtin_amdgcn_mfma_f32_16x16x32_bf16(A[i], ones, bacc[i], 0, 0, 0);
+            }
           }
-#pragma unroll
-          for (int jb = 0; jb < G::NPW; jb += JB) {
-#pragma unroll
-            for (int j = jb; j < jb + JB && j < G::NPW; j++) {
-              const int tofs = ((j / L::KW) * L::IW + j % L::KW) * G::CIP;
-              B[j - jb] = tr_frag(yb + ir0[s] + coff + tofs, yb + ir1[s] + coff + tofs);
-            }
-            __builtin_amdgcn_sched_barrier(0);
-#pragma unroll
-            for (int j = jb; j < jb + JB && j < G::NPW; j++)
-#pragma unroll
-              for (int i = 0; i < G::MPW; i++) acc[i][j] = __builtin_amdgcn_mfma_f32_16x16x32_bf16(A[i], B[j - jb], acc[i][j], 0, 0, 0);
-            __builtin_amdgcn_sched_barrier(0);
-          }
-          if (ng == 0) {
-#pragma unroll
-            for (int i = 0; i < G::MPW; i++) bacc[i] = __builtin_amdgcn_mfma_f32_16x16x32_bf16(A[i], ones, bacc[i], 0, 0, 0);
-          }
-        }
-      }
-      L3_ST(3);
-      if (nxt < n_img) put(y2s + (kb ^ 1) * G::Y2E);
-      __syncthreads();
-      L3_ST(4);
-    }
-    if (j0 < n_img) flush(j0 + ((n_img - 1 - j0) / a.wpp) * a.wpp, z2s + (kb ^ 1) * G::Z2E);
-    if constexpr (ROLE == 1) {
-      float* sl = a.slab + (long)blockIdx.x * TG::SLABF;
-#pragma unroll
-      for (int i = 0; i < G::MPW; i++)
-#pragma unroll
-        for (int j = 0; j < G::NPW; j++)
-          *reinterpret_cast<f32x4*>(sl + (((wv * G::MPW + i) * G::NPW + j) * 64 + lane) * 4) = acc[i][j];
-      if (ng == 0 && l16 == 0) {
-#pragma unroll
-        for (int i = 0; i < G::MPW; i++)
-#pragma unroll
-          for (int r = 0; r < 4; r++) sl[L::CO * L::TAPS + 16 * (mg * G::MPW + i) + 4 * g + r] = bacc[i][r];
-      }
-    }
-    dt = wave_sum(dt);
-    if (lane == 0) shd[w] = dt;
-    __syncthreads();
-    if (tid == 0 && j0 < n_img) {
-      float sum = 0.f;
-#pragma unroll
-      for (int ww = 0; ww < NW3; ww++) sum += shd[ww];
-      a.dtp[p][j0] = sum;
-    }
+        }
+        L3_ST(3);
+        if (nxt < hi) put(y2s + (kb ^ 1) * G::Y2E);
+        __syncthreads();
+        L3_ST(4);
+        zprev = a.dz2[p] + (long)(gi - a.ln.start[p]) * G::Z2E;
+      }
+      segment_end(p);
+      if (pend == hi) break;
+      p = np;
+    }
+    flush(zprev, z2s + (kb ^ 1) * G::Z2E);
 #ifdef L3_STAMPS
     L3_ST(5);
     if (tid == 64 * w && blockIdx.x == 0 && (w == 0 || w == ND3)) {
@@ -831,28 +934,60 @@
 inline int cdivi(long a, long b) { return (int)((a + b - 1) / b); }
 constexpr int cdivi_c(int a, int b) { return (a + b - 1) / b; }
 
+struct LinePlan {
+  ImgLine ln;
+  int N, nwg, maxper, nslab, cnt[EBW_MAXP];
+};
+LinePlan make_line(int nprob, const int* n, int cap) {
+  LinePlan lp{};
+  ImgLine& ln = lp.ln;
+  for (int p = 0; p < nprob; p++) ln.start[p + 1] = ln.start[p] + (n[p] > 0 ? n[p] : 0);
+  const int N = ln.start[nprob];
+  for (int p = nprob; p < EBW_MAXP; p++) ln.start[p + 1] = N;
+  lp.N = N;
+  lp.nwg = cap < N ? cap : N;
+  ln.nwg = lp.nwg > 0 ? lp.nwg : 1;
+  ln.q = N / ln.nwg; ln.r = N % ln.nwg;
+  lp.maxper = ln.q + (ln.r ? 1 : 0);
+  int b = 0;
+  for (int p = 0; p < nprob; p++) {
+    ln.sbase[p] = lp.nslab;
+    if (ln.start[p + 1] == ln.start[p]) { ln.fwg[p] = b; continue; }
+    while (line_lo(ln, b + 1) <= ln.start[p]) b++;
+    ln.fwg[p] = b;
+    while (line_lo(ln, b + 1) < ln.start[p + 1]) b++;
+    lp.cnt[p] = b - ln.fwg[p] + 1;
+    lp.nslab += lp.cnt[p];
+  }
+  return lp;
+}
+
+constexpr int kCUs = 256;
+constexpr int per_cu(size_t lds) { return 2 * lds <= 160 * 1024 ? 2 : 1; }
+
 struct WsPlan {
   size_t wpk2[EBW_MAXP], wpk3[EBW_MAXP], dz2[EBW_MAXP], dz1[EBW_MAXP], slab1, slab2, slab3, total;
-  int wpp;
+  LinePlan wide, d3, d2;
 };
 template <class G>
-WsPlan plan(int nprob, const int* n) {
+WsPlan plan(int nprob, const int* n, int max_wg) {
   WsPlan w{};
-  long maxn = 1;
-  for (int p = 0; p < nprob; p++) maxn = n[p] > maxn ? n[p] : maxn;
-  const int per = 256 / nprob > 1 ? 256 / nprob : 1;
-  w.wpp = (int)(per < maxn ? per : maxn);
+  const int cap = max_wg > 0 && max_wg < kCUs ? max_wg : kCUs;
+  w.wide = make_line(nprob, n, cap);
+  w.d3 = make_line(nprob, n, per_cu(dgrad_lds_bytes<typename G::L3>()) * cap);
+  w.d2 = make_line(nprob, n, per_cu(dgrad_lds_bytes<typename G::L2>()) * cap);
   size_t off = 0;
   for (int p = 0; p < nprob; p++) {
+    const size_t np = n[p] > 0 ? n[p] : 0;
     w.wpk2[p] = off; off += al256((size_t)G::L2::NCOMBO * G::L2::KS * 64 * 16);
     w.wpk3[p] = off; off += al256((size_t)G::L3::NCOMBO * G::L3::KS * 64 * 16);
-    w.dz2[p] = off; off += al256((size_t)n[p] * G::L3::IH * G::L3::IW * 64 * 2);
-    w.dz1[p] = off; off += al256((size_t)n[p] * G::L2::IH * G::L2::IW * 32 * 2);
-  }
-  const size_t nwg = (size_t)nprob * w.wpp;
-  w.slab1 = off; off += al256(nwg * TrGeo<typename G::L1>::SLABF * 4);
-  w.slab2 = off; off += al256(nwg * TrGeo<typename G::L2>::SLABF * 4);
-  w.slab3 = off; off += al256(nwg * TrGeo<typename G::L3>::SLABF * 4);
+    w.dz2[p] = off; off += al256(np * G::L3::IH * G::L3::IW * 64 * 2);
+    w.dz1[p] = off; off += al256(np * G::L2::IH * G::L2::IW * 32 * 2);
+  }
+  const size_t nsl = (size_t)(w.wide.nwg > 0 ? w.wide.nwg : 1) + nprob - 1;
+  w.slab1 = off; off += al256(nsl * TrGeo<typename G::L1>::SLABF * 4);
+  w.slab2 = off; off += al256(nsl * TrGeo<typename G::L2>::SLABF * 4);
+  w.slab3 = off; off += al256(nsl * TrGeo<typename G::L3>::SLABF * 4);
   w.total = off;
   return w;
 }
@@ -891,14 +1026,14 @@
   return TACORL_OK;
 }
 template <class G>
-int run(int nprob, const EbwProblem* pr, int accumulate, void* ws, size_t ws_bytes, hipStream_t st, int mode, int parts) {
+int run(int nprob, const EbwProblem* pr, int accumulate, void* ws, size_t ws_bytes, hipStream_t st, int mode, int parts, int max_wg) {
   using L1 = typename G::L1; using L2 = typename G::L2; using L3 = typename G::L3;
   int n[EBW_MAXP];
   for (int p = 0; p < nprob; p++) n[p] = pr[p].n;
-  const WsPlan w = plan<G>(nprob, n);
+  const WsPlan w = plan<G>(nprob, n, max_wg);
   if (ws_bytes < w.total) return TACORL_ENOMEM;
   unsigned char* base = (unsigned char*)ws;
-  const int nwg = nprob * w.wpp;
+  const int nwg = w.wide.nwg;
   PkArgs k2{}, k3{};
   for (int p = 0; p < nprob; p++) {
     k2.w[p] = pr[p].w2; k2.out[p] = (uint4*)(base + w.wpk2[p]);
@@ -915,22 +1050,15 @@
   for (int p = 0; p < nprob; p++) {
     __bf16* dz2 = (__bf16*)(base + w.dz2[p]);
     __bf16* dz1 = (__bf16*)(base + w.dz1[p]);
-    d3.dz[p] = pr[p].dz3; d3.yin[p] = (const __bf16*)pr[p].y2; d3.wpk[p] = k3.out[p]; d3.dx[p] = dz2; d3.n[p] = n[p];
-    d2.dz[p] = dz2; d2.yin[p] = (const __bf16*)pr[p].y1; d2.wpk[p] = k2.out[p]; d2.dx[p] = dz1; d2.n[p] = n[p];
-    g3.in[p] = pr[p].y2; g3.dz[p] = pr[p].dz3; g3.n[p] = n[p];
-    g2.in[p] = pr[p].y1; g2.dz[p] = dz2; g2.n[p] = n[p];
-    g1.in[p] = pr[p].img; g1.dz[p] = dz1; g1.n[p] = n[p];
+    d3.dz[p] = pr[p].dz3; d3.yin[p] = (const __bf16*)pr[p].y2; d3.wpk[p] = k3.out[p]; d3.dx[p] = dz2;
+    d2.dz[p] = dz2; d2.yin[p] = (const __bf16*)pr[p].y1; d2.wpk[p] = k2.out[p]; d2.dx[p] = dz1;
+    g3.in[p] = pr[p].y2; g3.dz[p] = pr[p].dz3;
+    g2.in[p] = pr[p].y1; g2.dz[p] = dz2;
+    g1.in[p] = pr[p].img; g1.dz[p] = dz1;
     gw1[p] = pr[p].g_w1; gb1[p] = pr[p].g_b1; gw2[p] = pr[p].g_w2; gb2[p] = pr[p].g_b2;
     gw3[p] = pr[p].g_w3; gb3[p] = pr[p].g_b3;
   }
-  d3.wpp = d2.wpp = g3.wpp = g2.wpp = g1.wpp = w.wpp;
-  constexpr int dg2 = 2;
-  long maxn = 1;
-  for (int p = 0; p < nprob; p++) maxn = n[p] > maxn ? n[p] : maxn;
-  auto per_cu = [](size_t lds) { return (size_t)dg2 * lds <= 160 * 1024 ? dg2 : 1; };
-  const int k3w = per_cu(dgrad_lds_bytes<L3>()), k2w = per_cu(dgrad_lds_bytes<L2>());
-  d3.wpp = (int)((long)k3w * w.wpp < maxn ? (long)k3w * w.wpp : maxn);
-  d2.wpp = (int)((long)k2w * w.wpp < maxn ? (long)k2w * w.wpp : maxn);
+  d3.ln = w.d3.ln; d2.ln = w.d2.ln; g3.ln = g2.ln = g1.ln = w.wide.ln;
   g1.slab = (float*)(base + w.slab1); g2.slab = (float*)(base + w.slab2); g3.slab = (float*)(base + w.slab3);
   int rc;
   const bool fused3 = (parts & EBW_FUSED3) != 0;
@@ -941,21 +1069,21 @@
       for (int p = 0; p < nprob; p++) {
         f.y3[p] = pr[p].y3; f.temp[p] = pr[p].temp; f.sa[p] = pr[p].sa; f.d_sa[p] = pr[p].d_sa;
         f.y2[p] = (const __bf16*)pr[p].y2; f.wpk[p] = k3.out[p]; f.dz2[p] = (__bf16*)(base + w.dz2[p]);
-        f.dtp[p] = pr[p].dtp; f.n[p] = n[p];
-      }
-      f.slab = g3.slab; f.wpp = w.wpp;
+        f.dtp[p] = pr[p].dtp;
+      }
+      f.slab = g3.slab; f.ln = w.wide.ln;
       if constexpr (L3Geo<L3>::ok) {
-        if ((rc = launch_l3<L3>(f, nwg, st))) return rc;
+        if (nwg > 0 && (rc = launch_l3<L3>(f, nwg, st))) return rc;
       } else {
         return TACORL_EINVAL;
       }
     } else {
-      if ((parts & EBW_DGRAD3) && (rc = launch_dgrad<L3, float>(d3, nprob * d3.wpp, st))) return rc;
-      if ((parts & EBW_WGRAD3) && (rc = launch_wgrad_tr<L3, __bf16, float>(g3, nwg, st))) return rc;
-    }
-    if ((parts & EBW_DGRAD2) && (rc = launch_dgrad<L2, __bf16>(d2, nprob * d2.wpp, st))) return rc;
-    if ((parts & EBW_WGRAD2) && (rc = launch_wgrad_tr<L2, __bf16, __bf16>(g2, nwg, st))) return rc;
-    if ((parts & EBW_WGRAD1) && (rc = launch_wgrad_tr<L1, __bf16, __bf16>(g1, nwg, st))) return rc;
+      if ((parts & EBW_DGRAD3) && nwg > 0 && (rc = launch_dgrad<L3, float>(d3, w.d3.nwg, st))) return rc;
+      if ((parts & EBW_WGRAD3) && nwg > 0 && (rc = launch_wgrad_tr<L3, __bf16, float>(g3, nwg, st))) return rc;
+    }
+    if ((parts & EBW_DGRAD2) && nwg > 0 && (rc = launch_dgrad<L2, __bf16>(d2, w.d2.nwg, st))) return rc;
+    if ((parts & EBW_WGRAD2) && nwg > 0 && (rc = launch_wgrad_tr<L2, __bf16, __bf16>(g2, nwg, st))) return rc;
+    if ((parts & EBW_WGRAD1) && nwg > 0 && (rc = launch_wgrad_tr<L1, __bf16, __bf16>(g1, nwg, st))) return rc;
     if (!(parts & EBW_REDUCE)) return hipGetLastError() == hipSuccess ? TACORL_OK : TACORL_ELAUNCH;
     RdTrArgs t{};
     t.slab[0] = g1.slab; t.slab[1] = g2.slab; t.slab[2] = g3.slab;
@@ -965,15 +1093,16 @@
       t.ngrp[l] = TG::T::NGRP; t.kgrp[l] = TG::T::KGRP; t.slabf[l] = TG::SLABF;
     };
     fill(0, TrGeo<L1>{}, L1::CO, L1::TAPS); fill(1, TrGeo<L2>{}, L2::CO, L2::TAPS); fill(2, TrGeo<L3>{}, L3::CO, L3::TAPS);
-    t.wpp = w.wpp; t.accumulate = accumulate;
+    t.accumulate = accumulate;
     for (int p = 0; p < nprob; p++) {
+      t.sbase[p] = w.wide.ln.sbase[p]; t.cnt[p] = w.wide.cnt[p];
       t.gw[0][p] = gw1[p]; t.gb[0][p] = gb1[p]; t.gw[1][p] = gw2[p]; t.gb[1][p] = gb2[p];
       t.gw[2][p] = gw3[p]; t.gb[2][p] = gb3[p];
     }
     constexpr int maxper_t = cmax(L1::SLABF, cmax(L2::SLABF, L3::SLABF));
     static_assert(cdivi_c(maxper_t, 64) - 1 > cdivi_c(L1::SLABF, 64), "the temperature block must lie beyond conv1's elements");
     if (fused3) {
-      for (int p = 0; p < nprob; p++) { t.dtp[p] = pr[p].dtp; t.g_temp[p] = pr[p].g_temp; t.ndt[p] = n[p] < w.wpp ? n[p] : w.wpp; }
+      for (int p = 0; p < nprob; p++) { t.dtp[p] = pr[p].dtp; t.g_temp[p] = pr[p].g_temp; t.ndt[p] = w.wide.cnt[p]; }
       t.ileave[2] = 1; t.mpw[2] = L3Geo<L3>::MPW; t.npw[2] = L3Geo<L3>::NPW; t.mgrp[2] = L3Tile::MGRP; t.ngrp[2] = L3Tile::NGRP;
     }
     hipLaunchKernelGGL(ebw_reduce_tr_kernel, dim3(cdivi(maxper_t, 64), 3 * nprob), dim3(256), 0, st, t);
@@ -997,17 +1126,35 @@
 #undef X
   return false;
 }
-size_t ebw_ws_bytes(int nprob, const int* n_img, int H, int W) {
+size_t ebw_ws_bytes(int nprob, const int* n_img, int H, int W, int max_wg) {
   if (nprob < 1 || nprob > EBW_MAXP) return 0;
-#define X(h, w) if (H == h && W == w) return plan<Geo<h, w>>(nprob, n_img).total;
+#define X(h, w) if (H == h && W == w) return plan<Geo<h, w>>(nprob, n_img, max_wg).total;
   EBW_GEOMS(X)
 #undef X
   return 0;
 }
+int ebw_plan_query(int nprob, const int* n_img, int H, int W, int max_wg, int* out, int* ranges) {
+  if (nprob < 1 || nprob > EBW_MAXP) return TACORL_EINVAL;
+  WsPlan w{};
+  bool ok = false;
+#define X(h, w_) if (H == h && W == w_) { w = plan<Geo<h, w_>>(nprob, n_img, max_wg); ok = true; }
+  EBW_GEOMS(X)
+#undef X
+  if (!ok) return TACORL_EINVAL;
+  const LinePlan* lp[3] = {&w.wide, &w.d3, &w.d2};
+  for (int c = 0; c < 3; c++) {
+    int* o = out + c * EBW_PLAN_STRIDE;
+    o[0] = lp[c]->nwg; o[1] = lp[c]->maxper;
+    for (int p = 0; p < EBW_MAXP; p++) o[2 + p] = p < nprob ? lp[c]->cnt[p] : 0;
+    if (ranges)
+      for (int b = 0; b <= lp[c]->nwg; b++) ranges[c * EBW_PLAN_RANGES + b] = lp[c]->nwg > 0 ? line_lo(lp[c]->ln, b) : 0;
+  }
+  return TACORL_OK;
+}
 int ebw_conv_backward(int nprob, const EbwProblem* pr, int H, int W, int accumulate, void* ws, size_t ws_bytes,
-                      hipStream_t st, int mode, int parts) {
+                      hipStream_t st, int mode, int parts, int max_wg) {
   if (nprob < 1 || nprob > EBW_MAXP) return TACORL_EINVAL;
-#define X(h, w) if (H == h && W == w) return run<Geo<h, w>>(nprob, pr, accumulate, ws, ws_bytes, st, mode, parts);
+#define X(h, w) if (H == h && W == w) return run<Geo<h, w>>(nprob, pr, accumulate, ws, ws_bytes, st, mode, parts, max_wg);
   EBW_GEOMS(X)
 #undef X
   return TACORL_EINVAL;
```

Result: slower. 1219 grad-steps/s (-1.0%).
